# laprade117/interactive-unet

Measured on AMD Instinct MI355X. Metric: voxels/sec (train step + full-volume predict) on 128^3 chunks, higher is better.
Workload: dtype bf16

## Files before the change

### include/iunet.h

```cpp
#ifndef IUNET_H
#define IUNET_H
#ifdef __cplusplus
extern "C" {
#endif

const char* iunet_last_error(void);
int iunet_abi_version(void);

long long iunet_pack_conv3_elems(int Cout, int Cin, int taps, int mode);
int iunet_pack_conv3(int dtype, const void* w, const void* scale, void* dst, int Cout, int Cin, int taps, int mode,
                     void* stream);
long long iunet_pack_first_conv_elems(int Cout, int Cin, int taps);
int iunet_pack_first_conv(int dtype, const void* w, const void* scale, void* dst, int Cout, int Cin, int taps,
                          void* stream);
int iunet_pack_convT(int dtype, const void* w, void* dst, int Cin, int Cout, int npos, void* stream);

int iunet_pack_desc_bytes(void);
int iunet_pack_batch(const void* descs, int n, int quant_max_cout, void* stream);

int iunet_conv3_fwd(int dtype, int nd, const void* x, long long x_sstride, void* y, long long y_sstride,
                    const void* wpk, const void* bias, void* stats, int N, int D, int H, int W, int Cin, int Cout,
                    int epi, int layout, void* stream);
int iunet_conv3_pick_layout(int nd, int N, int D, int H, int W, int Cin, int Cout);
int iunet_conv3_tile_pairs(int nd, int N, int D, int H, int W, int Cin, int Cout);
int iunet_conv3_compact_ok(int nd, int N, int D, int H, int W, int Cin, int Cout, int act, int bw);
int iunet_conv3_packs_compact(int taps, int Cin);
int iunet_conv3_plan(int nd, int N, int D, int H, int W, int Cin, int Cout, int act, int bw, int have_compact, int* fused);
int iunet_conv3_fwd_act(int dtype, int nd, const void* x, long long x_sstride, void* y, long long y_sstride,
                        const void* wpk, const void* bias, void* stats, const void* in_scale, const void* in_shift,
                        int N, int D, int H, int W, int Cin, int Cout, int epi, int layout, void* stream);
int iunet_conv3_num_tiles(int nd, int N, int D, int H, int W);
int iunet_conv3_stats_parts(int nd, int N, int D, int H, int W, int Cout, int layout);
int iunet_first_conv_fwd(int dtype, int nd, const void* x, int in_dtype, const long long* in_strides, void* y,
                         long long y_sstride, const void* w, const void* bias, void* stats, int N, int D, int H, int W,
                         int Cin, int Cout, int relu, void* stream);
int iunet_maxpool_fwd(int dtype, int nd, const void* x, long long x_ss, void* y, long long y_ss, int C, int N, int Do,
                      int Ho, int Wo, void* stream);
int iunet_convT_fwd(int dtype, int nd, const void* x, long long x_ss, void* y, long long y_ss, const void* wpk,
                    const void* bias, int N, int D, int H, int W, int Cin, int Cout, void* stream);
int iunet_head_fwd(int dtype, const void* x, long long x_ss, int C0, const void* w, const void* bias, int ncls,
                   void* logits, void* probs, void* cls, const long long* out_strides, float divisor, int accumulate,
                   int N, int D, int H, int W, void* stream);

long long iunet_f32_pack_conv_elems(int Cout, int Cin, int taps);
int iunet_f32_pack_conv(const void* w, void* dst, void* bias_out, const void* gamma, const void* beta, const void* mean,
                        const void* var, float eps, int Cout, int Cin, int taps, int transposed, void* stream);
int iunet_f32_conv_fwd(int nd, const void* x, int in_dtype, const long long* in_strides, void* y, long long y_ss,
                       const void* wpk, const void* bias, int N, int D, int H, int W, int Cin, int Cout, int relu,
                       int transposed, void* stream);
int iunet_f32_maxpool_fwd(int nd, const void* x, long long x_ss, void* y, long long y_ss, int C, int N, int Do, int Ho, int Wo,
                          void* stream);
int iunet_f32_head_fwd(const void* x, long long x_ss, int C0, const void* w, const void* bias, int ncls, void* logits,
                       void* probs, void* cls, const long long* out_strides, float divisor, int accumulate, int N, int D, int H,
                       int W, void* stream);

int iunet_f32_bn_stats(const void* y, long long y_ss, int C, int N, long long vox, float eps, float momentum, void* mean, void* stdv,
                       void* run_mean, void* run_var, void* stream);
int iunet_f32_bn_relu_fwd(const void* y, long long y_ss, void* z, long long z_ss, const void* mean, const void* stdv, const void* gamma,
                          const void* beta, int C, int N, long long vox, void* stream);
int iunet_f32_bn_relu_bwd(const void* dz, long long dz_ss, const void* y, long long y_ss, void* dy, long long dy_ss, const void* mean,
                          const void* stdv, const void* gamma, const void* beta, void* dgamma, void* dbeta, int C, int N, long long vox,
                          void* stream);
int iunet_f32_maxpool_bwd(int nd, const void* z, long long z_ss, const void* dpool, long long dp_ss, void* dz, long long dz_ss, int C,
                          int N, int Do, int Ho, int Wo, int accumulate, void* stream);
int iunet_f32_wgrad_splits(int nd, int N, int D, int H, int W, int Cin, int Cout);
int iunet_f32_wgrad(int nd, const void* x, long long x_ss, const void* dy, long long dy_ss, void* slab, int N, int D, int H, int W,
                    int Cin, int Cout, int taps, void* stream);
int iunet_f32_head_loss_num_parts(int N, long long vox);
int iunet_f32_head_loss_fwd(const void* x, long long x_ss, int C0, const void* w, const void* bias, int ncls, const void* target,
                            const void* weight, int tdtype, int kind, void* slab, void* out4, void* coef, int N, long long vox,
                            void* stream);
int iunet_f32_head_loss_bwd(const void* x, long long x_ss, int C0, const void* w, const void* bias, int ncls, const void* target,
                            const void* weight, int tdtype, const void* coef, void* dlogits, long long dl_ss, void* dx, long long dx_ss,
                            int N, long long vox, void* stream);
int iunet_f32_channel_sum(const void* t, long long t_ss, void* out, int C, int N, long long vox, void* stream);

int iunet_x2_convT_kc(int Cin);
int iunet_x2_prep(const void* w, void* wv, void* oscale, void* bias_out, const void* gamma, const void* beta, const void* mean,
                  const void* var, const void* bias_in, float eps, float act_in, float act_out, int Cout, int Cin, int taps,
                  int transposed, int chunk, void* stream);
int iunet_x2_prep_desc_bytes(void);
int iunet_x2_prep_batch(const void* table, int n, int rows, void* stream);
int iunet_x2m_prep_batch(const void* table, int n, int rows, void* stream);
int iunet_x2_first_conv_fwd(int nd, const void* x, int in_dtype, const long long* in_strides, void* y, long long y_sstride, int y_lo,
                            const void* w, const void* oscale, const void* bias, float act_scale, int N, int D, int H, int W, int Cin,
                            int Cout, int relu, void* stream);
int iunet_x2_pack_mode(int nd);
int iunet_x2_conv3_fwd(int nd, const void* x, long long x_sstride, int x_lo, void* y, long long y_sstride, int y_lo, const void* wpk,
                       const void* oscale, const void* bias, int N, int D, int H, int W, int Cin, int Cout, int epi, void* stream);
int iunet_x2_conv3_fwd_flag(int nd, const void* x, long long x_sstride, int x_lo, void* y, long long y_sstride, int y_lo, const void* wpk,
                            const void* oscale, const void* bias, int N, int D, int H, int W, int Cin, int Cout, int epi, void* sat, void* stream);
int iunet_x2_maxpool_fwd(int nd, const void* x, long long x_ss, int x_lo, void* y, long long y_ss, int y_lo, int C, int N, int Do,
// ... 197 lines not shown
                           const void* gamma, const void* beta, int groups, float eps, void* slab, void* scale, void* shift, void* mean,
                           void* invstd, int C, int N, int Do, int Ho, int Wo, void* stream);
int iunet_conv3_sample_stats_rows(int dtype, int nd, int N, int D, int H, int W, int Cin, int Cout, int layout);
int iunet_conv3_fwd_sample_stats(int dtype, int nd, const void* x, long long x_sstride, void* y, long long y_sstride, const void* wpk,
                                 void* stats, int N, int D, int H, int W, int Cin, int Cout, int layout, void* stream);
int iunet_gn_relu_fwd_rows(int dtype, const void* y, long long y_ss, void* z, long long z_ss, const void* gamma, const void* beta,
                           int groups, float eps, void* slab, int rows, void* scale, void* shift, void* mean, void* invstd, int C, int N,
                           long long vox, void* stream);
int iunet_gn_relu_pool_fwd_rows(int dtype, int nd, const void* y, long long y_ss, void* z, long long z_ss, void* pooled, long long p_ss,
                                const void* gamma, const void* beta, int groups, float eps, void* slab, int rows, void* scale, void* shift,
                                void* mean, void* invstd, int C, int N, int Do, int Ho, int Wo, void* stream);
int iunet_conv3_dgrad_sample_bnstats(int dtype, int nd, const void* dy, long long dy_sstride, void* dz, long long dz_sstride, const void* wpk,
                                     void* stats, const void* yp, long long yp_sstride, const void* mean, const void* invstd, const void* scale,
                                     const void* shift, int N, int D, int H, int W, int Cin, int Cout, int layout, void* stream);
int iunet_gn_relu_bwd_rows(int dtype, const void* dz, long long dz_ss, const void* y, long long y_ss, void* dy, long long dy_ss,
                           const void* gamma, int groups, const void* scale, const void* shift, const void* mean, const void* invstd,
                           void* dgamma, void* dbeta, void* slab, int rows, void* coef, int C, int N, long long vox, void* stream);
int iunet_gn_relu_pool_bwd(int dtype, int nd, const void* dskip, long long ds_ss, const void* dpool, long long dp_ss, const void* y,
                           long long y_ss, void* dy, long long dy_ss, const void* gamma, int groups, const void* scale, const void* shift,
                           const void* mean, const void* invstd, void* dgamma, void* dbeta, void* slab, void* coef, int C, int N, int Do,
                           int Ho, int Wo, void* stream);
int iunet_bn_relu_pool_bwd(int dtype, int nd, const void* dskip, long long ds_ss, const void* dpool, long long dp_ss,
                           const void* y, long long y_ss, void* dy, long long dy_ss, const void* mean, const void* invstd,
                           const void* gamma, const void* scale, const void* shift, void* dgamma, void* dbeta, void* slab,
                           void* coef, int C, int N, int Do, int Ho, int Wo, void* stream);
int iunet_maxpool_bwd(int dtype, int nd, const void* z, long long z_ss, const void* dpool, long long dp_ss, void* dz,
                      long long dz_ss, int add_skip, int C, int N, int Do, int Ho, int Wo, void* stream);
int iunet_head_loss_num_parts(int N, long long vox);
int iunet_head_loss_fwd(int dtype, const void* x, long long x_ss, int C0, const void* w, const void* bias, int ncls,
                        const void* target, const void* weight, int tdtype, int kind, void* slab, void* out4, void* coef,
                        int N, long long vox, void* stream);
int iunet_head_loss_bwd_num_parts(int N, long long vox, int ncls, int C0);
int iunet_head_loss_bwd(int dtype, const void* x, long long x_ss, int C0, const void* w, const void* bias, int ncls,
                        const void* target, const void* weight, int tdtype, const void* coef, float loss_scale, void* dx,
                        long long dx_ss, void* dwslab, int N, long long vox, void* stream);
int iunet_head_loss_fwd_act(int dtype, const void* x, long long x_ss, int C0, const void* w, const void* bias, int ncls,
                            const void* target, const void* weight, int tdtype, int kind, void* slab, void* out4, void* coef,
                            const void* in_scale, const void* in_shift, int N, long long vox, void* stream);
int iunet_head_loss_bwd_act(int dtype, const void* x, long long x_ss, int C0, const void* w, const void* bias, int ncls,
                            const void* target, const void* weight, int tdtype, const void* coef, float loss_scale, void* dx,
                            long long dx_ss, void* dwslab, const void* in_scale, const void* in_shift, int N, long long vox,
                            void* stream);
int iunet_reduce_slab(void* slab, int nparts, long long n, void* out, float alpha, int accumulate, void* stream);
int iunet_conv3_wgrad_blocks(int nd, int N, int D, int H, int W, int Cin, int Cout);
long long iunet_conv3_wgrad_slab_floats(int nd, int N, int D, int H, int W, int Cin, int Cout);
int iunet_conv3_wgrad(int dtype, int nd, const void* x, long long x_ss, const void* dy, long long dy_ss, void* slab,
                      void* dW, float alpha, int N, int D, int H, int W, int Cin, int Cout, void* stream);
int iunet_conv3_wgrad_act(int dtype, int nd, const void* x, long long x_ss, const void* dy, long long dy_ss, void* slab,
                          void* dW, float alpha, const void* x_scale, const void* x_shift, int N, int D, int H, int W,
                          int Cin, int Cout, void* stream);
int iunet_pack_convT_dgrad(int dtype, const void* w, void* dst, int Cin, int Cout, int npos, void* stream);
int iunet_convT_dgrad(int dtype, int nd, const void* dy, long long dy_ss, void* dx, long long dx_ss, const void* wpk,
                      int N, int D, int H, int W, int Cin, int Cout, void* stream);
int iunet_convT_wgrad_blocks(int nd, int N, int D, int H, int W, int Cin, int Cout);
int iunet_convT_wgrad(int dtype, int nd, const void* x, long long x_ss, const void* dy, long long dy_ss, void* wslab,
                      void* bslab, void* dW, void* db, int N, int D, int H, int W, int Cin, int Cout, void* stream);
int iunet_first_conv_wgrad_blocks(int nd, int N, int D, int H, int W);
int iunet_first_conv_wgrad(int dtype, int nd, const void* x, int in_dtype, const long long* in_strides, const void* dy,
                           long long dy_ss, void* slab, void* dW, int N, int D, int H, int W, int Cin, int Cout,
                           void* stream);
int iunet_first_conv_wgrad_bn(int dtype, int nd, const void* x, int in_dtype, const long long* in_strides, const void* dz,
                              long long dz_ss, const void* y, long long y_ss, const void* mean, const void* invstd,
                              const void* coef, const void* scale, const void* shift, void* slab, void* dW, int N, int D, int H,
                              int W, int Cin, int Cout, void* stream);
int iunet_check_finite(const void* g, long long n, void* flag, void* stream);
int iunet_adamw_step(void* p, const void* g, void* m, void* v, long long n, float lr, float b1, float b2, float eps,
                     float wd, int step, float grad_scale_inv, const void* skip_flag, void* stream);

int iunet_train_state_init(void* state, float loss_scale, int dynamic, void* stream);
int iunet_head_loss_bwd_dev(int dtype, const void* x, long long x_ss, int C0, const void* w, const void* bias, int ncls,
                            const void* target, const void* weight, int tdtype, const void* coef, const void* state, void* dx,
                            long long dx_ss, void* dwslab, const void* in_scale, const void* in_shift, int N, long long vox,
                            void* stream);
int iunet_head_bn_bwd_ok(int C0, int ncls);
int iunet_head_bn_bwd(int dtype, const void* y, long long y_ss, int C0, const void* w, const void* bias, int ncls, const void* target,
                      const void* weight, int tdtype, const void* coef, float loss_scale, const void* state, const void* scale,
                      const void* shift, const void* mean, const void* invstd, const void* gamma, void* dgamma, void* dbeta, void* dy,
                      long long dy_ss, void* dwslab, void* bnslab, void* bncoef, void* dl_scratch, int N, long long vox, void* stream);
int iunet_head_gn_bwd(int dtype, const void* y, long long y_ss, int C0, const void* w, const void* bias, int ncls, const void* target,
                      const void* weight, int tdtype, const void* coef, float loss_scale, const void* state, const void* scale,
                      const void* shift, const void* mean, const void* invstd, const void* gamma, int groups, void* dgamma, void* dbeta, void* dy,
                      long long dy_ss, void* dwslab, void* bnslab, void* bncoef, void* dl_scratch, int N, long long vox, void* stream);
int iunet_head_loss_fwd_act_ps(int dtype, const void* x, long long x_ss, int C0, const void* w, const void* bias, int ncls,
                               const void* target, const void* weight, int tdtype, int kind, void* slab, void* out4, void* coef,
                               const void* in_scale, const void* in_shift, int per_sample, int N, long long vox, void* stream);
int iunet_head_grad_scatter(const void* row, void* dw, void* db, int ncls, int C0, void* stream);
int iunet_adamw_step_dev(void* p, const void* g, void* m, void* v, long long n, float lr, float b1, float b2, float eps, float wd,
                         void* state, int check, float world, void* stream);

typedef struct iunet_train iunet_train;
int iunet_train_create(int dim, int levels, int base, int cin, int ncls, int dtype, int loss_kind, iunet_train** out);
int iunet_train_create_ex(int dim, int levels, int base, int cin, int ncls, int dtype, int loss_kind, int norm, int groups, iunet_train** out);
int iunet_train_create_nested(int dim, int levels, int base, int cin, int ncls, int dtype, int loss_kind, iunet_train** out);
void iunet_train_destroy(iunet_train* t);
long long iunet_train_num_params(const iunet_train* t);
int iunet_train_num_tensors(const iunet_train* t);
int iunet_train_param(const iunet_train* t, int index, char* name, int name_cap, long long* offset, long long* numel);
int iunet_train_num_bn(const iunet_train* t);
long long iunet_train_packed_bytes(const iunet_train* t);
long long iunet_train_workspace_bytes(const iunet_train* t, int N, int D, int H, int W);
int iunet_train_bind(iunet_train* t, void* flat, void* grad, void* m, void* v, void* const* running, void* packed, void* state, void* stream);
int iunet_train_repack(iunet_train* t, void* stream);
int iunet_train_forward_backward(iunet_train* t, const void* x, int in_dtype, const long long* in_strides, const void* target,
                                 const void* weight, int tdtype, int N, int D, int H, int W, void* workspace, void* out4, void* stream);
typedef void (*iunet_train_hook)(void* ctx, int stage);
int iunet_train_forward_backward_hooks(iunet_train* t, const void* x, int in_dtype, const long long* in_strides, const void* target,
                                       const void* weight, int tdtype, int N, int D, int H, int W, void* workspace, void* out4,
                                       iunet_train_hook hook, void* hook_ctx, void* stream);
int iunet_train_update(iunet_train* t, float lr, float b1, float b2, float eps, float wd, float world, void* stream);
// ... 108 lines not shown
```

### interactive-unet_amd/csrc/capi.hip

```cpp
#include "common.h"
#include <cstdarg>
#include <cstdio>

static thread_local char g_err[512] = "";

void iunet_set_error(const char* fmt, ...) {
  va_list ap;
  va_start(ap, fmt);
  vsnprintf(g_err, sizeof(g_err), fmt, ap);
  va_end(ap);
}

#define DT_OK(dt) IUNET_REQUIRE((dt) == 0 || (dt) == 1, "dtype must be 0 (f16) or 1 (bf16), got %d", (dt))

extern "C" {

const char* iunet_last_error(void) { return g_err; }
int iunet_abi_version(void) { return 1; }

int iunet_conv3_num_tiles(int nd, int N, int D, int H, int W) { return iunet_conv3_tiles(nd, N, D, H, W); }

int iunet_conv3_stats_parts(int nd, int N, int D, int H, int W, int Cout, int layout) {
  return layout >= 2 ? iunet_conv3_v4_stats_parts(nd, Cout) : iunet_conv3_tiles(nd, N, D, H, W);
}
// ... 112 lines not shown
  IUNET_REQUIRE(nd == 3 || D == 1, "conv3: 2-D conv needs D == 1");
  const float* par[4] = {(const float*)mean, (const float*)invstd, (const float*)scale, (const float*)shift};
  return iunet_conv3_v4_launch(dtype, nd, dy, dy_sstride, dz, dz_sstride, wpk, nullptr, (float*)stats, N, D, H, W, Cin, Cout, 0, nullptr, nullptr,
                               (hipStream_t)stream, yp, yp_sstride, par, layout == 3, 1, nullptr);
}

int iunet_conv3_dgrad_bnstats_lay(int dtype, int nd, const void* dy, long long dy_sstride, void* dz, long long dz_sstride,
                                  const void* wpk, void* stats, const void* yp, long long yp_sstride, const void* mean,
                                  const void* invstd, const void* scale, const void* shift, int N, int D, int H, int W, int Cin,
                                  int Cout, int layout, void* stream) {
  DT_OK(dtype);
  IUNET_REQUIRE(dy && dz && wpk && stats && yp && mean && invstd && scale && shift, "conv3_dgrad_bnstats: null pointer");
  IUNET_REQUIRE_GRID("conv3_dgrad_bnstats", N, D, H, W);
  IUNET_REQUIRE(layout == 2 || layout == 3, "conv3_dgrad_bnstats: layout 2, or 3 (the compact operator: 2-D, Cin <= 64; iunet_conv3_compact_ok(.., bw = 1)) -- got %d", layout);
  const float* par[4] = {(const float*)mean, (const float*)invstd, (const float*)scale, (const float*)shift};
  return iunet_conv3_launch(dtype, nd, dy, dy_sstride, dz, dz_sstride, wpk, nullptr, (float*)stats, N, D, H, W, Cin, Cout, 0, layout,
                            (hipStream_t)stream, nullptr, nullptr, yp, yp_sstride, par);
}

int iunet_conv3_dgrad_bnstats(int dtype, int nd, const void* dy, long long dy_sstride, void* dz, long long dz_sstride,
                              const void* wpk, void* stats, const void* yp, long long yp_sstride, const void* mean,
                              const void* invstd, const void* scale, const void* shift, int N, int D, int H, int W, int Cin,
                              int Cout, void* stream) {
  return iunet_conv3_dgrad_bnstats_lay(dtype, nd, dy, dy_sstride, dz, dz_sstride, wpk, stats, yp, yp_sstride, mean, invstd, scale, shift,
                                       N, D, H, W, Cin, Cout, 2, stream);
}

int iunet_first_conv_fwd(int dtype, int nd, const void* x, int in_dtype, const long long* in_strides, void* y,
                         long long y_sstride, const void* w, const void* bias, void* stats, int N, int D, int H, int W,
                         int Cin, int Cout, int relu, void* stream) {
  DT_OK(dtype);
  IUNET_REQUIRE(x && y && w && in_strides, "first_conv: null pointer");
  IUNET_REQUIRE(in_dtype >= 0 && in_dtype <= 3, "first_conv: bad input dtype %d", in_dtype);
  IUNET_REQUIRE(nd == 2 || nd == 3, "first_conv: nd must be 2 or 3");
  IUNET_REQUIRE(nd == 3 || D == 1, "first_conv: 2-D needs D == 1");
  return iunet_first_conv_launch(dtype, nd, x, in_dtype, in_strides[0], in_strides[1], in_strides[2], in_strides[3],
                                 in_strides[4], y, y_sstride, w, (const float*)bias, (float*)stats, N, D,
                                 H, W, Cin, Cout, relu, (hipStream_t)stream);
}

int iunet_maxpool_fwd(int dtype, int nd, const void* x, long long x_ss, void* y, long long y_ss, int C, int N, int Do,
                      int Ho, int Wo, void* stream) {
  DT_OK(dtype);
  IUNET_REQUIRE(x && y, "maxpool: null pointer");
  IUNET_REQUIRE(C % 8 == 0, "maxpool: C must be a multiple of 8");
  return iunet_maxpool_launch(dtype, nd, x, x_ss, y, y_ss, C / 8, N, Do, Ho, Wo, (hipStream_t)stream);
}

int iunet_convT_fwd(int dtype, int nd, const void* x, long long x_ss, void* y, long long y_ss, const void* wpk,
                    const void* bias, int N, int D, int H, int W, int Cin, int Cout, void* stream) {
  DT_OK(dtype);
  IUNET_REQUIRE(x && y && wpk, "convT: null pointer");
  return iunet_convT_launch(dtype, nd, x, x_ss, y, y_ss, wpk, (const float*)bias, N, D, H, W, Cin, Cout, (hipStream_t)stream);
}

int iunet_head_fwd(int dtype, const void* x, long long x_ss, int C0, const void* w, const void* bias, int ncls,
                   void* logits, void* probs, void* cls, const long long* out_strides, float divisor, int accumulate,
                   int N, int D, int H, int W, void* stream) {
  DT_OK(dtype);
  IUNET_REQUIRE(x && w && bias && out_strides, "head: null pointer");
  IUNET_REQUIRE(C0 % 8 == 0, "head: C0 must be a multiple of 8");
  return iunet_head_launch(dtype, x, x_ss, C0, (const float*)w, (const float*)bias, ncls, (float*)logits, (float*)probs,
                           (unsigned char*)cls, out_strides, divisor, accumulate, N, D, H, W, (hipStream_t)stream);
}

long long iunet_f32_pack_conv_elems(int Cout, int Cin, int taps) {
  if (Cout <= 0 || Cout % 32 || Cin <= 0 || taps <= 0) return 0;
  return iunet_f32_pack_size(Cout, Cin, taps);
}

int iunet_f32_pack_conv(const void* w, void* dst, void* bias_out, const void* gamma, const void* beta, const void* mean,
                        const void* var, float eps, int Cout, int Cin, int taps, int transposed, void* stream) {
  IUNET_REQUIRE(w && dst, "f32_pack_conv: null pointer");
  IUNET_REQUIRE(Cout > 0 && Cout % 32 == 0 && Cin > 0, "f32_pack_conv: Cout must be a positive multiple of 32, Cin > 0 (got %d, %d)", Cout, Cin);
  IUNET_REQUIRE(transposed ? (taps == 4 || taps == 8) : (taps == 9 || taps == 27 || taps == 1),
                "f32_pack_conv: taps must be 9 / 27 (conv), 1 (pointwise) or 4 / 8 (transposed), got %d", taps);
  IUNET_REQUIRE(!gamma || (beta && mean && var && bias_out), "f32_pack_conv: a BatchNorm fold needs gamma, beta, mean, var and bias_out");
  return iunet_f32_pack_launch((const float*)w, (float*)dst, (float*)bias_out, (const float*)gamma, (const float*)beta,
                               (const float*)mean, (const float*)var, eps, Cout, Cin, taps, transposed, (hipStream_t)stream);
}

int iunet_f32_conv_fwd(int nd, const void* x, int in_dtype, const long long* in_strides, void* y, long long y_ss,
                       const void* wpk, const void* bias, int N, int D, int H, int W, int Cin, int Cout, int relu,
                       int transposed, void* stream) {
  IUNET_REQUIRE(x && y && wpk && in_strides, "f32_conv: null pointer");
  IUNET_REQUIRE(nd == 2 || nd == 3, "f32_conv: nd must be 2 or 3");
  IUNET_REQUIRE(N > 0 && D > 0 && H > 0 && W > 0 && (nd == 3 || D == 1), "f32_conv: bad shape %d %d %d %d", N, D, H, W);
  IUNET_REQUIRE(in_dtype >= 0 && in_dtype <= 3, "f32_conv: bad input dtype %d", in_dtype);
  IUNET_REQUIRE(Cout > 0 && Cout % 32 == 0 && Cin > 0, "f32_conv: Cout must be a positive multiple of 32, Cin > 0 (got %d, %d)", Cout, Cin);
  IUNET_REQUIRE(transposed >= 0 && transposed <= 2, "f32_conv: transposed must be 0 (conv), 1 (ConvTranspose k2 s2) or 2 (1x1), got %d", transposed);
  return iunet_f32_conv_launch(nd, x, in_dtype, in_strides, (float*)y, y_ss, (const float*)wpk, (const float*)bias, N, D, H, W,
                               Cin, Cout, relu, transposed, (hipStream_t)stream);
}

int iunet_f32_maxpool_fwd(int nd, const void* x, long long x_ss, void* y, long long y_ss, int C, int N, int Do, int Ho, int Wo,
                          void* stream) {
  IUNET_REQUIRE(x && y, "f32_maxpool: null pointer");
  IUNET_REQUIRE(nd == 2 || nd == 3, "f32_maxpool: nd must be 2 or 3");
  IUNET_REQUIRE(C > 0 && N > 0 && Do > 0 && Ho > 0 && Wo > 0, "f32_maxpool: bad shape");
  return iunet_f32_maxpool_launch(nd, (const float*)x, x_ss, (float*)y, y_ss, C, N, Do, Ho, Wo, (hipStream_t)stream);
}

int iunet_f32_head_fwd(const void* x, long long x_ss, int C0, const void* w, const void* bias, int ncls, void* logits,
                       void* probs, void* cls, const long long* out_strides, float divisor, int accumulate, int N, int D, int H,
                       int W, void* stream) {
  IUNET_REQUIRE(x && w && bias && out_strides, "f32_head: null pointer");
// ... 96 lines not shown
```

### interactive-unet_amd/csrc/launchers.h

```cpp
#pragma once
#include <hip/hip_runtime.h>

void iunet_set_error(const char* fmt, ...);

int iunet_conv3_launch(int dtype, int nd, const void* x, long long x_sstride, void* y, long long y_sstride,
                       const void* wpk, const float* bias, float* stats, int N, int D, int H, int W, int Cin,
                       int Cout, int epi, int layout, hipStream_t stream, const float* in_scale = nullptr,
                       const float* in_shift = nullptr, const void* bw_y = nullptr, long long bw_y_ss = 0,
                       const float* const* bw_par = nullptr);
int iunet_conv3_tiles(int nd, int N, int D, int H, int W);
long long iunet_pack_conv3_size(int Cout, int Cin, int taps, int mode);
int iunet_pack_conv3_launch(int dtype, const float* w, const float* scale, void* dst, int Cout, int Cin, int taps,
                            int mode, hipStream_t stream);

int iunet_conv3_v4_launch(int dtype, int nd, const void* x, long long x_sstride, void* y, long long y_sstride, const void* wpk,
                          const float* bias, float* stats, int N, int D, int H, int W, int Cin, int Cout, int epi,
                          const float* in_scale, const float* in_shift, hipStream_t stream, const void* bw_y = nullptr,
                          long long bw_y_ss = 0, const float* const* bw_par = nullptr, int compact = 0, int per_sample = 0,
                          int* query_rows = nullptr);
int iunet_conv3_v4_stats_parts(int nd, int Cout);
int iunet_conv3_v4_pairs(int nd, int N, int D, int H, int W, int Cin, int Cout, int bw);
int iunet_conv3_v4_x2_launch(int nd, const void* x, long long x_sstride, int x_lo, void* y, long long y_sstride, int y_lo, const void* wpk,
                             const float* oscale, const float* bias, int N, int D, int H, int W, int Cin, int Cout, int epi,
                             int* sat, hipStream_t stream);
int iunet_conv3_v4_x2_pack_mode(int nd);

int iunet_first_conv_launch(int dtype, int nd, const void* x, int in_dtype, long long sN, long long sC, long long sD,
                            long long sH, long long sW, void* y, long long y_sstride, const void* w,
                            const float* bias, float* stats, int N, int D, int H, int W, int Cin, int Cout, int relu,
                            hipStream_t stream, int out8 = 0);
int iunet_pack_first_conv_launch(int dtype, const float* w, const float* scale, void* dst, int Cout, int Cin, int taps,
                                 hipStream_t stream);
int iunet_maxpool_launch(int dtype, int nd, const void* x, long long x_ss, void* y, long long y_ss, int planes, int N,
                         int Do, int Ho, int Wo, hipStream_t stream);
int iunet_maxpool_q_launch(int nd, const void* x, long long x_ss, void* y, long long y_ss, int planes16, int N, int Do, int Ho, int Wo,
                           hipStream_t stream);
int iunet_convT_launch(int dtype, int nd, const void* x, long long x_ss, void* y, long long y_ss, const void* wpk,
                       const float* bias, int N, int D, int H, int W, int Cin, int Cout, hipStream_t stream, int out8 = 0);
int iunet_pack_convT_launch(int dtype, const float* w, void* dst, int Cin, int Cout, int npos, hipStream_t stream);
int iunet_head_launch(int dtype, const void* x, long long x_ss, int C0, const float* w, const float* bias, int ncls,
                      float* logits, float* probs, unsigned char* cls, const long long* os, float divisor, int accumulate, int N,
                      int D, int H, int W,
                      hipStream_t stream);

long long iunet_f32_pack_size(int Cout, int Cin, int taps);
int iunet_f32_pack_launch(const float* w, float* dst, float* bias_out, const float* gamma, const float* beta,
                          const float* mean, const float* var, float eps, int Cout, int Cin, int taps, int transposed,
                          hipStream_t stream);
int iunet_f32_conv_launch(int nd, const void* x, int in_dtype, const long long* st, float* y, long long y_ss, const float* wpk,
                          const float* bias, int N, int D, int H, int W, int Cin, int Cout, int relu, int transposed,
                          hipStream_t stream);
int iunet_f32_maxpool_launch(int nd, const float* x, long long x_ss, float* y, long long y_ss, int C, int N, int Do, int Ho,
                             int Wo, hipStream_t stream);
int iunet_f32_head_launch(const float* x, long long x_ss, int C0, const float* w, const float* bias, int ncls, float* logits,
                          float* probs, unsigned char* cls, const long long* os, float divisor, int accumulate, int N, int D,
                          int H, int W, hipStream_t stream);

long long iunet_f8_pack_bytes(int Cout, int Cin, int taps);
int iunet_f8_pack_launch(const float* w, const float* gamma, const float* beta, const float* mean, const float* var, float eps,
                         void* dst, float* wscale, float* bias_out, int Cout, int Cin, int taps, hipStream_t stream);
long long iunet_conv3_f8_workspace_floats(int nd, int N, int D, int H, int W, int Cin, int Cout);
int iunet_conv3_f8_launch(int dtype, int nd, const void* x, long long x_sstride, void* y, long long y_sstride, const void* wpk,
                          const float* wscale, const float* bias, int N, int D, int H, int W, int Cin, int Cout, int epi,
                          float* workspace, hipStream_t stream);
int iunet_conv3_f8_launch_q(int dtype, int nd, const void* x, long long x_sstride, int x_fmt, void* y, long long y_sstride, int y_fmt,
                            const void* wpk, const float* wscale, const float* bias, int N, int D, int H, int W, int Cin, int Cout,
                            int epi, float* workspace, hipStream_t stream);

int iunet_f8_k128(int taps, int Cin);
int iunet_conv3_f8k_launch(int dtype, const void* x, long long x_sstride, void* y, long long y_sstride, const void* wpk,
                           const float* wscale, const float* bias, int N, int D, int H, int W, int Cin, int Cout, int epi,
                           int ksplit, float* partial, int small, int in8, int out8, hipStream_t stream);

int iunet_conv3_wgrad_v2_blocks(int N, int D, int H, int W, int Cin, int Cout);
int iunet_conv3_wgrad_v2_launch(int dtype, const void* x, long long x_ss, const void* dy, long long dy_ss, float* slab,
                                int N, int D, int H, int W, int Cin, int Cout, const float* x_scale, const float* x_shift,
                                hipStream_t stream);
int iunet_conv2_wgrad_v2_blocks(int N, int H, int W, int Cin, int Cout, int* rows);
int iunet_conv2_wgrad_v2_launch(int dtype, const void* x, long long x_ss, const void* dy, long long dy_ss, float* slab, int N, int H, int W,
                                int Cin, int Cout, const float* x_scale, const float* x_shift, hipStream_t stream);

int iunet_loss_finalize_launch(const float* slab, int nparts, int ncls, int kind, int has_weight, double nvox_total, float* out4,
                               float* coef, hipStream_t stream);
```

### interactive-unet_amd/csrc/pointwise.hip

```cpp
#include "common.h"
#include "head_out.h"

namespace {

struct FirstConvParams {
  const void* x;
  long long sN, sC, sD, sH, sW;
  int in_dtype;
  void* y; long long y_sstride;
  const void* w;
  const float* bias;
  float* stats;
  int N, D, H, W, Cin, Cout, nd, relu;
  int out8;
};

__device__ __forceinline__ float load_in(const void* p, long long off, int dt) {
  switch (dt) {
    case 0: return ((const float*)p)[off];
    case 1: return (float)((const f16*)p)[off];
    case 2: return (float)((const unsigned char*)p)[off] / 255.0f;
    default: return (float)((const bf16*)p)[off];
  }
}
// ... 155 lines not shown
#pragma unroll
  for (int j = 0; j < 8; ++j) o[j] = from_f32<T>(m[j]);
  *(V8*)(y + n * y_ss + (long long)pl * ovox * 8 + r * 8) = o;
}

template <int ND>
__global__ __launch_bounds__(256) void maxpool_q_kernel(const unsigned char* __restrict__ x, long long x_ss, unsigned char* __restrict__ y,
                                                        long long y_ss, int planes16, int Do, int Ho, int Wo) {
  const long long ovox = (long long)Do * Ho * Wo;
  const long long total = ovox * planes16;
  const long long i = (long long)blockIdx.x * 256 + threadIdx.x;
  if (i >= total) return;
  const int n = blockIdx.y;
  const int pl = (int)(i / ovox);
  const long long r = i - (long long)pl * ovox;
  const int ox = (int)(r % Wo), oy = (int)((r / Wo) % Ho), oz = (int)(r / ((long long)Wo * Ho));
  const int Di = ND == 3 ? Do * 2 : 1, Hi = Ho * 2, Wi = Wo * 2;
  const unsigned char* xp = x + n * x_ss + (long long)pl * Di * Hi * Wi * 16;
  float m[16];
#pragma unroll
  for (int j = 0; j < 16; ++j) m[j] = -INFINITY;
#pragma unroll
  for (int a = 0; a < (ND == 3 ? 2 : 1); ++a)
#pragma unroll
    for (int b = 0; b < 2; ++b)
#pragma unroll
      for (int c = 0; c < 2; ++c) {
        const int z = ND == 3 ? oz * 2 + a : 0;
        const u32x4 v = *(const u32x4*)(xp + (((long long)z * Hi + oy * 2 + b) * Wi + ox * 2 + c) * 16);
#pragma unroll
        for (int d = 0; d < 4; ++d) {
          m[4 * d + 0] = fmaxf(m[4 * d + 0], __builtin_amdgcn_cvt_f32_fp8((int)v[d], 0));
          m[4 * d + 1] = fmaxf(m[4 * d + 1], __builtin_amdgcn_cvt_f32_fp8((int)v[d], 1));
          m[4 * d + 2] = fmaxf(m[4 * d + 2], __builtin_amdgcn_cvt_f32_fp8((int)v[d], 2));
          m[4 * d + 3] = fmaxf(m[4 * d + 3], __builtin_amdgcn_cvt_f32_fp8((int)v[d], 3));
        }
      }
  u32x4 o;
#pragma unroll
  for (int d = 0; d < 4; ++d) {
    int w = __builtin_amdgcn_cvt_pk_fp8_f32(m[4 * d], m[4 * d + 1], 0, false);
    w = __builtin_amdgcn_cvt_pk_fp8_f32(m[4 * d + 2], m[4 * d + 3], w, true);
    o[d] = (unsigned)w;
  }
  *(u32x4*)(y + n * y_ss + ((long long)pl * ovox + r) * 16) = o;
}

struct ConvTParams {
  const void* x; long long x_sstride;
  void* y; long long y_sstride;
  const void* wpk; const float* bias;
  int N, D, H, W, Cin, Cout;
  int out8;
};

template <typename T, int ND, bool O8 = false>
__global__ __launch_bounds__(256) void convT_kernel(ConvTParams p) {
  using V8 = typename Vec8<T>::type;
  constexpr int NPOS = ND == 3 ? 8 : 4;
  const int lane = threadIdx.x & 63, wave = threadIdx.x >> 6;
  const int l15 = lane & 15, q = lane >> 4;
  const int xg = (p.W + 15) / 16;
  const long long rows = (long long)p.D * p.H * xg;
  const long long wid = (long long)blockIdx.x * 4 + wave;
  if (wid >= rows * p.N) return;
  const int n = (int)(wid / rows);
  const long long r = wid - n * rows;
  const int xb = (int)(r % xg), y = (int)((r / xg) % p.H), z = (int)(r / ((long long)xg * p.H));
  const int cob = blockIdx.y;
  const int x = xb * 16 + l15;
  const bool ok = x < p.W;
  const int xc = ok ? x : p.W - 1;
  const long long in_plane = (long long)p.D * p.H * p.W * 8;
  const T* xin = (const T*)p.x + n * p.x_sstride + (((long long)z * p.H + y) * p.W + xc) * 8;
  const int nk = p.Cin >> 5;
  const V8* wp = (const V8*)p.wpk + (long long)cob * nk * NPOS * 2 * 64 + lane;

  f32x4 acc[NPOS][2];
#pragma unroll
  for (int s = 0; s < NPOS; ++s) { acc[s][0] = f32x4{0, 0, 0, 0}; acc[s][1] = f32x4{0, 0, 0, 0}; }
  for (int ks = 0; ks < nk; ++ks) {
    const V8 b = *(const V8*)(xin + (long long)(ks * 4 + q) * in_plane);
#pragma unroll
    for (int s = 0; s < NPOS; ++s) {
      const V8 a0 = wp[((ks * NPOS + s) * 2 + 0) * 64];
      const V8 a1 = wp[((ks * NPOS + s) * 2 + 1) * 64];
      acc[s][0] = mfma16<T>(a0, b, acc[s][0]);
      acc[s][1] = mfma16<T>(a1, b, acc[s][1]);
    }
  }
  const int Do = ND == 3 ? p.D * 2 : 1, Ho = p.H * 2, Wo = p.W * 2;
  const long long out_plane = (long long)Do * Ho * Wo * 8;
  T* yout = (T*)p.y + n * p.y_sstride + (long long)(cob * 4 + q) * out_plane;
  float bias[8];
#pragma unroll
  for (int j = 0; j < 8; ++j) bias[j] = p.bias ? p.bias[cob * 32 + q * 8 + j] : 0.f;
  const int src_lo = ((lane & 48) | (l15 >> 1)) * 4, src_hi = src_lo + 8 * 4;
  const bool odd = l15 & 1;
  const int x0 = xb * 16;
#pragma unroll
  for (int sp = 0; sp < NPOS / 2; ++sp) {
    const int a = ND == 3 ? (sp >> 1) : 0, b = sp & 1;
    typedef int i32x4 __attribute__((ext_vector_type(4)));
    i32x4 oc[2];
#pragma unroll
    for (int c = 0; c < 2; ++c) {
      V8 o;
#pragma unroll
      for (int j = 0; j < 4; ++j) {
        o[j] = from_f32<T>(acc[sp * 2 + c][0][j] + bias[j]);
        o[4 + j] = from_f32<T>(acc[sp * 2 + c][1][j] + bias[4 + j]);
      }
      oc[c] = __builtin_bit_cast(i32x4, o);
    }
    const int oz = ND == 3 ? z * 2 + a : 0;
    T* row = yout + (((long long)oz * Ho + y * 2 + b) * Wo + 2 * x0) * 8;
#pragma unroll
    for (int h = 0; h < 2; ++h) {
      const int src = h ? src_hi : src_lo;
      i32x4 v;
#pragma unroll
      for (int d = 0; d < 4; ++d) {
        const int t0 = __builtin_amdgcn_ds_bpermute(src, oc[0][d]);
        const int t1 = __builtin_amdgcn_ds_bpermute(src, oc[1][d]);
        v[d] = odd ? t1 : t0;
      }
      const int xo = 2 * x0 + 16 * h + l15;
      if (xo < Wo) {
        if constexpr (!O8) *(i32x4*)(row + (16 * h + l15) * 8) = v;
        else e4m3_store8<T>((unsigned char*)p.y + (long long)n * p.y_sstride, cob * 4 + q, ((long long)oz * Ho + y * 2 + b) * Wo + xo,
                            (long long)Do * Ho * Wo, __builtin_bit_cast(u32x4, v));
      }
    }
  }
}

template <typename T, int ND, int NK, bool O8 = false, int NT = 256>
__global__ __launch_bounds__(NT, NT == 256 ? 2 : 1) void convT_lds_kernel(ConvTParams p) {
  constexpr int NW = NT / 64;
  using V8 = typename Vec8<T>::type;
  constexpr int NPOS = ND == 3 ? 8 : 4;
  constexpr int G = 2;
  extern __shared__ __attribute__((aligned(256))) unsigned char smem[];
  const int lane = threadIdx.x & 63, wave = threadIdx.x >> 6;
  const int l15 = lane & 15, q = lane >> 4;
  const int cob = blockIdx.y;
  {
    const u32x4* wsrc = (const u32x4*)p.wpk + (long long)cob * NK * NPOS * 2 * 64;
    stage_to_lds(smem, wsrc, NK * NPOS * 2 * 64, threadIdx.x, NT);
    if (threadIdx.x < 32) ((float*)(smem + NK * NPOS * 2 * 1024))[threadIdx.x] = p.bias ? p.bias[cob * 32 + threadIdx.x] : 0.f;
  }
  __syncthreads();
  const int xg = (p.W + 15) / 16;
  const long long rows = (long long)p.D * p.H * xg, ngroups = rows * p.N;
  const long long in_plane = (long long)p.D * p.H * p.W * 8;
  const int Do = ND == 3 ? p.D * 2 : 1, Ho = p.H * 2, Wo = p.W * 2;
  const long long out_plane = (long long)Do * Ho * Wo * 8;
  const int src_lo = ((lane & 48) | (l15 >> 1)) * 4, src_hi = src_lo + 8 * 4;
  const bool odd = l15 & 1;

  struct Where { int n, z, y, xb; const T* xin; };
  auto locate = [&](long long wid) -> Where {
    wid = wid < ngroups ? wid : ngroups - 1;
    Where w;
    w.n = (int)(wid / rows);
    const long long r = wid - w.n * rows;
    w.xb = (int)(r % xg); w.y = (int)((r / xg) % p.H); w.z = (int)(r / ((long long)xg * p.H));
    const int xc = min(w.xb * 16 + l15, p.W - 1);
    w.xin = (const T*)p.x + w.n * p.x_sstride + (((long long)w.z * p.H + w.y) * p.W + xc) * 8 + (long long)q * in_plane;
    return w;
  };
  const long long stride = (long long)gridDim.x * NW * G;
  long long g0 = ((long long)blockIdx.x * NW + wave) * G;
  if (g0 >= ngroups) return;
  Where cur[G];
  V8 b[G][NK];
#pragma unroll
  for (int g = 0; g < G; ++g) {
    cur[g] = locate(g0 + g);
#pragma unroll
    for (int ks = 0; ks < NK; ++ks) b[g][ks] = *(const V8*)(cur[g].xin + (long long)(ks * 4) * in_plane);
  }
  for (; g0 < ngroups; g0 += stride) {
    Where nxt[G];
#pragma unroll
    for (int g = 0; g < G; ++g) nxt[g] = locate(g0 + stride + g);
    unsigned woff = lane * 16;
    asm volatile("" : "+v"(woff));
    const V8* wl = (const V8*)(smem + woff);
#pragma unroll
    for (int hf = 0; hf < 2; ++hf) {
      constexpr int HP = NPOS / 2;
      f32x4 acc[G][HP][2];
#pragma unroll
      for (int g = 0; g < G; ++g)
#pragma unroll
        for (int s = 0; s < HP; ++s) { acc[g][s][0] = f32x4{0, 0, 0, 0}; acc[g][s][1] = f32x4{0, 0, 0, 0}; }
#pragma unroll
      for (int ks = 0; ks < NK; ++ks) {
#pragma unroll
        for (int s = 0; s < HP; ++s) {
          const V8 a0 = wl[((ks * NPOS + hf * HP + s) * 2 + 0) * 64];
          const V8 a1 = wl[((ks * NPOS + hf * HP + s) * 2 + 1) * 64];
#pragma unroll
          for (int g = 0; g < G; ++g) {
            acc[g][s][0] = mfma16<T>(a0, b[g][ks], acc[g][s][0]);
            acc[g][s][1] = mfma16<T>(a1, b[g][ks], acc[g][s][1]);
          }
        }
        if (hf == 1) {
#pragma unroll
          for (int g = 0; g < G; ++g) b[g][ks] = *(const V8*)(nxt[g].xin + (long long)(ks * 4) * in_plane);
        }
      }
#pragma unroll
      for (int g = 0; g < G; ++g) {
        if (g0 + g >= ngroups) break;
        T* yout = (T*)p.y + cur[g].n * p.y_sstride + (long long)(cob * 4 + q) * out_plane;
        const int x0 = cur[g].xb * 16;
#pragma unroll
        for (int s2 = 0; s2 < HP / 2; ++s2) {
          const int sp = hf * (HP / 2) + s2;
          const int a = ND == 3 ? (sp >> 1) : 0, bb = sp & 1;
          typedef int i32x4 __attribute__((ext_vector_type(4)));
          i32x4 oc[2];
          const f32x4 bias0 = ((const f32x4*)(smem + NK * NPOS * 2 * 1024))[2 * q], bias1 = ((const f32x4*)(smem + NK * NPOS * 2 * 1024))[2 * q + 1];
#pragma unroll
          for (int c = 0; c < 2; ++c) {
            V8 o;
#pragma unroll
            for (int j = 0; j < 4; ++j) {
              o[j] = from_f32<T>(acc[g][s2 * 2 + c][0][j] + bias0[j]);
              o[4 + j] = from_f32<T>(acc[g][s2 * 2 + c][1][j] + bias1[j]);
            }
            oc[c] = __builtin_bit_cast(i32x4, o);
          }
          const int oz = ND == 3 ? cur[g].z * 2 + a : 0;
          if constexpr (O8) {
            unsigned E[2][2];
            e4m3_pack8<T>(__builtin_bit_cast(u32x4, oc[0]), E[0][0], E[0][1]);
            e4m3_pack8<T>(__builtin_bit_cast(u32x4, oc[1]), E[1][0], E[1][1]);
            const bool oq = q & 1;
            const int partner = (lane ^ 16) * 4;
            const unsigned r0 = (unsigned)__builtin_amdgcn_ds_bpermute(partner, (int)(oq ? E[0][0] : E[1][0]));
            const unsigned r1 = (unsigned)__builtin_amdgcn_ds_bpermute(partner, (int)(oq ? E[0][1] : E[1][1]));
            const u32x4 gran = oq ? u32x4{r0, r1, E[1][0], E[1][1]} : u32x4{E[0][0], E[0][1], r0, r1};
            if (x0 + l15 < p.W)
              *(u32x4*)((unsigned char*)p.y + (long long)cur[g].n * p.y_sstride +
                        ((long long)((cob * 4 + q) >> 1) * ((long long)Do * Ho * Wo) + ((long long)oz * Ho + cur[g].y * 2 + bb) * Wo + 2 * (x0 + l15) + (oq ? 1 : 0)) * 16) = gran;
            continue;
          }
          T* row = yout + (((long long)oz * Ho + cur[g].y * 2 + bb) * Wo + 2 * x0) * 8;
#pragma unroll
          for (int h = 0; h < 2; ++h) {
            const int src = h ? src_hi : src_lo;
            i32x4 v;
#pragma unroll
            for (int d = 0; d < 4; ++d) {
              const int t0 = __builtin_amdgcn_ds_bpermute(src, oc[0][d]);
              const int t1 = __builtin_amdgcn_ds_bpermute(src, oc[1][d]);
              v[d] = odd ? t1 : t0;
            }
            if (2 * x0 + 16 * h + l15 < Wo) {
              if constexpr (!O8) *(i32x4*)(row + (16 * h + l15) * 8) = v;
              else e4m3_store8<T>((unsigned char*)p.y + (long long)cur[g].n * p.y_sstride, cob * 4 + q,
                                  ((long long)oz * Ho + cur[g].y * 2 + bb) * Wo + 2 * x0 + 16 * h + l15, (long long)Do * Ho * Wo,
                                  __builtin_bit_cast(u32x4, v));
            }
          }
        }
      }
    }
#pragma unroll
    for (int g = 0; g < G; ++g) cur[g] = nxt[g];
  }
}

template <typename T, int ND, bool O8 = false>
__global__ __launch_bounds__(256) void convT_chunk_kernel(ConvTParams p) {
  constexpr int NK = 4;
  using V8 = typename Vec8<T>::type;
  constexpr int NPOS = ND == 3 ? 8 : 4;
  constexpr int G = 2;
  extern __shared__ __attribute__((aligned(256))) unsigned char smem[];
  const int lane = threadIdx.x & 63, wave = threadIdx.x >> 6;
  const int l15 = lane & 15, q = lane >> 4;
  const int cob = blockIdx.y;
  const int nchunks = (p.Cin >> 5) / NK;
  const u32x4* wsrc = (const u32x4*)p.wpk + (long long)cob * nchunks * NK * NPOS * 2 * 64;
  const int xg = (p.W + 15) / 16;
  const long long rows = (long long)p.D * p.H * xg, ngroups = rows * p.N;
  const long long in_plane = (long long)p.D * p.H * p.W * 8;
  const int Do = ND == 3 ? p.D * 2 : 1, Ho = p.H * 2, Wo = p.W * 2;
  const long long out_plane = (long long)Do * Ho * Wo * 8;
  float bias[8];
#pragma unroll
  for (int j = 0; j < 8; ++j) bias[j] = p.bias ? p.bias[cob * 32 + q * 8 + j] : 0.f;
  const int src_lo = ((lane & 48) | (l15 >> 1)) * 4, src_hi = src_lo + 8 * 4;
  const bool odd = l15 & 1;
  const V8* wl = (const V8*)smem + lane;

  for (long long base = (long long)blockIdx.x * 4 * G; base < ngroups; base += (long long)gridDim.x * 4 * G) {
    const long long g0 = base + wave * G;
    int n_[G], z_[G], y_[G], xb_[G];
    const T* xin_[G];
#pragma unroll
    for (int g = 0; g < G; ++g) {
      const long long wid = g0 + g < ngroups ? g0 + g : ngroups - 1;
      n_[g] = (int)(wid / rows);
      const long long r = wid - n_[g] * rows;
      xb_[g] = (int)(r % xg); y_[g] = (int)((r / xg) % p.H); z_[g] = (int)(r / ((long long)xg * p.H));
      const int xc = min(xb_[g] * 16 + l15, p.W - 1);
      xin_[g] = (const T*)p.x + n_[g] * p.x_sstride + (((long long)z_[g] * p.H + y_[g]) * p.W + xc) * 8;
    }
    f32x4 acc[G][NPOS][2];
#pragma unroll
    for (int g = 0; g < G; ++g)
#pragma unroll
      for (int s = 0; s < NPOS; ++s) { acc[g][s][0] = f32x4{0, 0, 0, 0}; acc[g][s][1] = f32x4{0, 0, 0, 0}; }
    constexpr int CHB = NK * NPOS * 2 * 1024;
    const unsigned lds0 = (unsigned)(size_t)(__attribute__((address_space(3))) unsigned char*)smem;
    auto dma_chunk = [&](int ch) {
      const u32x4* src = wsrc + (long long)ch * (CHB / 16);
#pragma unroll
      for (int i = 0; i < CHB / 16 / 256; ++i) {
        const int base = (i * 4 + wave) * 64;
        const unsigned dst = __builtin_amdgcn_readfirstlane(lds0 + (ch & 1) * CHB + base * 16);
        const u32x4* gsrc = src + base + lane;
        unsigned keep;
        asm volatile("s_mov_b32 %0, m0\n\ts_mov_b32 m0, %2\n\ts_nop 0\n\tglobal_load_lds_dwordx4 %1, off\n\ts_mov_b32 m0, %0"
                     : "=&s"(keep) : "v"(gsrc), "s"(dst) : "memory");
      }
    };
    auto load_b = [&](int ch, V8 (&bb)[G][NK]) {
#pragma unroll
      for (int g = 0; g < G; ++g)
#pragma unroll
        for (int ks = 0; ks < NK; ++ks) bb[g][ks] = *(const V8*)(xin_[g] + (long long)((ch * NK + ks) * 4 + q) * in_plane);
    };
    V8 bcur[G][NK], bnext[G][NK];
    __syncthreads();
    dma_chunk(0);
    load_b(0, bcur);
    for (int ch = 0; ch < nchunks; ++ch) {
      asm volatile("s_waitcnt vmcnt(0)" ::: "memory");
      __syncthreads();
      if (ch + 1 < nchunks) { dma_chunk(ch + 1); load_b(ch + 1, bnext); }
      const V8* wb = wl + (ch & 1) * (CHB / 16);
#pragma unroll
      for (int ks = 0; ks < NK; ++ks)
#pragma unroll
        for (int s = 0; s < NPOS; ++s) {
          const V8 a0 = wb[((ks * NPOS + s) * 2 + 0) * 64];
          const V8 a1 = wb[((ks * NPOS + s) * 2 + 1) * 64];
#pragma unroll
          for (int g = 0; g < G; ++g) {
            acc[g][s][0] = mfma16<T>(a0, bcur[g][ks], acc[g][s][0]);
            acc[g][s][1] = mfma16<T>(a1, bcur[g][ks], acc[g][s][1]);
          }
        }
      if (ch + 1 < nchunks) {
#pragma unroll
        for (int g = 0; g < G; ++g)
#pragma unroll
          for (int ks = 0; ks < NK; ++ks) bcur[g][ks] = bnext[g][ks];
      }
    }
#pragma unroll
    for (int g = 0; g < G; ++g) {
      if (g0 + g >= ngroups) break;
      T* yout = (T*)p.y + n_[g] * p.y_sstride + (long long)(cob * 4 + q) * out_plane;
      const int x0 = xb_[g] * 16;
#pragma unroll
      for (int sp = 0; sp < NPOS / 2; ++sp) {
        const int a = ND == 3 ? (sp >> 1) : 0, bb = sp & 1;
        typedef int i32x4 __attribute__((ext_vector_type(4)));
        i32x4 oc[2];
#pragma unroll
        for (int c = 0; c < 2; ++c) {
          V8 o;
#pragma unroll
          for (int j = 0; j < 4; ++j) {
            o[j] = from_f32<T>(acc[g][sp * 2 + c][0][j] + bias[j]);
            o[4 + j] = from_f32<T>(acc[g][sp * 2 + c][1][j] + bias[4 + j]);
          }
          oc[c] = __builtin_bit_cast(i32x4, o);
        }
        const int oz = ND == 3 ? z_[g] * 2 + a : 0;
        T* row = yout + (((long long)oz * Ho + y_[g] * 2 + bb) * Wo + 2 * x0) * 8;
#pragma unroll
        for (int h = 0; h < 2; ++h) {
          const int src = h ? src_hi : src_lo;
          i32x4 v;
#pragma unroll
          for (int d = 0; d < 4; ++d) {
            const int t0 = __builtin_amdgcn_ds_bpermute(src, oc[0][d]);
            const int t1 = __builtin_amdgcn_ds_bpermute(src, oc[1][d]);
            v[d] = odd ? t1 : t0;
          }
          if (2 * x0 + 16 * h + l15 < Wo) {
// ... 70 lines not shown
  FirstConvParams p;
  p.x = x; p.sN = sN; p.sC = sC; p.sD = sD; p.sH = sH; p.sW = sW; p.in_dtype = in_dtype;
  p.y = y; p.y_sstride = y_sstride; p.w = w; p.bias = bias; p.stats = stats;
  p.N = N; p.D = D; p.H = H; p.W = W; p.Cin = Cin; p.Cout = Cout; p.nd = nd; p.relu = relu; p.out8 = out8;
  const int TZ = nd == 3 ? 4 : 1, TY = nd == 3 ? 8 : 16, TX = nd == 3 ? 16 : 32;
  dim3 grid(N * ((D + TZ - 1) / TZ) * ((H + TY - 1) / TY) * ((W + TX - 1) / TX), Cout / 32);
#define IUNET_FC(TT, NDV, CI) hipLaunchKernelGGL((first_conv_kernel<TT, NDV, CI>), grid, dim3(256), 0, stream, p)
#define IUNET_FC_CIN(TT, NDV)                                              \
  switch (Cin) { case 1: IUNET_FC(TT, NDV, 1); break; case 2: IUNET_FC(TT, NDV, 2); break; \
                 case 3: IUNET_FC(TT, NDV, 3); break; default: IUNET_FC(TT, NDV, 4); break; }
  if (dtype == 0) { if (nd == 3) { IUNET_FC_CIN(f16, 3) } else { IUNET_FC_CIN(f16, 2) } }
  else            { if (nd == 3) { IUNET_FC_CIN(bf16, 3) } else { IUNET_FC_CIN(bf16, 2) } }
#undef IUNET_FC_CIN
#undef IUNET_FC
  IUNET_CHECK_HIP(hipGetLastError());
  return IUNET_OK;
}

int iunet_pack_first_conv_launch(int dtype, const float* w, const float* scale, void* dst, int Cout, int Cin, int taps,
                                 hipStream_t stream) {
  const int total = Cout * (((taps * Cin + 31) / 32) * 32);
  if (dtype == 0) hipLaunchKernelGGL(pack_first_conv_kernel<f16>, dim3((total + 255) / 256), dim3(256), 0, stream, w, scale, (f16*)dst, Cout, Cin, taps);
  else hipLaunchKernelGGL(pack_first_conv_kernel<bf16>, dim3((total + 255) / 256), dim3(256), 0, stream, w, scale, (bf16*)dst, Cout, Cin, taps);
  IUNET_CHECK_HIP(hipGetLastError());
  return IUNET_OK;
}

int iunet_maxpool_launch(int dtype, int nd, const void* x, long long x_ss, void* y, long long y_ss, int planes, int N,
                         int Do, int Ho, int Wo, hipStream_t stream) {
  const long long total = (long long)Do * Ho * Wo * planes;
  dim3 grid((unsigned)((total + 255) / 256), N);
  if (dtype == 0) {
    if (nd == 3) hipLaunchKernelGGL((maxpool_kernel<f16, 3>), grid, dim3(256), 0, stream, (const f16*)x, x_ss, (f16*)y, y_ss, planes, Do, Ho, Wo);
    else hipLaunchKernelGGL((maxpool_kernel<f16, 2>), grid, dim3(256), 0, stream, (const f16*)x, x_ss, (f16*)y, y_ss, planes, Do, Ho, Wo);
  } else {
    if (nd == 3) hipLaunchKernelGGL((maxpool_kernel<bf16, 3>), grid, dim3(256), 0, stream, (const bf16*)x, x_ss, (bf16*)y, y_ss, planes, Do, Ho, Wo);
    else hipLaunchKernelGGL((maxpool_kernel<bf16, 2>), grid, dim3(256), 0, stream, (const bf16*)x, x_ss, (bf16*)y, y_ss, planes, Do, Ho, Wo);
  }
  IUNET_CHECK_HIP(hipGetLastError());
  return IUNET_OK;
}

int iunet_maxpool_q_launch(int nd, const void* x, long long x_ss, void* y, long long y_ss, int planes16, int N, int Do, int Ho, int Wo,
                           hipStream_t stream) {
  const long long total = (long long)Do * Ho * Wo * planes16;
  dim3 grid((unsigned)((total + 255) / 256), N);
  if (nd == 3) hipLaunchKernelGGL((maxpool_q_kernel<3>), grid, dim3(256), 0, stream, (const unsigned char*)x, x_ss, (unsigned char*)y, y_ss, planes16, Do, Ho, Wo);
  else hipLaunchKernelGGL((maxpool_q_kernel<2>), grid, dim3(256), 0, stream, (const unsigned char*)x, x_ss, (unsigned char*)y, y_ss, planes16, Do, Ho, Wo);
  IUNET_CHECK_HIP(hipGetLastError());
  return IUNET_OK;
}

int iunet_convT_launch(int dtype, int nd, const void* x, long long x_ss, void* y, long long y_ss, const void* wpk,
                       const float* bias, int N, int D, int H, int W, int Cin, int Cout, hipStream_t stream, int out8) {
  IUNET_REQUIRE(Cin % 32 == 0 && Cout % 32 == 0, "convT: Cin (%d) and Cout (%d) must be multiples of 32", Cin, Cout);
  IUNET_REQUIRE(!out8 || nd == 3, "convT: e4m3 planes out exist in 3-D only (the K = 128 fp8 convolution's format)");
  ConvTParams p;
  p.x = x; p.x_sstride = x_ss; p.y = y; p.y_sstride = y_ss; p.wpk = wpk; p.bias = bias;
  p.N = N; p.D = D; p.H = H; p.W = W; p.Cin = Cin; p.Cout = Cout; p.out8 = out8;
  const long long waves = (long long)N * D * H * ((W + 15) / 16);
  const int nk = Cin / 32;
  static const int chunk4 = getenv("IUNET_CONVT_CHUNK4") ? atoi(getenv("IUNET_CONVT_CHUNK4")) : 0;
  static const int res8 = getenv("IUNET_CONVT_RES8") ? atoi(getenv("IUNET_CONVT_RES8")) : 1;
  if ((nk <= 4 || (nk == 8 && res8 && nd == 3 && waves >= 2048)) && waves >= 256 && !(chunk4 && nk == 4)) {
    const int npos = nd == 3 ? 8 : 4;
    const int lds = nk * npos * 2 * 1024 + 128;
    const bool big = lds > 65 * 1024;
    const int per_wg = big ? 16 : 8;
    int gx = (int)((waves + per_wg - 1) / per_wg);
    static const int cap_all = getenv("IUNET_CONVT_CAP") ? atoi(getenv("IUNET_CONVT_CAP")) : 512;
    const int cap = (big ? cap_all / 2 : cap_all) / (Cout / 32) > 8 ? (big ? cap_all / 2 : cap_all) / (Cout / 32) : 8;
    if (gx > cap) gx = cap;
    dim3 g2(gx, Cout / 32);
#define CTL(TT, NDV, NKV, NTV) do { if (out8 && NDV == 3) { IUNET_SET_MAX_LDS((convT_lds_kernel<TT, 3, NKV, true, NTV>), lds); \
    hipLaunchKernelGGL((convT_lds_kernel<TT, 3, NKV, true, NTV>), g2, dim3(NTV), lds, stream, p); } else { IUNET_SET_MAX_LDS((convT_lds_kernel<TT, NDV, NKV, false, NTV>), lds); \
    hipLaunchKernelGGL((convT_lds_kernel<TT, NDV, NKV, false, NTV>), g2, dim3(NTV), lds, stream, p); } } while (0)
#define CTL_NK(TT, NDV) switch (nk) { case 1: CTL(TT, NDV, 1, 256); break; case 2: CTL(TT, NDV, 2, 256); break; case 3: CTL(TT, NDV, 3, 256); break; \
    case 4: CTL(TT, NDV, 4, 256); break; default: CTL(TT, NDV, 8, (NDV == 3 ? 512 : 256)); break; }
    if (dtype == 0) { if (nd == 3) { CTL_NK(f16, 3) } else { CTL_NK(f16, 2) } }
    else            { if (nd == 3) { CTL_NK(bf16, 3) } else { CTL_NK(bf16, 2) } }
#undef CTL_NK
#undef CTL
    IUNET_CHECK_HIP(hipGetLastError());
    return IUNET_OK;
  }
  if (nk >= 4 && nk % 4 == 0 && waves >= 64) {
    const int npos = nd == 3 ? 8 : 4;
    const int lds = 2 * 4 * npos * 2 * 1024;
    int gx = (int)((waves + 7) / 8);
    const int cap = 512 / (Cout / 32) > 1 ? 512 / (Cout / 32) : 1;
    if (gx > cap) gx = cap;
    dim3 g2(gx, Cout / 32);
#define CTC(TT, NDV) do { if (out8 && NDV == 3) { IUNET_SET_MAX_LDS((convT_chunk_kernel<TT, 3, true>), lds); \
    hipLaunchKernelGGL((convT_chunk_kernel<TT, 3, true>), g2, dim3(256), lds, stream, p); } else { IUNET_SET_MAX_LDS((convT_chunk_kernel<TT, NDV>), lds); \
    hipLaunchKernelGGL((convT_chunk_kernel<TT, NDV>), g2, dim3(256), lds, stream, p); } } while (0)
    if (dtype == 0) { if (nd == 3) CTC(f16, 3); else CTC(f16, 2); } else { if (nd == 3) CTC(bf16, 3); else CTC(bf16, 2); }
#undef CTC
    IUNET_CHECK_HIP(hipGetLastError());
    return IUNET_OK;
  }
  dim3 grid((unsigned)((waves + 3) / 4), Cout / 32);
  if (dtype == 0) {
    if (nd == 3 && out8) hipLaunchKernelGGL((convT_kernel<f16, 3, true>), grid, dim3(256), 0, stream, p);
    else if (nd == 3) hipLaunchKernelGGL((convT_kernel<f16, 3>), grid, dim3(256), 0, stream, p);
    else hipLaunchKernelGGL((convT_kernel<f16, 2>), grid, dim3(256), 0, stream, p);
  } else {
    if (nd == 3 && out8) hipLaunchKernelGGL((convT_kernel<bf16, 3, true>), grid, dim3(256), 0, stream, p);
    else if (nd == 3) hipLaunchKernelGGL((convT_kernel<bf16, 3>), grid, dim3(256), 0, stream, p);
    else hipLaunchKernelGGL((convT_kernel<bf16, 2>), grid, dim3(256), 0, stream, p);
  }
  IUNET_CHECK_HIP(hipGetLastError());
  return IUNET_OK;
}

int iunet_pack_convT_launch(int dtype, const float* w, void* dst, int Cin, int Cout, int npos, hipStream_t stream) {
  const long long total = (long long)Cin * Cout * npos;
  const int blocks = (int)((total + 255) / 256 < 4096 ? (total + 255) / 256 : 4096);
  if (dtype == 0) hipLaunchKernelGGL(pack_convT_kernel<f16>, dim3(blocks), dim3(256), 0, stream, w, (f16*)dst, Cin, Cout, npos);
  else hipLaunchKernelGGL(pack_convT_kernel<bf16>, dim3(blocks), dim3(256), 0, stream, w, (bf16*)dst, Cin, Cout, npos);
  IUNET_CHECK_HIP(hipGetLastError());
  return IUNET_OK;
}

int iunet_head_launch(int dtype, const void* x, long long x_ss, int C0, const float* w, const float* bias, int ncls,
                      float* logits, float* probs, unsigned char* cls, const long long* os, float divisor, int accumulate, int N,
                      int D, int H, int W, hipStream_t stream) {
  IUNET_REQUIRE(ncls >= 2 && ncls <= 10, "head: num_classes must be 2..10 (got %d)", ncls);
  HeadParams p;
  p.x = x; p.x_sstride = x_ss; p.planes = C0 / 8; p.w = w; p.bias = bias;
  if (const int rc = head_out_fill(p.o, "head", logits, probs, cls, os, divisor, accumulate)) return rc;
  p.N = N; p.D = D; p.H = H; p.W = W;
  const long long vox = (long long)D * H * W;
  dim3 grid((unsigned)((vox + 255) / 256), N);
#define IUNET_HEAD(TT, NC) case NC: hipLaunchKernelGGL((head_kernel<TT, NC>), grid, dim3(256), 0, stream, p); break;
#define IUNET_HEAD_ALL(TT) switch (ncls) { IUNET_HEAD(TT, 2) IUNET_HEAD(TT, 3) IUNET_HEAD(TT, 4) IUNET_HEAD(TT, 5) \
  IUNET_HEAD(TT, 6) IUNET_HEAD(TT, 7) IUNET_HEAD(TT, 8) IUNET_HEAD(TT, 9) IUNET_HEAD(TT, 10) }
  if (dtype == 0) { IUNET_HEAD_ALL(f16) } else { IUNET_HEAD_ALL(bf16) }
#undef IUNET_HEAD_ALL
#undef IUNET_HEAD
  IUNET_CHECK_HIP(hipGetLastError());
  return IUNET_OK;
}
```

### interactive-unet_amd/csrc/train_misc.hip

```cpp
#include "common.h"

namespace {


struct ConvTDgradParams {
  const void* dy; long long dy_ss;
  void* dx; long long dx_ss;
  const void* wpk;
  int N, D, H, W, Cin, Cout;
};

template <typename T, int ND>
__global__ __launch_bounds__(256) void convT_dgrad_kernel(ConvTDgradParams p) {
  using V8 = V8T<T>;
  constexpr int NPOS = ND == 3 ? 8 : 4;
  const int lane = threadIdx.x & 63, wave = threadIdx.x >> 6;
  const int l15 = lane & 15, q = lane >> 4;
  const int xg = (p.W + 15) / 16;
  const long long rows = (long long)p.D * p.H * xg;
  const long long wid = (long long)blockIdx.x * 4 + wave;
  if (wid >= rows * p.N) return;
  const int n = (int)(wid / rows);
  const long long r = wid - n * rows;
  const int xb = (int)(r % xg), y = (int)((r / xg) % p.H), z = (int)(r / ((long long)xg * p.H));
  const int cib = blockIdx.y;
  const int x = xb * 16 + l15;
  const bool ok = x < p.W;
  const int xc = ok ? x : p.W - 1;
  const int Do = ND == 3 ? p.D * 2 : 1, Ho = p.H * 2, Wo = p.W * 2;
  const long long out_plane = (long long)Do * Ho * Wo * 8;
  const T* dyin = (const T*)p.dy + n * p.dy_ss;
  const int nk = p.Cout >> 5;
  const V8* wp = (const V8*)p.wpk + (long long)cib * NPOS * nk * 2 * 64 + lane;
  f32x4 acc0 = f32x4{0, 0, 0, 0}, acc1 = f32x4{0, 0, 0, 0};
#pragma unroll
  for (int s = 0; s < NPOS; ++s) {
    const int a = ND == 3 ? (s >> 2) : 0, b = (s >> 1) & 1, c = s & 1;
    const int oz = ND == 3 ? z * 2 + a : 0;
    const long long voff = (((long long)oz * Ho + y * 2 + b) * Wo + xc * 2 + c) * 8;
    for (int kc = 0; kc < nk; ++kc) {
      const V8 bf = *(const V8*)(dyin + (long long)(kc * 4 + q) * out_plane + voff);
      const V8 a0 = wp[((s * nk + kc) * 2 + 0) * 64];
      const V8 a1 = wp[((s * nk + kc) * 2 + 1) * 64];
      acc0 = mfma16<T>(a0, bf, acc0);
      acc1 = mfma16<T>(a1, bf, acc1);
    }
  }
  const long long in_plane = (long long)p.D * p.H * p.W * 8;
  V8 o;
#pragma unroll
  for (int j = 0; j < 4; ++j) { o[j] = from_f32<T>(acc0[j]); o[4 + j] = from_f32<T>(acc1[j]); }
  if (ok)
    *(V8*)((T*)p.dx + n * p.dx_ss + (long long)(cib * 4 + q) * in_plane + (((long long)z * p.H + y) * p.W + x) * 8) = o;
}

template <typename T, int ND, int NK, int NCI>
__global__ __launch_bounds__(256, (NCI * NK * (ND == 3 ? 16 : 8) <= 64) ? 2 : 1) void convT_dgrad_lds_kernel(ConvTDgradParams p) {
  using V8 = V8T<T>;
  constexpr int NPOS = ND == 3 ? 8 : 4, G = 2;
  constexpr int WCI = NPOS * NK * 2 * 64;
  extern __shared__ __attribute__((aligned(256))) unsigned char smem[];
  const int lane = threadIdx.x & 63, wave = threadIdx.x >> 6;
  const int l15 = lane & 15, q = lane >> 4;
  const int cib0 = blockIdx.y * NCI;
  {
    const u32x4* wsrc = (const u32x4*)p.wpk + (long long)cib0 * WCI;
    stage_to_lds(smem, wsrc, NCI * WCI, threadIdx.x, 256);
  }
  __syncthreads();
  const int xg = (p.W + 15) / 16;
  const long long rows = (long long)p.D * p.H * xg, ngroups = rows * p.N;
  const int Do = ND == 3 ? p.D * 2 : 1, Ho = p.H * 2, Wo = p.W * 2;
  const long long out_plane = (long long)Do * Ho * Wo * 8, in_plane = (long long)p.D * p.H * p.W * 8;
  for (long long g0 = ((long long)blockIdx.x * 4 + wave) * G; g0 < ngroups; g0 += (long long)gridDim.x * 4 * G) {
    unsigned woff = lane * 16;
    asm volatile("" : "+v"(woff));
    const V8* wl = (const V8*)(smem + woff);
    f32x4 acc[NCI][G][2];
    const T* dyb[G];
    long long xoff[G];
    bool okg[G];
#pragma unroll
    for (int g = 0; g < G; ++g) {
      const long long wid = g0 + g < ngroups ? g0 + g : ngroups - 1;
      const int n = (int)(wid / rows);
      const long long r = wid - n * rows;
      const int xb = (int)(r % xg), y = (int)((r / xg) % p.H), z = (int)(r / ((long long)xg * p.H));
      const int x = xb * 16 + l15, xc = min(x, p.W - 1);
      okg[g] = x < p.W && g0 + g < ngroups;
      const int oz = ND == 3 ? z * 2 : 0;
      dyb[g] = (const T*)p.dy + n * p.dy_ss + (((long long)oz * Ho + y * 2) * Wo + xc * 2) * 8;
      xoff[g] = n * p.dx_ss + (long long)(cib0 * 4 + q) * in_plane + (((long long)z * p.H + y) * p.W + x) * 8;
#pragma unroll
      for (int c = 0; c < NCI; ++c) { acc[c][g][0] = f32x4{0, 0, 0, 0}; acc[c][g][1] = f32x4{0, 0, 0, 0}; }
    }
#pragma unroll
    for (int s = 0; s < NPOS; ++s) {
      const int a = ND == 3 ? (s >> 2) : 0, b = (s >> 1) & 1, c = s & 1;
      const long long voff = (((long long)a * Ho + b) * Wo + c) * 8;
#pragma unroll
      for (int kc = 0; kc < NK; ++kc) {
        V8 bf[G];
#pragma unroll
        for (int g = 0; g < G; ++g) bf[g] = *(const V8*)(dyb[g] + (long long)(kc * 4 + q) * out_plane + voff);
#pragma unroll
        for (int c = 0; c < NCI; ++c) {
          const V8 a0 = wl[c * WCI + ((s * NK + kc) * 2 + 0) * 64];
          const V8 a1 = wl[c * WCI + ((s * NK + kc) * 2 + 1) * 64];
#pragma unroll
          for (int g = 0; g < G; ++g) {
            acc[c][g][0] = mfma16<T>(a0, bf[g], acc[c][g][0]);
            acc[c][g][1] = mfma16<T>(a1, bf[g], acc[c][g][1]);
          }
        }
      }
    }
#pragma unroll
    for (int c = 0; c < NCI; ++c)
#pragma unroll
      for (int g = 0; g < G; ++g) {
        V8 o;
#pragma unroll
        for (int j = 0; j < 4; ++j) { o[j] = from_f32<T>(acc[c][g][0][j]); o[4 + j] = from_f32<T>(acc[c][g][1][j]); }
        if (okg[g]) *(V8*)((T*)p.dx + xoff[g] + (long long)c * 4 * in_plane) = o;
      }
  }
}

template <typename T>
__global__ void pack_convT_dgrad_kernel(const float* __restrict__ w, T* __restrict__ dst, int Cin, int Cout, int npos) {
  const long long total = (long long)Cin * Cout * npos;
  const int nk = Cout >> 5;
  for (long long i = blockIdx.x * (long long)blockDim.x + threadIdx.x; i < total; i += (long long)gridDim.x * blockDim.x) {
    long long r = i;
    const int j = r & 7; r >>= 3;
    const int lane = r & 63; r >>= 6;
    const int t = r & 1; r >>= 1;
    const int kc = r % nk; r /= nk;
    const int s = r % npos;
    const int cib = r / npos;
    const int row = lane & 15, qq = lane >> 4;
    const int ci = cib * 32 + 8 * (row >> 2) + 4 * t + (row & 3);
    const int co = kc * 32 + 8 * qq + j;
    dst[i] = from_f32<T>(w[((long long)ci * Cout + co) * npos + s]);
  }
}

typedef short s16x4w __attribute__((ext_vector_type(4)));
typedef short s16x8w __attribute__((ext_vector_type(8)));
typedef __attribute__((address_space(3))) s16x4w* lds_s4w_ptr;

template <typename T>
__device__ __forceinline__ typename Vec8<T>::type tr_frag2(unsigned addr, unsigned hi_off) {
  const s16x4w lo = __builtin_amdgcn_ds_read_tr16_b64_v4i16((lds_s4w_ptr)addr);
  const s16x4w hi = __builtin_amdgcn_ds_read_tr16_b64_v4i16((lds_s4w_ptr)(addr + hi_off));
  const s16x8w v = __builtin_shufflevector(lo, hi, 0, 1, 2, 3, 4, 5, 6, 7);
  return __builtin_bit_cast(typename Vec8<T>::type, v);
}

struct ConvTWgradParams {
  const void* x; long long x_ss;
  const void* dy; long long dy_ss;
  float* wslab;
  float* bslab;
  int N, D, H, W, Cin, Cout;
  int tilesZ, tilesY, tilesX;
};

template <typename T, int ND, int NCI>
__global__ __launch_bounds__(256, 2) void convT_wgrad_kernel(ConvTWgradParams p) {
  using V8 = V8T<T>;
  constexpr int NPOS = ND == 3 ? 8 : 4;
  constexpr int TZ = ND == 3 ? 2 : 1, TY = ND == 3 ? 4 : 8, TX = 16;
  constexpr int NVI = TZ * TY * TX;
  constexpr int OZ = ND == 3 ? 2 * TZ : 1, OY = 2 * TY, OX = 2 * TX;
  constexpr int NVO = OZ * OY * OX;
  constexpr int PLANE_X = NVI * 16 + 64, PLANE_Y = NVO * 16 + 64;
  constexpr int OFF_Y = 4 * PLANE_X;
  constexpr int NKS = NVI / 32;
  constexpr int PL = NPOS / 4;
  extern __shared__ __attribute__((aligned(256))) unsigned char smem[];
  const unsigned lds0 = (unsigned)(size_t)(__attribute__((address_space(3))) unsigned char*)smem;
  const int tid = threadIdx.x, lane = tid & 63;
  const int wave = __builtin_amdgcn_readfirstlane(tid >> 6);
  const int g = lane >> 4, i16 = lane & 15, q = i16 >> 2, pp = i16 & 3, gh = g >> 1, gl = g & 1;
  const int cib0 = blockIdx.y * NCI, cob = blockIdx.z;
  const unsigned laneX = lds0 + (pp >> 1) * PLANE_X + (pp & 1) * 8 + (gh * 16 + gl * 8 + q) * 16;
  const unsigned laneY = lds0 + OFF_Y + (pp >> 1) * PLANE_Y + (pp & 1) * 8 + (gh * 2 * OX + 2 * (gl * 8 + q)) * 16;
  unsigned pos_off[PL];
#pragma unroll
  for (int i = 0; i < PL; ++i) {
    const int s = wave * PL + i;
    const int a = ND == 3 ? (s >> 2) : 0, b = (s >> 1) & 1, c = s & 1;
    pos_off[i] = (unsigned)(((a * OY + b) * OX + c) * 16);
  }
  f32x4 acc[NCI][PL][2][2];
#pragma unroll
  for (int c = 0; c < NCI; ++c)
#pragma unroll
    for (int i = 0; i < PL; ++i)
#pragma unroll
      for (int t = 0; t < 2; ++t) { acc[c][i][t][0] = f32x4{0, 0, 0, 0}; acc[c][i][t][1] = f32x4{0, 0, 0, 0}; }
  float bacc[8] = {0.f, 0.f, 0.f, 0.f, 0.f, 0.f, 0.f, 0.f};

  const int tps = p.tilesZ * p.tilesY * p.tilesX, ntiles = tps * p.N;
  const int Do = ND == 3 ? p.D * 2 : 1, Ho = p.H * 2, Wo = p.W * 2;
  const long long in_plane = (long long)p.D * p.H * p.W * 8, out_plane = (long long)Do * Ho * Wo * 8;
  constexpr int XIT = NVI * 4 / 256, YIT = NVO * 4 / 256;
  u32x4 xr[NCI * XIT], xkeep[NCI > 1 ? XIT : 1];
  V8 yr[YIT];
  auto load_tile = [&](int tile) {
    const int n = tile / tps;
    int trem = tile - n * tps;
    const int tz_i = trem / (p.tilesY * p.tilesX);
    trem -= tz_i * p.tilesY * p.tilesX;
    const int ty_i = trem / p.tilesX, tx_i = trem - ty_i * p.tilesX;
    const int z0 = tz_i * TZ, y0 = ty_i * TY, x0 = tx_i * TX;
    const T* xin = (const T*)p.x + (long long)n * p.x_ss + (long long)cib0 * 4 * in_plane;
    const T* dyin = (const T*)p.dy + (long long)n * p.dy_ss + (long long)cob * 4 * out_plane;
#pragma unroll
    for (int k = 0; k < NCI * XIT; ++k) {
      const int it = tid + k * 256;
      const int pl = it / NVI, pix = it - pl * NVI;
      const int px = pix % TX, t2 = pix / TX, py = t2 % TY, pz = t2 / TY;
      const int gz = z0 + pz, gy = y0 + py, gx = x0 + px;
      u32x4 v = u32x4{0u, 0u, 0u, 0u};
      if (gz < p.D && gy < p.H && gx < p.W) v = *(const u32x4*)(xin + pl * in_plane + (((long long)gz * p.H + gy) * p.W + gx) * 8);
      xr[k] = v;
    }
#pragma unroll
    for (int k = 0; k < YIT; ++k) {
      const int it = tid + k * 256;
      const int pl = it & 3, pix = it >> 2;
      const int px = pix % OX, t2 = pix / OX, py = t2 % OY, pz = t2 / OY;
      const int gz = 2 * z0 + pz, gy = 2 * y0 + py, gx = 2 * x0 + px;
      V8 v;
#pragma unroll
      for (int j = 0; j < 8; ++j) v[j] = from_f32<T>(0.f);
      if (gz < Do && gy < Ho && gx < Wo) v = *(const V8*)(dyin + pl * out_plane + (((long long)gz * Ho + gy) * Wo + gx) * 8);
      yr[k] = v;
    }
  };
  auto commit_x = [&](const u32x4* src) {
#pragma unroll
    for (int k = 0; k < XIT; ++k) {
      const int it = tid + k * 256;
      const int pl = it / NVI, pix = it - pl * NVI;
      *(u32x4*)(smem + pl * PLANE_X + pix * 16) = src[k];
    }
  };
  auto commit_tile = [&]() {
    commit_x(xr);
    if (NCI > 1) {
#pragma unroll
      for (int k = 0; k < XIT; ++k) xkeep[k] = xr[XIT + k];
    }
#pragma unroll
    for (int k = 0; k < YIT; ++k) {
      const int it = tid + k * 256;
      const int pl = it & 3, pix = it >> 2;
      *(V8*)(smem + OFF_Y + pl * PLANE_Y + pix * 16) = yr[k];
#pragma unroll
      for (int j = 0; j < 8; ++j) bacc[j] += to_f32<T>(yr[k][j]);
    }
  };
  if ((int)blockIdx.x < ntiles) load_tile(blockIdx.x);
  for (int tile = blockIdx.x; tile < ntiles; tile += gridDim.x) {
    __syncthreads();
    commit_tile();
    __syncthreads();
    if (tile + (int)gridDim.x < ntiles) load_tile(tile + gridDim.x);
#pragma unroll
    for (int c = 0; c < NCI; ++c) {
      if (c > 0) {
        __syncthreads();
        commit_x(xkeep);
        __syncthreads();
      }
#pragma unroll
      for (int ks = 0; ks < NKS; ++ks) {
        const int r = 2 * ks, rz = r / TY, ry = r % TY;
        const unsigned offX = (unsigned)(r * TX * 16);
        const unsigned offY = (unsigned)(((2 * rz * OY + 2 * ry) * OX) * 16);
        const V8 a0 = tr_frag2<T>(laneX + offX, 64);
        const V8 a1 = tr_frag2<T>(laneX + offX + 2 * PLANE_X, 64);
#pragma unroll
        for (int i = 0; i < PL; ++i) {
          const V8 b0 = tr_frag2<T>(laneY + offY + pos_off[i], 128);
          const V8 b1 = tr_frag2<T>(laneY + offY + pos_off[i] + 2 * PLANE_Y, 128);
          acc[c][i][0][0] = mfma16<T>(a0, b0, acc[c][i][0][0]);
          acc[c][i][0][1] = mfma16<T>(a0, b1, acc[c][i][0][1]);
          acc[c][i][1][0] = mfma16<T>(a1, b0, acc[c][i][1][0]);
          acc[c][i][1][1] = mfma16<T>(a1, b1, acc[c][i][1][1]);
        }
      }
    }
  }
#pragma unroll
  for (int c = 0; c < NCI; ++c) {
    float* ws = p.wslab + ((((long long)blockIdx.x * (gridDim.y * NCI) + cib0 + c) * gridDim.z + cob) * NPOS) * 1024;
#pragma unroll
    for (int i = 0; i < PL; ++i) {
      const int s = wave * PL + i;
#pragma unroll
      for (int t = 0; t < 2; ++t)
#pragma unroll
        for (int u = 0; u < 2; ++u)
#pragma unroll
          for (int j = 0; j < 4; ++j) ws[s * 1024 + (t * 16 + 4 * g + j) * 32 + u * 16 + i16] = acc[c][i][t][u][j];
    }
  }
  if (blockIdx.y == 0) {
    __syncthreads();
    float* red = (float*)smem;
#pragma unroll
    for (int j = 0; j < 8; ++j) red[tid * 8 + j] = bacc[j];
    __syncthreads();
    if (tid < 32) {
// ... 198 lines not shown
  for (int i = tid; i < 32 * KKP; i += 256)
    slab[i] = red[i] + red[32 * KKP + i] + red[2 * 32 * KKP + i] + red[3 * 32 * KKP + i];
}

__global__ __launch_bounds__(256) void first_wgrad_reduce_kernel(const float* __restrict__ slab, int nb, int Cout, int Cin, int taps,
                                                                 int KKP, float* __restrict__ dW) {
  __shared__ float red[8][32];
  const int total = Cout * Cin * taps;
  const int o = threadIdx.x & 31, grp = threadIdx.x >> 5;
  const int i = blockIdx.x * 32 + o;
  float s = 0.f;
  if (i < total) {
    const int tap = i % taps, c = (i / taps) % Cin, co = i / (taps * Cin);
    const float* src = slab + (long long)co * KKP + tap * Cin + c;
    const long long st = (long long)Cout * KKP;
    int b = grp;
    float s1 = 0.f, s2 = 0.f, s3 = 0.f;
    for (; b + 24 < nb; b += 32) {
      const float a0 = src[b * st], a1 = src[(b + 8) * st], a2 = src[(b + 16) * st], a3 = src[(b + 24) * st];
      s += a0; s1 += a1; s2 += a2; s3 += a3;
    }
    for (; b < nb; b += 8) s += src[b * st];
    s = (s + s1) + (s2 + s3);
  }
  red[grp][o] = s;
  __syncthreads();
  if (grp == 0 && i < total) {
    float a = red[0][o];
#pragma unroll
    for (int g = 1; g < 8; ++g) a += red[g][o];
    dW[i] = a;
  }
}

}

#define DT_OK(dt) IUNET_REQUIRE((dt) == 0 || (dt) == 1, "dtype must be 0 (f16) or 1 (bf16), got %d", (dt))

extern "C" {

int iunet_pack_convT_dgrad(int dtype, const void* w, void* dst, int Cin, int Cout, int npos, void* stream) {
  DT_OK(dtype);
  IUNET_REQUIRE(w && dst, "pack_convT_dgrad: null pointer");
  IUNET_REQUIRE(Cin >= 32 && Cout >= 32 && Cin % 32 == 0 && Cout % 32 == 0, "pack_convT_dgrad: channels must be positive multiples of 32");
  IUNET_REQUIRE(npos == 4 || npos == 8, "pack_convT_dgrad: npos must be 4 or 8");
  const long long total = (long long)Cin * Cout * npos;
  const int blocks = (int)((total + 255) / 256 < 4096 ? (total + 255) / 256 : 4096);
  if (dtype == 0) hipLaunchKernelGGL(pack_convT_dgrad_kernel<f16>, dim3(blocks), dim3(256), 0, (hipStream_t)stream, (const float*)w, (f16*)dst, Cin, Cout, npos);
  else hipLaunchKernelGGL(pack_convT_dgrad_kernel<bf16>, dim3(blocks), dim3(256), 0, (hipStream_t)stream, (const float*)w, (bf16*)dst, Cin, Cout, npos);
  IUNET_CHECK_HIP(hipGetLastError());
  return IUNET_OK;
}

int iunet_convT_dgrad(int dtype, int nd, const void* dy, long long dy_ss, void* dx, long long dx_ss, const void* wpk,
                      int N, int D, int H, int W, int Cin, int Cout, void* stream) {
  DT_OK(dtype);
  IUNET_REQUIRE(dy && dx && wpk, "convT_dgrad: null pointer");
  IUNET_REQUIRE(nd == 2 || nd == 3, "convT_dgrad: nd must be 2 or 3");
  IUNET_REQUIRE_GRID("convT_dgrad", N, D, H, W);
  IUNET_REQUIRE(Cin >= 32 && Cout >= 32 && Cin % 32 == 0 && Cout % 32 == 0, "convT_dgrad: channels must be positive multiples of 32 (%d, %d)", Cin, Cout);
  ConvTDgradParams p;
  p.dy = dy; p.dy_ss = dy_ss; p.dx = dx; p.dx_ss = dx_ss; p.wpk = wpk; p.N = N; p.D = D; p.H = H; p.W = W; p.Cin = Cin; p.Cout = Cout;
  const long long waves = (long long)N * D * H * ((W + 15) / 16);
  const int nk = Cout / 32;
  if (nk <= 4 && waves >= 256) {
    const int nci = (nk <= 2 && (Cin / 32) % 2 == 0 && (nd == 3 ? 8 : 4) * nk * 2 * 1024 * 2 <= 32768) ? 2 : 1;
    const int lds = (nd == 3 ? 8 : 4) * nk * 2 * 1024 * nci;
    int gx = (int)((waves + 7) / 8);
    const int cap = 1024 / (Cin / 32 / nci);
    if (gx > cap) gx = cap;
    dim3 g2(gx, Cin / 32 / nci);
#define CDL(TT, NDV, NKV) do { if (nci == 2) { IUNET_SET_MAX_LDS((convT_dgrad_lds_kernel<TT, NDV, NKV, 2>), lds); \
      hipLaunchKernelGGL((convT_dgrad_lds_kernel<TT, NDV, NKV, 2>), g2, dim3(256), lds, (hipStream_t)stream, p); } \
    else { IUNET_SET_MAX_LDS((convT_dgrad_lds_kernel<TT, NDV, NKV, 1>), lds); \
      hipLaunchKernelGGL((convT_dgrad_lds_kernel<TT, NDV, NKV, 1>), g2, dim3(256), lds, (hipStream_t)stream, p); } } while (0)
#define CDL_NK(TT, NDV) switch (nk) { case 1: CDL(TT, NDV, 1); break; case 2: CDL(TT, NDV, 2); break; case 3: CDL(TT, NDV, 3); break; default: CDL(TT, NDV, 4); break; }
    if (dtype == 0) { if (nd == 3) { CDL_NK(f16, 3) } else { CDL_NK(f16, 2) } }
    else            { if (nd == 3) { CDL_NK(bf16, 3) } else { CDL_NK(bf16, 2) } }
#undef CDL_NK
#undef CDL
    IUNET_CHECK_HIP(hipGetLastError());
    return IUNET_OK;
  }
  dim3 grid((unsigned)((waves + 3) / 4), Cin / 32);
  if (dtype == 0) { if (nd == 3) hipLaunchKernelGGL((convT_dgrad_kernel<f16, 3>), grid, dim3(256), 0, (hipStream_t)stream, p);
                    else hipLaunchKernelGGL((convT_dgrad_kernel<f16, 2>), grid, dim3(256), 0, (hipStream_t)stream, p); }
  else { if (nd == 3) hipLaunchKernelGGL((convT_dgrad_kernel<bf16, 3>), grid, dim3(256), 0, (hipStream_t)stream, p);
         else hipLaunchKernelGGL((convT_dgrad_kernel<bf16, 2>), grid, dim3(256), 0, (hipStream_t)stream, p); }
  IUNET_CHECK_HIP(hipGetLastError());
  return IUNET_OK;
}

int iunet_convT_wgrad_blocks(int nd, int N, int D, int H, int W, int Cin, int Cout) {
  if (N < 1 || D < 1 || H < 1 || W < 1 || Cin < 32 || Cout < 32) return 0;
  const int TZ = nd == 3 ? 2 : 1, TY = nd == 3 ? 4 : 8, TX = 16;
  const long long ntiles = (long long)N * ((D + TZ - 1) / TZ) * ((H + TY - 1) / TY) * ((W + TX - 1) / TX);
  const int nci = (Cin / 32) % 2 == 0 ? 2 : 1;
  const int pairs = (Cin / 32 / nci) * (Cout / 32);
  long long nb = (512 + pairs - 1) / pairs;
  if (nb > ntiles) nb = ntiles;
  return (int)(nb < 1 ? 1 : nb);
}

int iunet_convT_wgrad(int dtype, int nd, const void* x, long long x_ss, const void* dy, long long dy_ss, void* wslab,
                      void* bslab, void* dW, void* db, int N, int D, int H, int W, int Cin, int Cout, void* stream) {
  DT_OK(dtype);
  IUNET_REQUIRE(x && dy && wslab && bslab && dW && db, "convT_wgrad: null pointer");
  IUNET_REQUIRE(Cin >= 32 && Cout >= 32 && Cin % 32 == 0 && Cout % 32 == 0, "convT_wgrad: channels must be positive multiples of 32");
  IUNET_REQUIRE(nd == 2 || nd == 3, "convT_wgrad: nd must be 2 or 3");
  IUNET_REQUIRE_GRID("convT_wgrad", N, D, H, W);
  ConvTWgradParams p;
  p.x = x; p.x_ss = x_ss; p.dy = dy; p.dy_ss = dy_ss; p.wslab = (float*)wslab; p.bslab = (float*)bslab;
  p.N = N; p.D = D; p.H = H; p.W = W; p.Cin = Cin; p.Cout = Cout;
  const int TZ = nd == 3 ? 2 : 1, TY = nd == 3 ? 4 : 8, TX = 16;
  p.tilesZ = (D + TZ - 1) / TZ; p.tilesY = (H + TY - 1) / TY; p.tilesX = (W + TX - 1) / TX;
  const int nb = iunet_convT_wgrad_blocks(nd, N, D, H, W, Cin, Cout);
  const int npos = nd == 3 ? 8 : 4;
  const int nvi = 128, nvo = nd == 3 ? 1024 : 512;
  const int lds = 4 * (nvi * 16 + 64) + 4 * (nvo * 16 + 64);
  const int nci = (Cin / 32) % 2 == 0 ? 2 : 1;
  dim3 grid(nb, Cin / 32 / nci, Cout / 32);
#define CTW(TT, NDV) do { if (nci == 2) { IUNET_SET_MAX_LDS((convT_wgrad_kernel<TT, NDV, 2>), lds); \
      hipLaunchKernelGGL((convT_wgrad_kernel<TT, NDV, 2>), grid, dim3(256), lds, (hipStream_t)stream, p); } \
    else { IUNET_SET_MAX_LDS((convT_wgrad_kernel<TT, NDV, 1>), lds); \
      hipLaunchKernelGGL((convT_wgrad_kernel<TT, NDV, 1>), grid, dim3(256), lds, (hipStream_t)stream, p); } } while (0)
  if (dtype == 0) { if (nd == 3) CTW(f16, 3); else CTW(f16, 2); } else { if (nd == 3) CTW(bf16, 3); else CTW(bf16, 2); }
#undef CTW
  const long long total = (long long)Cin * Cout * npos;
  hipLaunchKernelGGL(convT_wgrad_reduce_kernel, dim3((unsigned)(total / 64)), dim3(256), 0, (hipStream_t)stream,
                     (const float*)wslab, nb, Cin, Cout, npos, (float*)dW);
  IUNET_CHECK_HIP(hipGetLastError());
  return iunet_reduce_slab(bslab, nb, Cout, db, 1.0f, 0, stream);
}

int iunet_first_conv_wgrad_blocks(int nd, int N, int D, int H, int W) {
  if (N < 1 || D < 1 || H < 1 || W < 1) return 0;
  const int TZ = nd == 3 ? 4 : 1, TY = nd == 3 ? 8 : 16, TX = nd == 3 ? 16 : 32;
  const long long ntiles = (long long)N * ((D + TZ - 1) / TZ) * ((H + TY - 1) / TY) * ((W + TX - 1) / TX);
  return (int)(ntiles < 512 ? ntiles : 512);
}

static int first_wgrad_impl(int dtype, int nd, const void* x, int in_dtype, const long long* in_strides, const void* dy,
                            long long dy_ss, void* slab, void* dW, int N, int D, int H, int W, int Cin, int Cout,
                            const void* yraw, long long y_ss, const float* mean, const float* invstd, const float* coef,
                            const float* scale, const float* shift, void* stream) {
  DT_OK(dtype);
  IUNET_REQUIRE(x && dy && slab && dW && in_strides, "first_conv_wgrad: null pointer");
  IUNET_REQUIRE(Cin >= 1 && Cin <= 4 && Cout >= 32 && Cout % 32 == 0, "first_conv_wgrad: Cin 1..4, Cout a positive multiple of 32");
  IUNET_REQUIRE(nd == 2 || nd == 3, "first_conv_wgrad: nd must be 2 or 3");
  IUNET_REQUIRE(in_dtype >= 0 && in_dtype <= 3, "first_conv_wgrad: bad input dtype %d", in_dtype);
  IUNET_REQUIRE_GRID("first_conv_wgrad", N, D, H, W);
  FirstWgradParams p;
  p.x = x; p.sN = in_strides[0]; p.sC = in_strides[1]; p.sD = in_strides[2]; p.sH = in_strides[3]; p.sW = in_strides[4];
  p.in_dtype = in_dtype; p.dy = dy; p.dy_ss = dy_ss; p.slab = (float*)slab;
  p.yraw = yraw; p.y_ss = y_ss; p.mean = mean; p.invstd = invstd; p.coef = coef; p.scale = scale; p.shift = shift;
  p.N = N; p.D = D; p.H = H; p.W = W; p.Cin = Cin; p.Cout = Cout;
  const int TZ = nd == 3 ? 4 : 1, TY = nd == 3 ? 8 : 16, TX = nd == 3 ? 16 : 32;
  p.tilesZ = (D + TZ - 1) / TZ; p.tilesY = (H + TY - 1) / TY; p.tilesX = (W + TX - 1) / TX;
  const int nb = iunet_first_conv_wgrad_blocks(nd, N, D, H, W);
  const int taps = nd == 3 ? 27 : 9, KKP = ((taps * Cin + 15) / 16) * 16;
  const int npix = (nd == 3 ? 6 : 1) * (TY + 2) * (TX + 2);
  const int xs_bytes = ((Cin * npix * 2 + 255) / 256) * 256;
  int lds = xs_bytes + 4 * (512 * 16 + 64);
  if (lds < 4 * 32 * KKP * 4) lds = 4 * 32 * KKP * 4;
  dim3 grid(nb, Cout / 32);
#define FW(TT, NDV, CI) do { IUNET_SET_MAX_LDS((first_wgrad_kernel<TT, NDV, CI>), lds); \
    hipLaunchKernelGGL((first_wgrad_kernel<TT, NDV, CI>), grid, dim3(256), lds, (hipStream_t)stream, p); } while (0)
#define FW_CIN(TT, NDV) switch (Cin) { case 1: FW(TT, NDV, 1); break; case 2: FW(TT, NDV, 2); break; case 3: FW(TT, NDV, 3); break; default: FW(TT, NDV, 4); break; }
  if (dtype == 0) { if (nd == 3) { FW_CIN(f16, 3) } else { FW_CIN(f16, 2) } }
  else            { if (nd == 3) { FW_CIN(bf16, 3) } else { FW_CIN(bf16, 2) } }
#undef FW_CIN
#undef FW
  const int total = Cout * Cin * taps;
  hipLaunchKernelGGL(first_wgrad_reduce_kernel, dim3((total + 31) / 32), dim3(256), 0, (hipStream_t)stream,
                     (const float*)slab, nb, Cout, Cin, taps, KKP, (float*)dW);
  IUNET_CHECK_HIP(hipGetLastError());
  return IUNET_OK;
}

int iunet_first_conv_wgrad(int dtype, int nd, const void* x, int in_dtype, const long long* in_strides, const void* dy,
                           long long dy_ss, void* slab, void* dW, int N, int D, int H, int W, int Cin, int Cout,
                           void* stream) {
  return first_wgrad_impl(dtype, nd, x, in_dtype, in_strides, dy, dy_ss, slab, dW, N, D, H, W, Cin, Cout, nullptr, 0, nullptr,
                          nullptr, nullptr, nullptr, nullptr, stream);
}
// ... 13 lines not shown
```

### interactive-unet_amd/csrc/train_net.hip

```cpp
#include "common.h"
#include "pack_desc.h"
#include <algorithm>
#include <cstdio>
#include <cstdlib>
#include <string>
#include <vector>

namespace {

long long align256(long long v) { return (v + 255) & ~255ll; }
bool env_on(const char* name) { const char* e = getenv(name); return e != nullptr && e[0] != 0; }

struct TParam { std::string name; long long off, numel; };

struct TPack {
  int cout = 0, cin = 0, dg = 0;
  long long buf[2] = {-1, -1};
  long long elems[2] = {0, 0};
};

struct TConv {
  std::string name;
  int ci, co, l, first;
  long long w, gamma, beta;
  int bn;
  TPack fwd, dgr;
  long long first_pk = -1, first_elems = 0;
};
struct TUp { int ci, co, l; long long w, b, fwd, dgr; };

struct TWs {
  std::vector<long long> y, z, dz, scale, shift, mean, invstd;
  std::vector<long long> cat, dcat, bslab, pin, dpin;
  std::vector<long long> up, ndcat, dT;
  long long dy, stats, wslab, bnslab, bncoef, lslab, hslab, htmp, out4, coef, bytes;
};

}

struct iunet_train {
  int norm = 0, groups = 8;
  int dim, levels, base, cin, ncls, dtype, kind;
  int taps, npos;
  bool fuse_act, fuse_bw, head_act, gn_conv_stats, gn_bw, head_bn, gn_head;
  std::vector<int> ch;
  std::vector<TParam> params;
  long long nparams = 0;
  std::vector<TConv> conv;
  std::vector<TUp> up;
  bool nested = false;
  std::vector<std::pair<int, int>> nodes;
  std::vector<int> node_at;
  long long head_w = 0, head_b = 0;
  long long packed_bytes = 0, table_off = 0;
  int ndesc = 0;
  float *flat = nullptr, *grad = nullptr, *m = nullptr, *v = nullptr, *state = nullptr;
  std::vector<float*> running;
  unsigned char* packed = nullptr;
};

namespace {

int stage_index(const iunet_train* n, bool dec, int l) { return dec ? n->levels + (n->levels - 2 - l) : l; }
const TConv& conv_of(const iunet_train* n, bool dec, int l, int j) { return n->conv[2 * stage_index(n, dec, l) + (j - 1)]; }

void pack_alloc(TPack& p, int cout, int cin, int taps, int dg, long long& pk) {
  p.cout = cout; p.cin = cin; p.dg = dg;
  auto take = [&](int k, int mode) { p.elems[k] = iunet_pack_conv3_elems(cout, cin, taps, mode | dg); p.buf[k] = pk; pk = align256(pk + p.elems[k] * 2); };
  take(0, 2);
  if (iunet_conv3_packs_compact(taps, dg ? cout : cin) > 0) take(1, 6);
}

int pack_pick(const TPack& p, int nd, int N, int D, int H, int W, bool act, bool bw, long long* off, int* fused = nullptr) {
  const int in_ch = p.dg ? p.cout : p.cin, out_ch = p.dg ? p.cin : p.cout;
  const int lay = iunet_conv3_plan(nd, N, D, H, W, in_ch, out_ch, act, bw, p.buf[1] >= 0, fused);
  *off = p.buf[lay == 3];
  return lay;
}

TWs ws_layout_nested(const iunet_train* n, int N, int D, int H, int W);

TWs ws_layout(const iunet_train* n, int N, int D, int H, int W) {
  if (n->nested) return ws_layout_nested(n, N, D, H, W);
  TWs L;
  const int lv = n->levels, dim = n->dim;
  long long off = 0;
  auto act = [&](long long elems) { const long long o = off; off = align256(off + elems * 2); return o; };
  auto f32 = [&](long long nfl) { const long long o = off; off = align256(off + nfl * 4); return o; };
  auto dims = [&](int l, int& d, int& h, int& w) { d = dim == 3 ? D >> l : 1; h = H >> l; w = W >> l; };
  auto vox = [&](int l) { int d, h, w; dims(l, d, h, w); return (long long)d * h * w; };
  const size_t nc = n->conv.size();
  L.y.assign(nc, -1); L.z.assign(nc, -1); L.dz.assign(nc, -1);
  L.scale.assign(nc, -1); L.shift.assign(nc, -1); L.mean.assign(nc, -1); L.invstd.assign(nc, -1);
  long long max_stats = 0, max_wslab = 0, max_bn = 0, max_dy = 0;
  for (size_t k = 0; k < nc; ++k) {
    const TConv& c = n->conv[k];
    int d, h, w;
// ... 99 lines not shown
  const long long v0 = vox(0);
  L.dy = act((long long)N * max_dy);
  L.stats = f32(max_stats); L.wslab = f32(max_wslab); L.bnslab = f32(max_bn);
  L.bncoef = f32(3ll * n->ch[lv - 1]);
  L.lslab = f32((long long)iunet_head_loss_num_parts(N, v0) * n->ncls * 8);
  L.hslab = f32((long long)iunet_head_loss_bwd_num_parts(N, v0, n->ncls, n->ch[0]) * n->ncls * (n->ch[0] + 1));
  L.htmp = f32((long long)n->ncls * (n->ch[0] + 1));
  L.out4 = f32(4);
  L.coef = f32((long long)n->ncls * 3);
  L.bytes = off;
  return L;
}

int copy_slot(void* dst, long long dst_ss, const void* src, long long src_ss, long long elems, int N, void* stream) {
  IUNET_CHECK_HIP(hipMemcpy2DAsync(dst, (size_t)dst_ss * 2, src, (size_t)src_ss * 2, (size_t)elems * 2, (size_t)N, hipMemcpyDeviceToDevice,
                                   (hipStream_t)stream));
  return IUNET_OK;
}

}

extern "C" {

int iunet_train_create(int dim, int levels, int base, int cin, int ncls, int dtype, int loss_kind, iunet_train** out) {
  return iunet_train_create_ex(dim, levels, base, cin, ncls, dtype, loss_kind, 0, 8, out);
}
static int train_create(int dim, int levels, int base, int cin, int ncls, int dtype, int loss_kind, int norm, int groups, bool nested, iunet_train** out);
int iunet_train_create_ex(int dim, int levels, int base, int cin, int ncls, int dtype, int loss_kind, int norm, int groups, iunet_train** out) {
  return train_create(dim, levels, base, cin, ncls, dtype, loss_kind, norm, groups, false, out);
}
int iunet_train_create_nested(int dim, int levels, int base, int cin, int ncls, int dtype, int loss_kind, iunet_train** out) {
  return train_create(dim, levels, base, cin, ncls, dtype, loss_kind, 0, 8, true, out);
}
static int train_create(int dim, int levels, int base, int cin, int ncls, int dtype, int loss_kind, int norm, int groups, bool nested, iunet_train** out) {
  IUNET_REQUIRE(out != nullptr, "train_create: null handle pointer");
  IUNET_REQUIRE(norm == 0 || (norm == 1 && groups > 0 && base % groups == 0), "train_create: norm must be 0 (batch) or 1 (group, groups dividing base): %d, %d groups", norm, groups);
  IUNET_REQUIRE(dim == 2 || dim == 3, "train_create: dim must be 2 or 3 (got %d)", dim);
  if (nested) IUNET_REQUIRE(levels >= 2 && levels <= 9, "train_create_nested: levels must be 2..9 (got %d)", levels);
  else IUNET_REQUIRE(levels >= 2 && levels <= 6, "train_create: levels must be 2..6 (got %d)", levels);
  IUNET_REQUIRE(base > 0 && base % 32 == 0, "train_create: base channels must be a positive multiple of 32 (got %d)", base);
  IUNET_REQUIRE(base == 32 || base == 64, "train_create: the fused head + loss kernels take 32 or 64 head input channels (base %d)", base);
  IUNET_REQUIRE(cin >= 1 && cin <= 4, "train_create: 1..4 input channels (got %d)", cin);
  IUNET_REQUIRE(ncls >= 2 && ncls <= 10, "train_create: 2..10 classes (app.py:162; got %d)", ncls);
  IUNET_REQUIRE(dtype == 0 || dtype == 1, "train_create: dtype must be 0 (fp16) or 1 (bf16), got %d", dtype);
  IUNET_REQUIRE(loss_kind >= 0 && loss_kind <= 6, "train_create: loss kind must be 0..6 (got %d)", loss_kind);
  IUNET_REQUIRE(iunet_pack_desc_bytes() == (int)sizeof(PackDesc), "train_create: PackDesc layout mismatch");
  iunet_train* n = new iunet_train();
  n->dim = dim; n->levels = levels; n->base = base; n->cin = cin; n->ncls = ncls; n->dtype = dtype; n->kind = loss_kind;
  n->taps = dim == 3 ? 27 : 9; n->npos = dim == 3 ? 8 : 4;
  n->norm = norm; n->groups = groups;
  n->fuse_act = norm == 0 && !env_on("IUNET_NO_ACT_FUSION");
  n->fuse_bw = norm == 0 && !env_on("IUNET_NO_BW_FUSION");
  n->head_act = norm == 0 && !env_on("IUNET_NO_HEAD_ACT");
  n->gn_head = norm == 1 && !env_on("IUNET_NO_HEAD_ACT") && !env_on("IUNET_NO_HEAD_BN_FUSION") && iunet_head_bn_bwd_ok(base, ncls);
  n->head_bn = n->head_act && !env_on("IUNET_NO_HEAD_BN_FUSION");
  n->gn_conv_stats = norm == 1 && !env_on("IUNET_NO_GN_CONV_STATS");
  n->gn_bw = n->gn_conv_stats && !env_on("IUNET_NO_GN_BW_FUSION");
  for (int l = 0; l < levels; ++l) n->ch.push_back(base << l);
  long long off = 0, pk = 0;
  int nbn = 0;
  auto add = [&](const std::string& name, long long numel) { n->params.push_back({name, off, numel}); const long long o = off; off += numel; return o; };
  auto stage = [&](const std::string& prefix, int ci, int co, int l) {
    for (int j = 1; j <= 2; ++j) {
      TConv c;
      c.ci = j == 1 ? ci : co; c.co = co; c.l = l; c.first = (prefix == "enc0" && j == 1);
      c.name = prefix + ".conv" + std::to_string(j);
      const std::string b = prefix + ".bn" + std::to_string(j);
      c.w = add(c.name + ".weight", (long long)co * c.ci * n->taps);
      c.gamma = add(b + ".weight", co);
      c.beta = add(b + ".bias", co);
      c.bn = nbn++;
      if (c.first) {
        c.first_elems = iunet_pack_first_conv_elems(co, c.ci, n->taps);
        c.first_pk = pk; pk = align256(pk + c.first_elems * 2);
        n->ndesc += 1;
      } else {
        pack_alloc(c.fwd, co, c.ci, n->taps, 0, pk);
        pack_alloc(c.dgr, co, c.ci, n->taps, 1, pk);
        for (int k = 0; k < 2; ++k) n->ndesc += (c.fwd.buf[k] >= 0) + (c.dgr.buf[k] >= 0);
      }
      n->conv.push_back(c);
    }
  };
  for (int l = 0; l < levels; ++l) stage("enc" + std::to_string(l), l == 0 ? cin : n->ch[l - 1], n->ch[l], l);
  auto up_op = [&](const std::string& p, int l) {
    TUp u;
    u.ci = n->ch[l + 1]; u.co = n->ch[l]; u.l = l;
    u.w = add(p + ".up.weight", (long long)u.ci * u.co * n->npos);
    u.b = add(p + ".up.bias", u.co);
    const long long ne = (long long)u.ci * u.co * n->npos;
    u.fwd = pk; pk = align256(pk + ne * 2);
    u.dgr = pk; pk = align256(pk + ne * 2);
    n->ndesc += 2;
    n->up.push_back(u);
  };
  n->nested = nested;
  n->node_at.assign((size_t)levels * levels, -1);
  for (int j = 1; j < levels && nested; ++j)
    for (int i = 0; i + j < levels; ++i) {
      n->node_at[i * levels + j] = (int)n->nodes.size();
      n->nodes.push_back({i, j});
      const std::string p = "dec" + std::to_string(i) + "_" + std::to_string(j);
      up_op(p, i);
      stage(p, (j + 1) * n->ch[i], n->ch[i], i);
    }
  for (int l = levels - 2; l >= 0 && !nested; --l) {
// ... 164 lines not shown
  if (n->nested) {
    for (int l = 0; l < lv; ++l) {
      const long long v = vox(l);
      const int c = n->ch[l], ci = l == 0 ? n->cin : n->ch[l - 1];
      const int k1 = 2 * l, k2 = 2 * l + 1;
      const bool fused = conv2_fused(l);
      void* z1p = fused ? nullptr : (void*)(WS + L.z[k1]);
      const void* x2 = fused ? (const void*)(WS + L.y[k1]) : (const void*)(WS + L.z[k1]);
      rc = l == 0 ? conv_fwd(k1, nullptr, 0, z1p, (long long)c * v, -1, nullptr, 0)
                  : conv_fwd(k1, WS + L.pin[l], (long long)ci * v, z1p, (long long)c * v, -1, nullptr, 0);
      if (rc) return rc;
      const long long z0_ss = (long long)(lv - l) * c * v;
      if (l < lv - 1) rc = conv_fwd(k2, x2, (long long)c * v, WS + L.cat[l], z0_ss, fused ? k1 : -1, WS + L.pin[l + 1], (long long)c * vox(l + 1));
      else rc = conv_fwd(k2, x2, (long long)c * v, WS + L.cat[l], z0_ss, fused ? k1 : -1, nullptr, 0);
      if (rc) return rc;
    }
    for (size_t k = 0; k < n->nodes.size(); ++k) {
      const int i = n->nodes[k].first, j = n->nodes[k].second;
      int di, hi, wi;
      dims(i + 1, di, hi, wi);
      const long long v = vox(i), vi = vox(i + 1);
      const int c = n->ch[i], cn = n->ch[i + 1];
      const int k1 = 2 * (lv + (int)k), k2 = k1 + 1;
      const TUp& u = n->up[k];
      const long long cat_ss = (long long)(lv - i) * c * v, src_ss = (long long)(lv - i - 1) * cn * vi;
      unsigned char* up = WS + L.cat[i] + (long long)j * c * v * 2;
      rc = iunet_convT_fwd(dt, dim, WS + L.cat[i + 1] + (long long)(j - 1) * cn * vi * 2, src_ss, up, cat_ss, K + u.fwd, P + u.b, N, di, hi, wi, cn, c,
                           stream);
      if (rc) return rc;
      const bool fused = conv2_fused(i);
      void* z1p = fused ? nullptr : (void*)(WS + L.z[k1]);
      const void* x2 = fused ? (const void*)(WS + L.y[k1]) : (const void*)(WS + L.z[k1]);
      rc = conv_fwd(k1, WS + L.cat[i], cat_ss, z1p, (long long)c * v, -1, nullptr, 0);
      if (rc) return rc;
      rc = copy_slot(WS + L.up[k], (long long)c * v, up, cat_ss, (long long)c * v, N, stream);
      if (rc) return rc;
      const bool last = k + 1 == n->nodes.size();
      void* z2 = last ? (n->head_act ? nullptr : (void*)(WS + L.z[k2])) : (void*)up;
      rc = conv_fwd(k2, x2, (long long)c * v, z2, last ? (long long)c * v : cat_ss, fused ? k1 : -1, nullptr, 0);
      if (rc) return rc;
    }
  }
  for (int l = 0; l < lv && !n->nested; ++l) {
    const long long v = vox(l);
    const int c = n->ch[l], ci = l == 0 ? n->cin : n->ch[l - 1];
    const int k1 = idx(false, l, 1), k2 = idx(false, l, 2);
    const bool fused = conv2_fused(l);
    void* z1p = fused ? nullptr : (void*)(WS + L.z[k1]);
    const void* x2 = fused ? (const void*)(WS + L.y[k1]) : (const void*)(WS + L.z[k1]);
    rc = l == 0 ? conv_fwd(k1, nullptr, 0, z1p, (long long)c * v, -1, nullptr, 0)
                : conv_fwd(k1, WS + L.pin[l], (long long)ci * v, z1p, (long long)c * v, -1, nullptr, 0);
    if (rc) return rc;
    if (l < lv - 1) rc = conv_fwd(k2, x2, (long long)c * v, WS + L.cat[l], 2ll * c * v, fused ? k1 : -1, WS + L.pin[l + 1], (long long)c * vox(l + 1));
    else rc = conv_fwd(k2, x2, (long long)c * v, WS + L.z[k2], (long long)c * v, fused ? k1 : -1, nullptr, 0);
    if (rc) return rc;
  }
  for (int l = lv - 2; l >= 0 && !n->nested; --l) {
    int di, hi, wi;
    dims(l + 1, di, hi, wi);
    const long long v = vox(l), vi = vox(l + 1);
    const int c = n->ch[l], cn = n->ch[l + 1];
    const int ksrc = l == lv - 2 ? idx(false, l + 1, 2) : idx(true, l + 1, 2);
    const TUp& u = n->up[lv - 2 - l];
    rc = iunet_convT_fwd(dt, dim, WS + L.z[ksrc], (long long)cn * vi, WS + L.cat[l] + (long long)c * v * 2, 2ll * c * v, K + u.fwd, P + u.b, N, di, hi,
                         wi, cn, c, stream);
    if (rc) return rc;
    const int k1 = idx(true, l, 1), k2 = idx(true, l, 2);
    const bool fused = conv2_fused(l);
    void* z1p = fused ? nullptr : (void*)(WS + L.z[k1]);
    const void* x2 = fused ? (const void*)(WS + L.y[k1]) : (const void*)(WS + L.z[k1]);
    rc = conv_fwd(k1, WS + L.cat[l], 2ll * c * v, z1p, (long long)c * v, -1, nullptr, 0);
    if (rc) return rc;
    void* z2 = (l == 0 && (n->head_act || n->gn_head)) ? nullptr : (void*)(WS + L.z[k2]);
    rc = conv_fwd(k2, x2, (long long)c * v, z2, (long long)c * v, fused ? k1 : -1, nullptr, 0);
    if (rc) return rc;
  }

  const long long v0 = vox(0);
  const int c0 = n->ch[0], kl = n->nested ? (int)n->conv.size() - 1 : idx(true, 0, 2);
  if (n->gn_head)
    rc = iunet_head_loss_fwd_act_ps(dt, WS + L.y[kl], (long long)c0 * v0, c0, P + n->head_w, P + n->head_b, n->ncls, target, weight, tdtype, n->kind,
                                    F(L.lslab), F(L.out4), F(L.coef), F(L.scale[kl]), F(L.shift[kl]), 1, N, v0, stream);
  else if (n->head_act)
    rc = iunet_head_loss_fwd_act(dt, WS + L.y[kl], (long long)c0 * v0, c0, P + n->head_w, P + n->head_b, n->ncls, target, weight, tdtype, n->kind,
                                 F(L.lslab), F(L.out4), F(L.coef), F(L.scale[kl]), F(L.shift[kl]), N, v0, stream);
  else
    rc = iunet_head_loss_fwd(dt, WS + L.z[kl], (long long)c0 * v0, c0, P + n->head_w, P + n->head_b, n->ncls, target, weight, tdtype, n->kind,
                             F(L.lslab), F(L.out4), F(L.coef), N, v0, stream);
  if (rc) return rc;
  if (out4 != nullptr) IUNET_CHECK_HIP(hipMemcpyAsync(out4, F(L.out4), 4 * sizeof(float), hipMemcpyDeviceToDevice, (hipStream_t)stream));

  int dy_ready = -1;
  {
    const int nparts = iunet_head_loss_bwd_num_parts(N, v0, n->ncls, c0);
    const TConv& cl = n->conv[kl];
    if (n->gn_head) {
      rc = iunet_head_gn_bwd(dt, WS + L.y[kl], (long long)c0 * v0, c0, P + n->head_w, P + n->head_b, n->ncls, target, weight, tdtype, F(L.coef), 0.f,
                             n->state, F(L.scale[kl]), F(L.shift[kl]), F(L.mean[kl]), F(L.invstd[kl]), P + cl.gamma, n->groups, G + cl.gamma, G + cl.beta,
                             WS + L.dy, (long long)c0 * v0, F(L.hslab), F(L.bnslab), F(L.bncoef), WS + L.dz[kl], N, v0, stream);
      dy_ready = kl;
    } else if (n->head_bn && iunet_head_bn_bwd_ok(c0, n->ncls)) {
      rc = iunet_head_bn_bwd(dt, WS + L.y[kl], (long long)c0 * v0, c0, P + n->head_w, P + n->head_b, n->ncls, target, weight, tdtype, F(L.coef), 0.f,
                             n->state, F(L.scale[kl]), F(L.shift[kl]), F(L.mean[kl]), F(L.invstd[kl]), P + cl.gamma, G + cl.gamma, G + cl.beta,
                             WS + L.dy, (long long)c0 * v0, F(L.hslab), F(L.bnslab), F(L.bncoef), WS + L.dz[kl] ,
                             N, v0, stream);
      dy_ready = kl;
    } else if (n->head_act)
      rc = iunet_head_loss_bwd_dev(dt, WS + L.y[kl], (long long)c0 * v0, c0, P + n->head_w, P + n->head_b, n->ncls, target, weight, tdtype, F(L.coef),
                                   n->state, WS + L.dz[kl], (long long)c0 * v0, F(L.hslab), F(L.scale[kl]), F(L.shift[kl]), N, v0, stream);
    else
      rc = iunet_head_loss_bwd_dev(dt, WS + L.z[kl], (long long)c0 * v0, c0, P + n->head_w, P + n->head_b, n->ncls, target, weight, tdtype, F(L.coef),
                                   n->state, WS + L.dz[kl], (long long)c0 * v0, F(L.hslab), nullptr, nullptr, N, v0, stream);
    if (rc) return rc;
    rc = iunet_reduce_slab(F(L.hslab), nparts, (long long)n->ncls * (c0 + 1), F(L.htmp), 1.0f, 0, stream);
    if (rc) return rc;
    rc = iunet_head_grad_scatter(F(L.htmp), G + n->head_w, G + n->head_b, n->ncls, c0, stream);
    if (rc) return rc;
  }
  auto conv_bwd = [&](int k, const void* dzp, long long dz_ss, const void* xp, long long x_ss, void* dxp, long long dx_ss, int x_act,
                      const void* dpool, long long dpool_ss, int feeds) -> int {
    const TConv& c = n->conv[k];
    int d, h, w;
    dims(c.l, d, h, w);
    const long long v = vox(c.l);
    void* dy = WS + L.dy;
    const void* y = WS + L.y[k];
// ... 96 lines not shown
      if (k + 1 == (int)n->nodes.size() && dy_ready != kl) {
        const bool fused = conv2_fused(i);
        const void* x2 = fused ? (const void*)(WS + L.y[k1]) : (const void*)(WS + L.z[k1]);
        rc = conv_bwd(kl, WS + L.dz[kl], (long long)c * v, x2, (long long)c * v, WS + L.dz[k1], (long long)c * v, fused ? k1 : -1, nullptr, 0, k1);
      } else {
        rc = node_conv2_bwd(s, i, j, nullptr, 0);
      }
      if (rc) return rc;
      const long long cat_ss = (long long)(lv - i) * c * v, dcat_ss = (long long)(j + 1) * c * v;
      rc = copy_slot(WS + L.cat[i] + (long long)j * c * v * 2, cat_ss, WS + L.up[k], (long long)c * v, (long long)c * v, N, stream);
      if (rc) return rc;
      rc = conv_bwd(k1, WS + L.dz[k1], (long long)c * v, WS + L.cat[i], cat_ss, WS + L.ndcat[k], dcat_ss, -1, nullptr, 0, -1);
      if (rc) return rc;
      const TUp& u = n->up[k];
      const void* src = WS + L.cat[i + 1] + (long long)(j - 1) * cn * vi * 2;
      void* dup = WS + L.ndcat[k] + (long long)j * c * v * 2;
      rc = iunet_convT_wgrad(dt, dim, src, (long long)(lv - i - 1) * cn * vi, dup, dcat_ss, F(L.wslab), F(L.bslab[k]), G + u.w, G + u.b, N, di, hi, wi, cn,
                             c, stream);
      if (rc) return rc;
      rc = iunet_convT_dgrad(dt, dim, dup, dcat_ss, WS + L.dT[k], (long long)cn * vi, K + u.dgr, N, di, hi, wi, cn, c, stream);
      if (rc) return rc;
    }
    if (hook) hook(hook_ctx, 0);
    for (int l = lv - 1; l >= 0; --l) {
      const long long v = vox(l);
      const int c = n->ch[l], k1 = 2 * l;
      rc = l < lv - 1 ? node_conv2_bwd(l, l, 0, WS + L.dpin[l + 1], (long long)c * vox(l + 1)) : node_conv2_bwd(l, l, 0, nullptr, 0);
      if (rc) return rc;
      if (l == 0) rc = conv_bwd(k1, WS + L.dz[k1], (long long)c * v, nullptr, 0, nullptr, 0, -1, nullptr, 0, -1);
      else {
        const int cp = n->ch[l - 1];
        rc = conv_bwd(k1, WS + L.dz[k1], (long long)c * v, WS + L.pin[l], (long long)cp * v, WS + L.dpin[l], (long long)cp * v, -1, nullptr, 0, -1);
      }
      if (rc) return rc;
      if (hook && l == lv - 1) hook(hook_ctx, 1);
    }
    return IUNET_OK;
  }
  for (int l = 0; l < lv - 1; ++l) {
    int di, hi, wi;
    dims(l + 1, di, hi, wi);
    const long long v = vox(l), vi = vox(l + 1);
    const int c = n->ch[l], cn = n->ch[l + 1];
    const int k1 = idx(true, l, 1), k2 = idx(true, l, 2);
    const bool fused = conv2_fused(l);
    const void* x2 = fused ? (const void*)(WS + L.y[k1]) : (const void*)(WS + L.z[k1]);
    rc = conv_bwd(k2, WS + L.dz[k2], (long long)c * v, x2, (long long)c * v, WS + L.dz[k1], (long long)c * v, fused ? k1 : -1, nullptr, 0, k1);
    if (rc) return rc;
    rc = conv_bwd(k1, WS + L.dz[k1], (long long)c * v, WS + L.cat[l], 2ll * c * v, WS + L.dcat[l], 2ll * c * v, -1, nullptr, 0, -1);
    if (rc) return rc;
    const int ksrc = l == lv - 2 ? idx(false, l + 1, 2) : idx(true, l + 1, 2);
    const TUp& u = n->up[lv - 2 - l];
    void* dup = WS + L.dcat[l] + (long long)c * v * 2;
    rc = iunet_convT_wgrad(dt, dim, WS + L.z[ksrc], (long long)cn * vi, dup, 2ll * c * v, F(L.wslab), F(L.bslab[l]), G + u.w, G + u.b, N, di, hi, wi, cn,
                           c, stream);
    if (rc) return rc;
    rc = iunet_convT_dgrad(dt, dim, dup, 2ll * c * v, WS + L.dz[ksrc], (long long)cn * vi, K + u.dgr, N, di, hi, wi, cn, c, stream);
    if (rc) return rc;
  }
  if (hook) hook(hook_ctx, 0);
  for (int l = lv - 1; l >= 0; --l) {
    const long long v = vox(l);
    const int c = n->ch[l];
    const int k1 = idx(false, l, 1), k2 = idx(false, l, 2);
    const bool fused = conv2_fused(l);
    const void* x2 = fused ? (const void*)(WS + L.y[k1]) : (const void*)(WS + L.z[k1]);
    if (l == lv - 1)
      rc = conv_bwd(k2, WS + L.dz[k2], (long long)c * v, x2, (long long)c * v, WS + L.dz[k1], (long long)c * v, fused ? k1 : -1, nullptr, 0, k1);
    else
      rc = conv_bwd(k2, WS + L.dcat[l], 2ll * c * v, x2, (long long)c * v, WS + L.dz[k1], (long long)c * v, fused ? k1 : -1, WS + L.dpin[l + 1],
                    (long long)c * vox(l + 1), k1);
    if (rc) return rc;
    if (l == 0) rc = conv_bwd(k1, WS + L.dz[k1], (long long)c * v, nullptr, 0, nullptr, 0, -1, nullptr, 0, -1);
    else {
      const int cp = n->ch[l - 1];
      rc = conv_bwd(k1, WS + L.dz[k1], (long long)c * v, WS + L.pin[l], (long long)cp * v, WS + L.dpin[l], (long long)cp * v, -1, nullptr, 0, -1);
    }
    if (rc) return rc;
    if (hook && l == lv - 1 && lv > 1) hook(hook_ctx, 1);
  }
  return IUNET_OK;
}

int iunet_train_update(iunet_train* n, float lr, float b1, float b2, float eps, float wd, float world, void* stream) {
  IUNET_REQUIRE(n && n->packed, "train_update: iunet_train_bind has not been called");
  const int rc = iunet_adamw_step_dev(n->flat, n->grad, n->m, n->v, n->nparams, lr, b1, b2, eps, wd, n->state, n->dtype == 0 ? 1 : 0, world, stream);
  if (rc) return rc;
  return iunet_pack_batch(n->packed + n->table_off, n->ndesc, 0, stream);
}

int iunet_train_step(iunet_train* n, const void* x, int in_dtype, const long long* in_strides, const void* target, const void* weight,
                     int tdtype, int N, int D, int H, int W, void* workspace, float lr, float b1, float b2, float eps, float wd, void* out4,
                     void* stream) {
  const int rc = iunet_train_forward_backward(n, x, in_dtype, in_strides, target, weight, tdtype, N, D, H, W, workspace, out4, stream);
  if (rc) return rc;
  return iunet_train_update(n, lr, b1, b2, eps, wd, 1.0f, stream);
}

}
```

### interactive-unet_amd/interactive_unet/train_engine.py

```python
import ctypes
import math

import os

import torch

from . import _native as nv
from . import topology
from .engine import BN_EPS
from .topology import _vox, check_spatial

LOSS_KINDS = {'ce': 0, 'dice': 1, 'iou': 2, 'mcc': 3, 'dice_ce': 4, 'iou_ce': 5, 'mcc_ce': 6}
BN_MOMENTUM = 0.1


def metrics(out4, sync):
    if not sync:
        return out4
    o = out4.tolist()
    return {'Loss': o[0], 'Dice': o[1], 'IoU': o[2], 'MCC': o[3]}


class TrainEngineBase:

# ... 49 lines not shown
        D, H, W = sp if self.dim == 3 else (1,) + sp
        vox = D * H * W
        if convert_x and X.dtype not in nv.IN_DTYPE_CODE:
            X = X.float()
        return X, y, w, N, D, H, W, vox, (self.cin * vox, vox, H * W, W, 1)

    def _repack_more(self):
        """sync_weights: what holds packed operators beside repack()'s."""

    def sync_weights(self):
        ver = sum(self.p(n)._version for n in self.names)
        if ver != getattr(self, '_seen_version', None):
            if getattr(self, '_seen_version', None) is not None:
                self.repack()
                self._repack_more()
                self.model._packed_sig = None
            self._seen_version = ver


class TrainEngine(TrainEngineBase):
    def __init__(self, model, lr=None, loss_kind='mcc_ce', betas=(0.9, 0.999), eps=1e-8, weight_decay=1e-2,
                 loss_scale=None, process_group=None):
        self.model = model
        self.dev = model.device
        if self.dev.type != 'cuda':
            raise RuntimeError('native training runs on the GPU only (no CPU fallback)')
        nv.lib()
        self.dim, self.levels, self.ch = model.dim, model.levels, topology.channels(model.base, model.levels)
        self.cin, self.ncls = model.num_channels, model.num_classes
        self.T = model.act_dtype
        if self.T not in nv.DTYPE_CODE:
            raise NotImplementedError("native training runs with 16-bit activations (act_dtype 'fp16' / 'bf16'); "
                                      "act_dtype='fp32' is the inference parity mode")
        self.dt = nv.DTYPE_CODE[self.T]
        self.es = 2
        self.taps, self.npos = 3 ** self.dim, 2 ** self.dim
        self.lr = model.lr if lr is None else lr
        self.kind = LOSS_KINDS[loss_kind] if isinstance(loss_kind, str) else int(loss_kind)
        self.betas, self.eps, self.wd = betas, eps, weight_decay
        self.dynamic_scale = self.T == torch.float16 and loss_scale is None
        self.state = torch.zeros(8, dtype=torch.float32, device=self.dev)
        nv.call('iunet_train_state_init', nv.ptr(self.state), float(loss_scale) if loss_scale is not None else (1024.0 if self.T == torch.float16 else 1.0),
                int(self.dynamic_scale), nv.stream())
        self.pg = process_group
        self.fuse_act = not os.environ.get('IUNET_NO_ACT_FUSION')
        self.norm, self.groups = getattr(model, 'norm', 'batch'), getattr(model, 'groups', 8)
        self.gn = self.norm == 'group'
        if self.gn:
            self.fuse_act = False
        self.fuse_bw = not self.gn and not os.environ.get('IUNET_NO_BW_FUSION')
        self.gn_conv_stats = self.gn and not os.environ.get('IUNET_NO_GN_CONV_STATS')
        self.gn_bw = self.gn_conv_stats and not os.environ.get('IUNET_NO_GN_BW_FUSION')
        self.head_act = not self.gn and not os.environ.get('IUNET_NO_HEAD_ACT')
        self.head_bn = self.head_act and not os.environ.get('IUNET_NO_HEAD_BN_FUSION')
        self.gn_head = (self.gn and not os.environ.get('IUNET_NO_HEAD_ACT') and not os.environ.get('IUNET_NO_HEAD_BN_FUSION')
                        and bool(nv.lib().iunet_head_bn_bwd_ok(self.ch[0], self.ncls)))
        self._bw_ready = {}
        self._flatten()
        self._bucket_bounds(self._first_decoder_param())
        if self.pg is not None:
            from . import dp
            dp.broadcast_state(self.flat, [model.tensor(n) for n in model._names
                                           if n.endswith('running_mean') or n.endswith('running_var')], self.pg)
            self.buckets = dp.GradBuckets(self.grad, self._dec_start, self.pg)
        self._alloc_packed()
        self._ws = {}
        self.probe = None
        self.use_handle = True
        self.repack()
        model._packed_sig = None

    @property
    def loss_scale(self):
        return float(self.state[0].item())

    @loss_scale.setter
    def loss_scale(self, value):
        self.state[0:1].fill_(float(value))
        self._fixed_scale = None

    @property
    def step_count(self):
        return int(self.state.view(torch.int32)[1].item())

    @property
    def good_steps(self):
        return int(self.state.view(torch.int32)[2].item())

    @property
    def last_step_ok(self):
        return int(self.state.view(torch.int32)[3].item()) == 0

    def _first_decoder_param(self):
        return f'dec{self.levels - 2}.up.weight'

    def _alloc_packed(self):
        self.pk = {}
        for prefix in self.stage_names():
            ci, co, _ = self.stage_io(prefix)
            for j, (a, b) in enumerate(((ci, co), (co, co)), 1):
                name = f'{prefix}.conv{j}'
                if name == 'enc0.conv1':
                    self.pk[name] = (torch.empty(nv.lib().iunet_pack_first_conv_elems(b, a, self.taps), dtype=self.T,
                                                 device=self.dev), None)
                else:
                    self.pk[name] = (nv.PackedConv(b, a, self.taps, self.T, self.dev),
# ... 120 lines not shown
            lay, w, _ = pk.pick(self.dim, N, *d, act=x_act is not None)
            nparts = nv.lib().iunet_conv3_stats_parts(self.dim, N, *d, co, lay)
            probe = self.probe if (self.probe is not None and self.probe['name'] == name) else None
            if probe is not None:
                e0 = torch.cuda.Event(enable_timing=True)
                e0.record()
            if self.gn and x_act is None and self.gn_conv_stats:
                gn_rows = nv.lib().iunet_conv3_sample_stats_rows(self.dt, self.dim, N, d[0], d[1], d[2], ci, co, lay)
            if gn_rows > 0:
                nv.call('iunet_conv3_fwd_sample_stats', self.dt, self.dim, x_ptr, x_ss, self._P(y), co * v, nv.ptr(w), nv.ptr(stats),
                        N, d[0], d[1], d[2], ci, co, lay, s)
            elif x_act is None:
                nv.call('iunet_conv3_fwd', self.dt, self.dim, x_ptr, x_ss, self._P(y), co * v, nv.ptr(w), None,
                        None if self.gn else nv.ptr(stats), N, d[0], d[1], d[2], ci, co, 0, lay, s)
            else:
                nv.call('iunet_conv3_fwd_act', self.dt, self.dim, x_ptr, x_ss, self._P(y), co * v, nv.ptr(w), None,
                        nv.ptr(stats), nv.ptr(ws['scale.' + x_act]), nv.ptr(ws['shift.' + x_act]),
                        N, d[0], d[1], d[2], ci, co, 0, lay, s)
            if probe is not None:
                e1 = torch.cuda.Event(enable_timing=True)
                e1.record()
                probe['events'].append((e0, e1, N))
        bn = name.replace('conv', 'bn')
        if self.gn:
            if pool is not None:
                p_ptr, p_ss, do = pool
                nv.call('iunet_gn_relu_pool_fwd_rows', self.dt, self.dim, self._P(y), co * v, z_ptr, z_ss, p_ptr, p_ss, nv.ptr(self.p(bn + '.weight')),
                        nv.ptr(self.p(bn + '.bias')), self.groups, BN_EPS, nv.ptr(stats if gn_rows > 0 else ws['bnslab']), gn_rows, nv.ptr(ws['scale.' + name]),
                        nv.ptr(ws['shift.' + name]), nv.ptr(ws['mean.' + name]), nv.ptr(ws['invstd.' + name]), co, N, do[0], do[1], do[2], s)
            else:
                nv.call('iunet_gn_relu_fwd_rows', self.dt, self._P(y), co * v, z_ptr, z_ss, nv.ptr(self.p(bn + '.weight')),
                        nv.ptr(self.p(bn + '.bias')), self.groups, BN_EPS, nv.ptr(stats if gn_rows > 0 else ws['bnslab']), gn_rows, nv.ptr(ws['scale.' + name]),
                        nv.ptr(ws['shift.' + name]), nv.ptr(ws['mean.' + name]), nv.ptr(ws['invstd.' + name]), co, N, v, s)
            return
        nv.call('iunet_bn_finalize', nv.ptr(stats), nparts, co, float(N) * v,
                nv.ptr(self.p(bn + '.weight')), nv.ptr(self.p(bn + '.bias')),
                nv.ptr(self.p(bn + '.running_mean')), nv.ptr(self.p(bn + '.running_var')), BN_MOMENTUM, BN_EPS,
                nv.ptr(ws['scale.' + name]), nv.ptr(ws['shift.' + name]), nv.ptr(ws['mean.' + name]),
                nv.ptr(ws['invstd.' + name]), s)
        if z_ptr is not None and pool is not None:
            p_ptr, p_ss, do = pool
            nv.call('iunet_bn_relu_pool_fwd', self.dt, self.dim, self._P(y), co * v, z_ptr, z_ss, p_ptr, p_ss,
                    nv.ptr(ws['scale.' + name]), nv.ptr(ws['shift.' + name]), co, N, do[0], do[1], do[2], s)
        elif z_ptr is not None:
            nv.call('iunet_bn_relu_fwd', self.dt, self._P(y), co * v, z_ptr, z_ss, nv.ptr(ws['scale.' + name]),
                    nv.ptr(ws['shift.' + name]), co, N, v, s)

    def _conv2_input(self, ws, stage, l, N):
        if self.fuse_act and self.pk[f'{stage}.conv2'][0].pick(self.dim, N, *ws['dims'][l], act=True)[2]:
            return self._P(ws[f'y.{stage}.conv1']), f'{stage}.conv1', None
        z1 = ws[f'z.{stage}.conv1']
        return self._P(z1), None, self._P(z1)

    def forward_train(self, x, x_strides, N, D, H, W):
        ws = self.workspace(N, D, H, W)
        L, ch, dims = self.levels, self.ch, ws['dims']
        s = nv.stream()
        for l in range(L):
            v = _vox(dims[l])
            ci = self.cin if l == 0 else ch[l - 1]
            x2, act, z1p = self._conv2_input(ws, f'enc{l}', l, N)
            if l == 0:
                self._stage_conv_fwd(ws, 'enc0.conv1', None, 0, ci, ch[0], 0, z1p, ch[0] * v, N, x_raw=(x, x_strides))
            else:
                self._stage_conv_fwd(ws, f'enc{l}.conv1', self._P(ws[f'pin{l}']), ci * v, ci, ch[l], l, z1p, ch[l] * v, N)
            if l < L - 1:
                do = dims[l + 1]
                self._stage_conv_fwd(ws, f'enc{l}.conv2', x2, ch[l] * v, ch[l], ch[l], l,
                                     self._P(ws[f'cat{l}']), 2 * ch[l] * v, N, x_act=act,
                                     pool=(self._P(ws[f'pin{l + 1}']), ch[l] * _vox(do), do))
            else:
                self._stage_conv_fwd(ws, f'enc{l}.conv2', x2, ch[l] * v, ch[l], ch[l], l,
                                     self._P(ws[f'z.enc{l}.conv2']), ch[l] * v, N, x_act=act)
        for l in range(L - 2, -1, -1):
            v, vi, di = _vox(dims[l]), _vox(dims[l + 1]), dims[l + 1]
            src = ws[f'z.enc{l + 1}.conv2'] if l == L - 2 else ws[f'z.dec{l + 1}.conv2']
            wf, _ = self.pk[f'dec{l}.up']
            nv.call('iunet_convT_fwd', self.dt, self.dim, self._P(src), ch[l + 1] * vi, self._P(ws[f'cat{l}'], ch[l] * v),
                    2 * ch[l] * v, nv.ptr(wf), nv.ptr(self.p(f'dec{l}.up.bias')), N, di[0], di[1], di[2],
                    ch[l + 1], ch[l], s)
            x2, act, z1p = self._conv2_input(ws, f'dec{l}', l, N)
            self._stage_conv_fwd(ws, f'dec{l}.conv1', self._P(ws[f'cat{l}']), 2 * ch[l] * v, 2 * ch[l], ch[l], l,
                                 z1p, ch[l] * v, N)
            z2 = None if (l == 0 and (self.head_act or self.gn_head)) else self._P(ws[f'z.dec{l}.conv2'])
            self._stage_conv_fwd(ws, f'dec{l}.conv2', x2, ch[l] * v, ch[l], ch[l], l, z2, ch[l] * v, N, x_act=act)
        return ws

    def train_loss_forward(self, ws, y, w, N, vox):
        if self.head_act or self.gn_head:
            return self.loss_forward(ws, ws['y.dec0.conv2'], y, w, N, vox, act='dec0.conv2')
        return self.loss_forward(ws, ws['z.dec0.conv2'], y, w, N, vox)

    def loss_forward(self, ws, feat, y, w, N, vox, act=None):
        hw = self.p('head.weight')
        tdt = {torch.float32: 0, torch.float16: 1}[y.dtype]
        if w is not None and w.dtype != y.dtype:
            w = w.to(y.dtype)
        if act is None:
            nv.call('iunet_head_loss_fwd', self.dt, self._P(feat), self.ch[0] * vox, self.ch[0], nv.ptr(hw),
                    nv.ptr(self.p('head.bias')), self.ncls, nv.ptr(y), nv.ptr(w), tdt, self.kind, nv.ptr(ws['lslab']),
                    nv.ptr(ws['out4']), nv.ptr(ws['coef']), N, vox, nv.stream())
        else:
            nv.call('iunet_head_loss_fwd_act_ps', self.dt, self._P(feat), self.ch[0] * vox, self.ch[0], nv.ptr(hw),
                    nv.ptr(self.p('head.bias')), self.ncls, nv.ptr(y), nv.ptr(w), tdt, self.kind, nv.ptr(ws['lslab']),
                    nv.ptr(ws['out4']), nv.ptr(ws['coef']), nv.ptr(ws['scale.' + act]), nv.ptr(ws['shift.' + act]),
                    int(self.gn), N, vox, nv.stream())
        return tdt, w

    def _stage_conv_bwd(self, ws, name, dz_ptr, dz_ss, z_ptr, z_ss, x_ptr, x_ss, ci, co, l, dx_ptr, dx_ss, N,
                        x_raw=None, x_act=None, pool_bwd=None, feeds=None, dy_ready=False):
        d = ws['dims'][l]
        v = _vox(d)
        s = nv.stream()
        bn = name.replace('conv', 'bn')
        dy = ws['dy']
        first = name == 'enc0.conv1'
        if dy_ready:
            pass
        elif self.gn and pool_bwd is not None:
            dp_ptr, dp_ss, do = pool_bwd
            nv.call('iunet_gn_relu_pool_bwd', self.dt, self.dim, dz_ptr, dz_ss, dp_ptr, dp_ss, self._P(ws['y.' + name]), co * v, self._P(dy), co * v,
                    nv.ptr(self.p(bn + '.weight')), self.groups, nv.ptr(ws['scale.' + name]), nv.ptr(ws['shift.' + name]),
                    nv.ptr(ws['mean.' + name]), nv.ptr(ws['invstd.' + name]), nv.ptr(self.g(bn + '.weight')),
                    nv.ptr(self.g(bn + '.bias')), nv.ptr(ws['bnslab']), nv.ptr(ws['bncoef']), co, N, do[0], do[1], do[2], s)
        elif self.gn:
            rows = self._bw_ready.pop(name, 0)
            nv.call('iunet_gn_relu_bwd_rows', self.dt, dz_ptr, dz_ss, self._P(ws['y.' + name]), co * v, self._P(dy), co * v,
                    nv.ptr(self.p(bn + '.weight')), self.groups, nv.ptr(ws['scale.' + name]), nv.ptr(ws['shift.' + name]),
                    nv.ptr(ws['mean.' + name]), nv.ptr(ws['invstd.' + name]), nv.ptr(self.g(bn + '.weight')),
                    nv.ptr(self.g(bn + '.bias')), nv.ptr(ws['stats'] if rows > 0 else ws['bnslab']), rows, nv.ptr(ws['bncoef']), co, N, v, s)
        elif pool_bwd is not None:
            dp_ptr, dp_ss, do = pool_bwd
            nv.call('iunet_bn_relu_pool_bwd', self.dt, self.dim, dz_ptr, dz_ss, dp_ptr, dp_ss, self._P(ws['y.' + name]), co * v,
                    self._P(dy), co * v, nv.ptr(ws['mean.' + name]), nv.ptr(ws['invstd.' + name]),
                    nv.ptr(self.p(bn + '.weight')), nv.ptr(ws['scale.' + name]), nv.ptr(ws['shift.' + name]),
                    nv.ptr(self.g(bn + '.weight')), nv.ptr(self.g(bn + '.bias')),
                    nv.ptr(ws['bnslab']), nv.ptr(ws['bncoef']), co, N, do[0], do[1], do[2], s)
# ... 45 lines not shown
                        nv.ptr(ws['stats']), self._P(ws['y.' + feeds]), ci * v, nv.ptr(ws['mean.' + feeds]),
                        nv.ptr(ws['invstd.' + feeds]), nv.ptr(ws['scale.' + feeds]), nv.ptr(ws['shift.' + feeds]),
                        N, d[0], d[1], d[2], co, ci, lay, s)
                self._bw_ready[feeds] = gn_rows
            else:
                nv.call('iunet_conv3_fwd', self.dt, self.dim, self._P(dy), co * v, dx_ptr, dx_ss, nv.ptr(wd), None, None,
                        N, d[0], d[1], d[2], co, ci, 0, lay, s)

    def backward(self, ws, x, x_strides, y, w, tdt, N):
        L, ch, dims = self.levels, self.ch, ws['dims']
        s = nv.stream()
        v0 = _vox(dims[0])
        dfeat = ws['dz.dec0.conv2']
        nparts = nv.lib().iunet_head_loss_bwd_num_parts(N, v0, self.ncls, ch[0])
        dy_ready = None
        if self.gn_head:
            bn = 'dec0.bn2'
            nv.call('iunet_head_gn_bwd', self.dt, self._P(ws['y.dec0.conv2']), ch[0] * v0, ch[0], nv.ptr(self.p('head.weight')),
                    nv.ptr(self.p('head.bias')), self.ncls, nv.ptr(y), nv.ptr(w), tdt, nv.ptr(ws['coef']), 0.0, nv.ptr(self.state),
                    nv.ptr(ws['scale.dec0.conv2']), nv.ptr(ws['shift.dec0.conv2']), nv.ptr(ws['mean.dec0.conv2']), nv.ptr(ws['invstd.dec0.conv2']),
                    nv.ptr(self.p(bn + '.weight')), self.groups, nv.ptr(self.g(bn + '.weight')), nv.ptr(self.g(bn + '.bias')), self._P(ws['dy']), ch[0] * v0,
                    nv.ptr(ws['hslab']), nv.ptr(ws['bnslab']), nv.ptr(ws['bncoef']), self._P(dfeat), N, v0, s)
            dy_ready = 'dec0.conv2'
        elif self.head_bn and nv.lib().iunet_head_bn_bwd_ok(ch[0], self.ncls):
            bn = 'dec0.bn2'
            nv.call('iunet_head_bn_bwd', self.dt, self._P(ws['y.dec0.conv2']), ch[0] * v0, ch[0], nv.ptr(self.p('head.weight')),
                    nv.ptr(self.p('head.bias')), self.ncls, nv.ptr(y), nv.ptr(w), tdt, nv.ptr(ws['coef']), 0.0, nv.ptr(self.state),
                    nv.ptr(ws['scale.dec0.conv2']), nv.ptr(ws['shift.dec0.conv2']), nv.ptr(ws['mean.dec0.conv2']), nv.ptr(ws['invstd.dec0.conv2']),
                    nv.ptr(self.p(bn + '.weight')), nv.ptr(self.g(bn + '.weight')), nv.ptr(self.g(bn + '.bias')), self._P(ws['dy']), ch[0] * v0,
                    nv.ptr(ws['hslab']), nv.ptr(ws['bnslab']), nv.ptr(ws['bncoef']), self._P(dfeat), N, v0, s)
            dy_ready = 'dec0.conv2'
        elif self.head_act:
            nv.call('iunet_head_loss_bwd_dev', self.dt, self._P(ws['y.dec0.conv2']), ch[0] * v0, ch[0], nv.ptr(self.p('head.weight')),
                    nv.ptr(self.p('head.bias')), self.ncls, nv.ptr(y), nv.ptr(w), tdt, nv.ptr(ws['coef']),
                    nv.ptr(self.state), self._P(dfeat), ch[0] * v0, nv.ptr(ws['hslab']), nv.ptr(ws['scale.dec0.conv2']),
                    nv.ptr(ws['shift.dec0.conv2']), N, v0, s)
        else:
            nv.call('iunet_head_loss_bwd_dev', self.dt, self._P(ws['z.dec0.conv2']), ch[0] * v0, ch[0], nv.ptr(self.p('head.weight')),
                    nv.ptr(self.p('head.bias')), self.ncls, nv.ptr(y), nv.ptr(w), tdt, nv.ptr(ws['coef']),
                    nv.ptr(self.state), self._P(dfeat), ch[0] * v0, nv.ptr(ws['hslab']), None, None, N, v0, s)
        nv.call('iunet_reduce_slab', nv.ptr(ws['hslab']), nparts, self.ncls * (ch[0] + 1), nv.ptr(ws['htmp']), 1.0, 0, s)
        nv.call('iunet_head_grad_scatter', nv.ptr(ws['htmp']), nv.ptr(self.g('head.weight')), nv.ptr(self.g('head.bias')), self.ncls, ch[0], s)
        for l in range(0, L - 1):
            v, vi, di = _vox(dims[l]), _vox(dims[l + 1]), dims[l + 1]
            z1, z2 = ws[f'z.dec{l}.conv1'], ws[f'z.dec{l}.conv2']
            dz1, dz2 = ws[f'dz.dec{l}.conv1'], ws[f'dz.dec{l}.conv2']
            x2, act, _ = self._conv2_input(ws, f'dec{l}', l, N)
            self._stage_conv_bwd(ws, f'dec{l}.conv2', self._P(dz2), ch[l] * v, self._P(z2), ch[l] * v, x2,
                                 ch[l] * v, ch[l], ch[l], l, self._P(dz1), ch[l] * v, N, x_act=act, feeds=f'dec{l}.conv1',
                                 dy_ready=dy_ready == f'dec{l}.conv2')
            self._stage_conv_bwd(ws, f'dec{l}.conv1', self._P(dz1), ch[l] * v, self._P(z1), ch[l] * v,
                                 self._P(ws[f'cat{l}']), 2 * ch[l] * v, 2 * ch[l], ch[l], l, self._P(ws[f'dcat{l}']),
                                 2 * ch[l] * v, N)
            src_name = f'enc{l + 1}.conv2' if l == L - 2 else f'dec{l + 1}.conv2'
            src, dsrc = ws['z.' + src_name], ws['dz.' + src_name]
            dup = self._P(ws[f'dcat{l}'], ch[l] * v)
            nv.call('iunet_convT_wgrad', self.dt, self.dim, self._P(src), ch[l + 1] * vi, dup, 2 * ch[l] * v,
                    nv.ptr(ws['wslab']), nv.ptr(ws[f'bslab{l}']), nv.ptr(self.g(f'dec{l}.up.weight')),
                    nv.ptr(self.g(f'dec{l}.up.bias')), N, di[0], di[1], di[2], ch[l + 1], ch[l], s)
            _, wd = self.pk[f'dec{l}.up']
            nv.call('iunet_convT_dgrad', self.dt, self.dim, dup, 2 * ch[l] * v, self._P(dsrc), ch[l + 1] * vi,
                    nv.ptr(wd), N, di[0], di[1], di[2], ch[l + 1], ch[l], s)
        if self.pg is not None:
            self.buckets.start_tail()
        for l in range(L - 1, -1, -1):
            v = _vox(dims[l])
            z1, dz1 = ws[f'z.enc{l}.conv1'], ws[f'dz.enc{l}.conv1']
            pool_bwd = None
            if l == L - 1:
                dz2_ptr, dz2_ss = self._P(ws[f'dz.enc{l}.conv2']), ch[l] * v
                z2_ptr, z2_ss = self._P(ws[f'z.enc{l}.conv2']), ch[l] * v
            else:
                do = dims[l + 1]
                pool_bwd = (self._P(ws[f'dpin{l + 1}']), ch[l] * _vox(do), do)
                dz2_ptr, dz2_ss = self._P(ws[f'dcat{l}']), 2 * ch[l] * v
                z2_ptr, z2_ss = self._P(ws[f'cat{l}']), 2 * ch[l] * v
            x2, act, _ = self._conv2_input(ws, f'enc{l}', l, N)
            self._stage_conv_bwd(ws, f'enc{l}.conv2', dz2_ptr, dz2_ss, z2_ptr, z2_ss, x2, ch[l] * v, ch[l],
                                 ch[l], l, self._P(dz1), ch[l] * v, N, x_act=act, pool_bwd=pool_bwd, feeds=f'enc{l}.conv1')
            if l == 0:
                self._stage_conv_bwd(ws, 'enc0.conv1', self._P(dz1), ch[0] * v, self._P(z1), ch[0] * v, None, 0,
                                     self.cin, ch[0], 0, None, 0, N, x_raw=(x, x_strides))
            else:
                self._stage_conv_bwd(ws, f'enc{l}.conv1', self._P(dz1), ch[l] * v, self._P(z1), ch[l] * v,
                                     self._P(ws[f'pin{l}']), ch[l - 1] * v, ch[l - 1], ch[l], l,
                                     self._P(ws[f'dpin{l}']), ch[l - 1] * v, N)
            if l == L - 1 and L > 1 and self.pg is not None and self._bottom_start is not None:
                self.buckets.start(self._bottom_start, self._dec_start)

    def optimizer_step(self):
        s = nv.stream()
        n = self.flat.numel()
        world = self.buckets.finish() if self.pg is not None else 1
        nv.call('iunet_adamw_step_dev', nv.ptr(self.flat), nv.ptr(self.grad), nv.ptr(self.m), nv.ptr(self.v), n,
                float(self.lr), self.betas[0], self.betas[1], self.eps, self.wd, nv.ptr(self.state),
                int(self.T == torch.float16), float(world), s)
        self.repack()
        self.model._packed_sig = None

    def train_step(self, X, y, w=None, sync=True):
        self.sync_weights()
        X, y, w, N, D, H, W, vox, xs = self._prep(X, y, w)
        h = self._handle()
        if h is not None and self.pg is not None:
            out4 = h.forward_backward(X, xs, y, w, N, D, H, W, buckets=self.buckets, bottom=(self._bottom_start, self._dec_start))
            world = self.buckets.finish()
            h.update(float(self.lr), self.betas, self.eps, self.wd, float(world))
            self._py_stale = True
            self.model._packed_sig = None
        elif h is not None:
            out4 = h.step(X, xs, y, w, N, D, H, W, float(self.lr), self.betas, self.eps, self.wd)
            self._py_stale = True
# ... 363 lines not shown
```

Before: 753.6 million.

## Fuse BN+ReLU of upsample sources into transposed-conv forward and weight-grad

Adds activation-fused variants of the transposed-conv forward and weight-gradient kernels that apply the previous layer's BN scale/shift and ReLU on load from the raw pre-norm output. The encoder/decoder conv2 stages feeding an upsample no longer write the normalized activation tensor z, which saves a full activation write and read per level. A convT dgrad variant with fused BN statistics is also introduced. In exchange, the per-channel affine is recomputed inside the convT kernels, which costs extra LDS staging and ALU work, and the code paths are enabled by default when group norm is off.

Result: no change. 753.4 million, median of 6 (-0.0%).

```diff
diff --git a/include/iunet.h b/include/iunet.h
--- a/include/iunet.h
+++ b/include/iunet.h
@@ -38,6 +38,9 @@
                       int Ho, int Wo, void* stream);
 int iunet_convT_fwd(int dtype, int nd, const void* x, long long x_ss, void* y, long long y_ss, const void* wpk,
                     const void* bias, int N, int D, int H, int W, int Cin, int Cout, void* stream);
+int iunet_convT_fwd_act(int dtype, int nd, const void* x, long long x_ss, void* y, long long y_ss, const void* wpk,
+                        const void* bias, const void* scale, const void* shift, int N, int D, int H, int W, int Cin, int Cout,
+                        void* stream);
 int iunet_head_fwd(int dtype, const void* x, long long x_ss, int C0, const void* w, const void* bias, int ncls,
                    void* logits, void* probs, void* cls, const long long* out_strides, float divisor, int accumulate,
                    int N, int D, int H, int W, void* stream);
@@ -341,9 +344,16 @@
 int iunet_pack_convT_dgrad(int dtype, const void* w, void* dst, int Cin, int Cout, int npos, void* stream);
 int iunet_convT_dgrad(int dtype, int nd, const void* dy, long long dy_ss, void* dx, long long dx_ss, const void* wpk,
                       int N, int D, int H, int W, int Cin, int Cout, void* stream);
+int iunet_convT_dgrad_stats_rows(int nd, int N, int D, int H, int W, int Cin, int Cout);
+int iunet_convT_dgrad_bnstats(int dtype, int nd, const void* dy, long long dy_ss, void* dx, long long dx_ss, const void* wpk, void* stats,
+                              const void* bw_y, long long bw_y_ss, const void* mean, const void* invstd, const void* scale, const void* shift,
+                              int N, int D, int H, int W, int Cin, int Cout, void* stream);
 int iunet_convT_wgrad_blocks(int nd, int N, int D, int H, int W, int Cin, int Cout);
 int iunet_convT_wgrad(int dtype, int nd, const void* x, long long x_ss, const void* dy, long long dy_ss, void* wslab,
                       void* bslab, void* dW, void* db, int N, int D, int H, int W, int Cin, int Cout, void* stream);
+int iunet_convT_wgrad_act(int dtype, int nd, const void* x, long long x_ss, const void* dy, long long dy_ss, void* wslab,
+                          void* bslab, void* dW, void* db, const void* x_scale, const void* x_shift, int N, int D, int H, int W,
+                          int Cin, int Cout, void* stream);
 int iunet_first_conv_wgrad_blocks(int nd, int N, int D, int H, int W);
 int iunet_first_conv_wgrad(int dtype, int nd, const void* x, int in_dtype, const long long* in_strides, const void* dy,
                            long long dy_ss, void* slab, void* dW, int N, int D, int H, int W, int Cin, int Cout,
diff --git a/interactive-unet_amd/csrc/capi.hip b/interactive-unet_amd/csrc/capi.hip
--- a/interactive-unet_amd/csrc/capi.hip
+++ b/interactive-unet_amd/csrc/capi.hip
@@ -188,6 +188,15 @@
   DT_OK(dtype);
   IUNET_REQUIRE(x && y && wpk, "convT: null pointer");
   return iunet_convT_launch(dtype, nd, x, x_ss, y, y_ss, wpk, (const float*)bias, N, D, H, W, Cin, Cout, (hipStream_t)stream);
+}
+
+int iunet_convT_fwd_act(int dtype, int nd, const void* x, long long x_ss, void* y, long long y_ss, const void* wpk,
+                        const void* bias, const void* scale, const void* shift, int N, int D, int H, int W, int Cin, int Cout, void* stream) {
+  DT_OK(dtype);
+  IUNET_REQUIRE(x && y && wpk, "convT_fwd_act: null pointer");
+  IUNET_REQUIRE(scale && shift, "convT_fwd_act: null scale / shift");
+  return iunet_convT_launch(dtype, nd, x, x_ss, y, y_ss, wpk, (const float*)bias, N, D, H, W, Cin, Cout, (hipStream_t)stream, 0,
+                            (const float*)scale, (const float*)shift);
 }
 
 int iunet_head_fwd(int dtype, const void* x, long long x_ss, int C0, const void* w, const void* bias, int ncls,
diff --git a/interactive-unet_amd/csrc/launchers.h b/interactive-unet_amd/csrc/launchers.h
--- a/interactive-unet_amd/csrc/launchers.h
+++ b/interactive-unet_amd/csrc/launchers.h
@@ -36,7 +36,8 @@
 int iunet_maxpool_q_launch(int nd, const void* x, long long x_ss, void* y, long long y_ss, int planes16, int N, int Do, int Ho, int Wo,
                            hipStream_t stream);
 int iunet_convT_launch(int dtype, int nd, const void* x, long long x_ss, void* y, long long y_ss, const void* wpk,
-                       const float* bias, int N, int D, int H, int W, int Cin, int Cout, hipStream_t stream, int out8 = 0);
+                       const float* bias, int N, int D, int H, int W, int Cin, int Cout, hipStream_t stream, int out8 = 0,
+                       const float* act_scale = nullptr, const float* act_shift = nullptr);
 int iunet_pack_convT_launch(int dtype, const float* w, void* dst, int Cin, int Cout, int npos, hipStream_t stream);
 int iunet_head_launch(int dtype, const void* x, long long x_ss, int C0, const float* w, const float* bias, int ncls,
                       float* logits, float* probs, unsigned char* cls, const long long* os, float divisor, int accumulate, int N,
diff --git a/interactive-unet_amd/csrc/pointwise.hip b/interactive-unet_amd/csrc/pointwise.hip
--- a/interactive-unet_amd/csrc/pointwise.hip
+++ b/interactive-unet_amd/csrc/pointwise.hip
@@ -231,9 +231,22 @@
   const void* wpk; const float* bias;
   int N, D, H, W, Cin, Cout;
   int out8;
+  const float* act_scale; const float* act_shift;
 };
 
-template <typename T, int ND, bool O8 = false>
+template <typename T>
+__device__ __forceinline__ V8T<T> bn_relu8_lds(V8T<T> v, const float* sc, const float* sh, int c0) {
+  const f32x4 s0 = *(const f32x4*)(sc + c0), s1 = *(const f32x4*)(sc + c0 + 4), h0 = *(const f32x4*)(sh + c0), h1 = *(const f32x4*)(sh + c0 + 4);
+  V8T<T> o;
+#pragma unroll
+  for (int j = 0; j < 4; ++j) {
+    o[j] = from_f32<T>(fmaxf(fmaf(s0[j], to_f32<T>(v[j]), h0[j]), 0.f));
+    o[4 + j] = from_f32<T>(fmaxf(fmaf(s1[j], to_f32<T>(v[4 + j]), h1[j]), 0.f));
+  }
+  return o;
+}
+
+template <typename T, int ND, bool O8 = false, bool ACT = false>
 __global__ __launch_bounds__(256) void convT_kernel(ConvTParams p) {
   using V8 = typename Vec8<T>::type;
   constexpr int NPOS = ND == 3 ? 8 : 4;
@@ -259,7 +272,8 @@
 #pragma unroll
   for (int s = 0; s < NPOS; ++s) { acc[s][0] = f32x4{0, 0, 0, 0}; acc[s][1] = f32x4{0, 0, 0, 0}; }
   for (int ks = 0; ks < nk; ++ks) {
-    const V8 b = *(const V8*)(xin + (long long)(ks * 4 + q) * in_plane);
+    V8 b = *(const V8*)(xin + (long long)(ks * 4 + q) * in_plane);
+    if constexpr (ACT) b = bn_relu8<T>(b, p.act_scale, p.act_shift, ks * 32 + q * 8);
 #pragma unroll
     for (int s = 0; s < NPOS; ++s) {
       const V8 a0 = wp[((ks * NPOS + s) * 2 + 0) * 64];
@@ -314,7 +328,7 @@
   }
 }
 
-template <typename T, int ND, int NK, bool O8 = false, int NT = 256>
+template <typename T, int ND, int NK, bool O8 = false, int NT = 256, bool ACT = false>
 __global__ __launch_bounds__(NT, NT == 256 ? 2 : 1) void convT_lds_kernel(ConvTParams p) {
   constexpr int NW = NT / 64;
   using V8 = typename Vec8<T>::type;
@@ -328,7 +342,13 @@
     const u32x4* wsrc = (const u32x4*)p.wpk + (long long)cob * NK * NPOS * 2 * 64;
     stage_to_lds(smem, wsrc, NK * NPOS * 2 * 64, threadIdx.x, NT);
     if (threadIdx.x < 32) ((float*)(smem + NK * NPOS * 2 * 1024))[threadIdx.x] = p.bias ? p.bias[cob * 32 + threadIdx.x] : 0.f;
-  }
+    if constexpr (ACT) {
+      float* act = (float*)(smem + NK * NPOS * 2 * 1024 + 128);
+      for (int c = threadIdx.x; c < NK * 32; c += NT) { act[c] = p.act_scale[c]; act[NK * 32 + c] = p.act_shift[c]; }
+    }
+  }
+  const float* act_sc = (const float*)(smem + NK * NPOS * 2 * 1024 + 128);
+  const float* act_sh = act_sc + NK * 32;
   __syncthreads();
   const int xg = (p.W + 15) / 16;
   const long long rows = (long long)p.D * p.H * xg, ngroups = rows * p.N;
@@ -377,6 +397,12 @@
         for (int s = 0; s < HP; ++s) { acc[g][s][0] = f32x4{0, 0, 0, 0}; acc[g][s][1] = f32x4{0, 0, 0, 0}; }
 #pragma unroll
       for (int ks = 0; ks < NK; ++ks) {
+        if constexpr (ACT) {
+          if (hf == 0) {
+#pragma unroll
+            for (int g = 0; g < G; ++g) b[g][ks] = bn_relu8_lds<T>(b[g][ks], act_sc, act_sh, ks * 32 + q * 8);
+          }
+        }
 #pragma unroll
         for (int s = 0; s < HP; ++s) {
           const V8 a0 = wl[((ks * NPOS + hf * HP + s) * 2 + 0) * 64];
@@ -455,7 +481,7 @@
   }
 }
 
-template <typename T, int ND, bool O8 = false>
+template <typename T, int ND, bool O8 = false, bool ACT = false>
 __global__ __launch_bounds__(256) void convT_chunk_kernel(ConvTParams p) {
   constexpr int NK = 4;
   using V8 = typename Vec8<T>::type;
@@ -478,6 +504,12 @@
   const int src_lo = ((lane & 48) | (l15 >> 1)) * 4, src_hi = src_lo + 8 * 4;
   const bool odd = l15 & 1;
   const V8* wl = (const V8*)smem + lane;
+  const float* act_sc = (const float*)(smem + 2 * NK * NPOS * 2 * 1024);
+  const float* act_sh = act_sc + p.Cin;
+  if constexpr (ACT) {
+    float* act = (float*)(smem + 2 * NK * NPOS * 2 * 1024);
+    for (int c = threadIdx.x; c < p.Cin; c += 256) { act[c] = p.act_scale[c]; act[p.Cin + c] = p.act_shift[c]; }
+  }
 
   for (long long base = (long long)blockIdx.x * 4 * G; base < ngroups; base += (long long)gridDim.x * 4 * G) {
     const long long g0 = base + wave * G;
@@ -525,6 +557,12 @@
       asm volatile("s_waitcnt vmcnt(0)" ::: "memory");
       __syncthreads();
       if (ch + 1 < nchunks) { dma_chunk(ch + 1); load_b(ch + 1, bnext); }
+      if constexpr (ACT) {
+#pragma unroll
+        for (int g = 0; g < G; ++g)
+#pragma unroll
+          for (int ks = 0; ks < NK; ++ks) bcur[g][ks] = bn_relu8_lds<T>(bcur[g][ks], act_sc, act_sh, (ch * NK + ks) * 32 + q * 8);
+      }
       const V8* wb = wl + (ch & 1) * (CHB / 16);
 #pragma unroll
       for (int ks = 0; ks < NK; ++ks)
@@ -701,11 +739,16 @@
 }
 
 int iunet_convT_launch(int dtype, int nd, const void* x, long long x_ss, void* y, long long y_ss, const void* wpk,
-                       const float* bias, int N, int D, int H, int W, int Cin, int Cout, hipStream_t stream, int out8) {
+                       const float* bias, int N, int D, int H, int W, int Cin, int Cout, hipStream_t stream, int out8,
+                       const float* act_scale, const float* act_shift) {
   IUNET_REQUIRE(Cin % 32 == 0 && Cout % 32 == 0, "convT: Cin (%d) and Cout (%d) must be multiples of 32", Cin, Cout);
   IUNET_REQUIRE(!out8 || nd == 3, "convT: e4m3 planes out exist in 3-D only (the K = 128 fp8 convolution's format)");
+  const bool act = act_scale != nullptr;
+  IUNET_REQUIRE(!act_scale == !act_shift, "convT: the input activation needs both scale and shift");
+  IUNET_REQUIRE(!act || !out8, "convT: the input activation exists with 16-bit output only (the training forward)");
+  IUNET_REQUIRE(!act || Cin <= 4096, "convT: the input activation keeps 8 bytes per input channel in LDS (Cin %d > 4096)", Cin);
   ConvTParams p;
-  p.x = x; p.x_sstride = x_ss; p.y = y; p.y_sstride = y_ss; p.wpk = wpk; p.bias = bias;
+  p.x = x; p.x_sstride = x_ss; p.y = y; p.y_sstride = y_ss; p.wpk = wpk; p.bias = bias; p.act_scale = act_scale; p.act_shift = act_shift;
   p.N = N; p.D = D; p.H = H; p.W = W; p.Cin = Cin; p.Cout = Cout; p.out8 = out8;
   const long long waves = (long long)N * D * H * ((W + 15) / 16);
   const int nk = Cin / 32;
@@ -713,7 +756,7 @@
   static const int res8 = getenv("IUNET_CONVT_RES8") ? atoi(getenv("IUNET_CONVT_RES8")) : 1;
   if ((nk <= 4 || (nk == 8 && res8 && nd == 3 && waves >= 2048)) && waves >= 256 && !(chunk4 && nk == 4)) {
     const int npos = nd == 3 ? 8 : 4;
-    const int lds = nk * npos * 2 * 1024 + 128;
+    const int lds = nk * npos * 2 * 1024 + 128 + (act ? nk * 256 : 0);
     const bool big = lds > 65 * 1024;
     const int per_wg = big ? 16 : 8;
     int gx = (int)((waves + per_wg - 1) / per_wg);
@@ -721,7 +764,8 @@
     const int cap = (big ? cap_all / 2 : cap_all) / (Cout / 32) > 8 ? (big ? cap_all / 2 : cap_all) / (Cout / 32) : 8;
     if (gx > cap) gx = cap;
     dim3 g2(gx, Cout / 32);
-#define CTL(TT, NDV, NKV, NTV) do { if (out8 && NDV == 3) { IUNET_SET_MAX_LDS((convT_lds_kernel<TT, 3, NKV, true, NTV>), lds); \
+#define CTL(TT, NDV, NKV, NTV) do { if (act) { IUNET_SET_MAX_LDS((convT_lds_kernel<TT, NDV, NKV, false, NTV, true>), lds); \
+    hipLaunchKernelGGL((convT_lds_kernel<TT, NDV, NKV, false, NTV, true>), g2, dim3(NTV), lds, stream, p); } else if (out8 && NDV == 3) { IUNET_SET_MAX_LDS((convT_lds_kernel<TT, 3, NKV, true, NTV>), lds); \
     hipLaunchKernelGGL((convT_lds_kernel<TT, 3, NKV, true, NTV>), g2, dim3(NTV), lds, stream, p); } else { IUNET_SET_MAX_LDS((convT_lds_kernel<TT, NDV, NKV, false, NTV>), lds); \
     hipLaunchKernelGGL((convT_lds_kernel<TT, NDV, NKV, false, NTV>), g2, dim3(NTV), lds, stream, p); } } while (0)
 #define CTL_NK(TT, NDV) switch (nk) { case 1: CTL(TT, NDV, 1, 256); break; case 2: CTL(TT, NDV, 2, 256); break; case 3: CTL(TT, NDV, 3, 256); break; \
@@ -735,12 +779,13 @@
   }
   if (nk >= 4 && nk % 4 == 0 && waves >= 64) {
     const int npos = nd == 3 ? 8 : 4;
-    const int lds = 2 * 4 * npos * 2 * 1024;
+    const int lds = 2 * 4 * npos * 2 * 1024 + (act ? Cin * 8 : 0);
     int gx = (int)((waves + 7) / 8);
     const int cap = 512 / (Cout / 32) > 1 ? 512 / (Cout / 32) : 1;
     if (gx > cap) gx = cap;
     dim3 g2(gx, Cout / 32);
-#define CTC(TT, NDV) do { if (out8 && NDV == 3) { IUNET_SET_MAX_LDS((convT_chunk_kernel<TT, 3, true>), lds); \
+#define CTC(TT, NDV) do { if (act) { IUNET_SET_MAX_LDS((convT_chunk_kernel<TT, NDV, false, true>), lds); \
+    hipLaunchKernelGGL((convT_chunk_kernel<TT, NDV, false, true>), g2, dim3(256), lds, stream, p); } else if (out8 && NDV == 3) { IUNET_SET_MAX_LDS((convT_chunk_kernel<TT, 3, true>), lds); \
     hipLaunchKernelGGL((convT_chunk_kernel<TT, 3, true>), g2, dim3(256), lds, stream, p); } else { IUNET_SET_MAX_LDS((convT_chunk_kernel<TT, NDV>), lds); \
     hipLaunchKernelGGL((convT_chunk_kernel<TT, NDV>), g2, dim3(256), lds, stream, p); } } while (0)
     if (dtype == 0) { if (nd == 3) CTC(f16, 3); else CTC(f16, 2); } else { if (nd == 3) CTC(bf16, 3); else CTC(bf16, 2); }
@@ -749,7 +794,12 @@
     return IUNET_OK;
   }
   dim3 grid((unsigned)((waves + 3) / 4), Cout / 32);
-  if (dtype == 0) {
+  if (act) {
+    if (dtype == 0) { if (nd == 3) hipLaunchKernelGGL((convT_kernel<f16, 3, false, true>), grid, dim3(256), 0, stream, p);
+                      else hipLaunchKernelGGL((convT_kernel<f16, 2, false, true>), grid, dim3(256), 0, stream, p); }
+    else { if (nd == 3) hipLaunchKernelGGL((convT_kernel<bf16, 3, false, true>), grid, dim3(256), 0, stream, p);
+           else hipLaunchKernelGGL((convT_kernel<bf16, 2, false, true>), grid, dim3(256), 0, stream, p); }
+  } else if (dtype == 0) {
     if (nd == 3 && out8) hipLaunchKernelGGL((convT_kernel<f16, 3, true>), grid, dim3(256), 0, stream, p);
     else if (nd == 3) hipLaunchKernelGGL((convT_kernel<f16, 3>), grid, dim3(256), 0, stream, p);
     else hipLaunchKernelGGL((convT_kernel<f16, 2>), grid, dim3(256), 0, stream, p);
diff --git a/interactive-unet_amd/csrc/train_misc.hip b/interactive-unet_amd/csrc/train_misc.hip
--- a/interactive-unet_amd/csrc/train_misc.hip
+++ b/interactive-unet_amd/csrc/train_misc.hip
@@ -8,9 +8,32 @@
   void* dx; long long dx_ss;
   const void* wpk;
   int N, D, H, W, Cin, Cout;
+  float* stats;
+  const void* bw_y; long long bw_y_ss;
+  const float *bw_mean, *bw_invstd, *bw_scale, *bw_shift;
 };
 
-template <typename T, int ND>
+template <int NCI>
+__device__ __forceinline__ void convT_bw_row(const float (&s1)[NCI][8], const float (&s2)[NCI][8], float* red, float* stats, int C, int cib0) {
+  const int lane = threadIdx.x & 63, wave = threadIdx.x >> 6, l15 = lane & 15, q = lane >> 4;
+#pragma unroll
+  for (int c = 0; c < NCI; ++c)
+#pragma unroll
+    for (int j = 0; j < 8; ++j) {
+      float a = s1[c][j], b = s2[c][j];
+#pragma unroll
+      for (int h = 8; h >= 1; h >>= 1) { a += __shfl_xor(a, h); b += __shfl_xor(b, h); }
+      if (l15 == 0) { red[((wave * NCI + c) * 32 + q * 8 + j) * 2] = a; red[((wave * NCI + c) * 32 + q * 8 + j) * 2 + 1] = b; }
+    }
+  __syncthreads();
+  if ((int)threadIdx.x < NCI * 64) {
+    const int t = threadIdx.x;
+    const float v = ((red[t] + red[NCI * 64 + t]) + red[2 * NCI * 64 + t]) + red[3 * NCI * 64 + t];
+    stats[((long long)blockIdx.x * C + cib0 * 32) * 2 + t] = v;
+  }
+}
+
+template <typename T, int ND, bool BW = false>
 __global__ __launch_bounds__(256) void convT_dgrad_kernel(ConvTDgradParams p) {
   using V8 = V8T<T>;
   constexpr int NPOS = ND == 3 ? 8 : 4;
@@ -18,15 +41,17 @@
   const int l15 = lane & 15, q = lane >> 4;
   const int xg = (p.W + 15) / 16;
   const long long rows = (long long)p.D * p.H * xg;
-  const long long wid = (long long)blockIdx.x * 4 + wave;
-  if (wid >= rows * p.N) return;
+  long long wid = (long long)blockIdx.x * 4 + wave;
+  const bool live = wid < rows * p.N;
+  if constexpr (!BW) { if (!live) return; }
+  else if (!live) wid = rows * p.N - 1;
   const int n = (int)(wid / rows);
   const long long r = wid - n * rows;
   const int xb = (int)(r % xg), y = (int)((r / xg) % p.H), z = (int)(r / ((long long)xg * p.H));
   const int cib = blockIdx.y;
   const int x = xb * 16 + l15;
-  const bool ok = x < p.W;
-  const int xc = ok ? x : p.W - 1;
+  const bool ok = x < p.W && live;
+  const int xc = x < p.W ? x : p.W - 1;
   const int Do = ND == 3 ? p.D * 2 : 1, Ho = p.H * 2, Wo = p.W * 2;
   const long long out_plane = (long long)Do * Ho * Wo * 8;
   const T* dyin = (const T*)p.dy + n * p.dy_ss;
@@ -50,12 +75,30 @@
   V8 o;
 #pragma unroll
   for (int j = 0; j < 4; ++j) { o[j] = from_f32<T>(acc0[j]); o[4 + j] = from_f32<T>(acc1[j]); }
-  if (ok)
-    *(V8*)((T*)p.dx + n * p.dx_ss + (long long)(cib * 4 + q) * in_plane + (((long long)z * p.H + y) * p.W + x) * 8) = o;
-}
-
-template <typename T, int ND, int NK, int NCI>
-__global__ __launch_bounds__(256, (NCI * NK * (ND == 3 ? 16 : 8) <= 64) ? 2 : 1) void convT_dgrad_lds_kernel(ConvTDgradParams p) {
+  const long long eoff = (long long)(cib * 4 + q) * in_plane + (((long long)z * p.H + y) * p.W + x) * 8;
+  if (ok) *(V8*)((T*)p.dx + n * p.dx_ss + eoff) = o;
+  if constexpr (BW) {
+    __shared__ float red[4 * 64];
+    float s1[1][8], s2[1][8];
+#pragma unroll
+    for (int j = 0; j < 8; ++j) { s1[0][j] = 0.f; s2[0][j] = 0.f; }
+    if (ok) {
+      const V8 yv = *(const V8*)((const T*)p.bw_y + n * p.bw_y_ss + eoff);
+      const int c0 = cib * 32 + q * 8;
+#pragma unroll
+      for (int j = 0; j < 8; ++j) {
+        const float yy = to_f32<T>(yv[j]);
+        norm_bwd_sums(norm_masked(norm_z<T>(p.bw_scale[c0 + j], yy, p.bw_shift[c0 + j]), to_f32<T>(o[j])), yy, p.bw_mean[c0 + j], p.bw_invstd[c0 + j],
+                      s1[0][j], s2[0][j]);
+      }
+    }
+    convT_bw_row<1>(s1, s2, red, p.stats, p.Cin, cib);
+  }
+}
+
+template <typename T, int ND, int NK, int NCI, bool BW = false>
+__global__ __launch_bounds__(256, (NCI * NK * (ND == 3 ? 16 : 8) <= 64) ? ((BW && NCI * NK * (ND == 3 ? 16 : 8) <= 32) ? 4 : 2) : 1)
+void convT_dgrad_lds_kernel(ConvTDgradParams p) {
   using V8 = V8T<T>;
   constexpr int NPOS = ND == 3 ? 8 : 4, G = 2;
   constexpr int WCI = NPOS * NK * 2 * 64;
@@ -66,6 +109,18 @@
   {
     const u32x4* wsrc = (const u32x4*)p.wpk + (long long)cib0 * WCI;
     stage_to_lds(smem, wsrc, NCI * WCI, threadIdx.x, 256);
+  }
+  float* bwp = (float*)(smem + NCI * WCI * 16);
+  float bs1[BW ? NCI : 1][8], bs2[BW ? NCI : 1][8];
+  if constexpr (BW) {
+    if (threadIdx.x < NCI * 32) {
+      const int t = threadIdx.x, c = cib0 * 32 + t;
+      bwp[t] = p.bw_mean[c]; bwp[NCI * 32 + t] = p.bw_invstd[c]; bwp[2 * NCI * 32 + t] = p.bw_scale[c]; bwp[3 * NCI * 32 + t] = p.bw_shift[c];
+    }
+#pragma unroll
+    for (int c = 0; c < NCI; ++c)
+#pragma unroll
+      for (int j = 0; j < 8; ++j) { bs1[c][j] = 0.f; bs2[c][j] = 0.f; }
   }
   __syncthreads();
   const int xg = (p.W + 15) / 16;
@@ -80,6 +135,7 @@
     const T* dyb[G];
     long long xoff[G];
     bool okg[G];
+    long long ydel[BW ? G : 1];
 #pragma unroll
     for (int g = 0; g < G; ++g) {
       const long long wid = g0 + g < ngroups ? g0 + g : ngroups - 1;
@@ -93,8 +149,10 @@
       xoff[g] = n * p.dx_ss + (long long)(cib0 * 4 + q) * in_plane + (((long long)z * p.H + y) * p.W + x) * 8;
 #pragma unroll
       for (int c = 0; c < NCI; ++c) { acc[c][g][0] = f32x4{0, 0, 0, 0}; acc[c][g][1] = f32x4{0, 0, 0, 0}; }
-    }
-#pragma unroll
+      if constexpr (BW) ydel[g] = __builtin_amdgcn_readfirstlane(n) * (p.bw_y_ss - p.dx_ss);
+    }
+    constexpr int UNR = (BW && NCI == 2 && NK == 1) ? NPOS / 2 : NPOS;
+#pragma unroll UNR
     for (int s = 0; s < NPOS; ++s) {
       const int a = ND == 3 ? (s >> 2) : 0, b = (s >> 1) & 1, c = s & 1;
       const long long voff = (((long long)a * Ho + b) * Wo + c) * 8;
@@ -123,8 +181,22 @@
 #pragma unroll
         for (int j = 0; j < 4; ++j) { o[j] = from_f32<T>(acc[c][g][0][j]); o[4 + j] = from_f32<T>(acc[c][g][1][j]); }
         if (okg[g]) *(V8*)((T*)p.dx + xoff[g] + (long long)c * 4 * in_plane) = o;
+        if constexpr (BW) if (okg[g]) {
+          const V8 yv = *(const V8*)((const T*)p.bw_y + xoff[g] + ydel[g] + (long long)c * 4 * in_plane);
+          const f32x4* bp = (const f32x4*)(bwp + c * 32 + q * 8);
+#pragma unroll
+          for (int h = 0; h < 2; ++h) {
+            const f32x4 mu = bp[h], is = bp[NCI * 8 + h], sc = bp[2 * NCI * 8 + h], sh = bp[3 * NCI * 8 + h];
+#pragma unroll
+            for (int j = 0; j < 4; ++j) {
+              const float yy = to_f32<T>(yv[4 * h + j]);
+              norm_bwd_sums(norm_masked(norm_z<T>(sc[j], yy, sh[j]), to_f32<T>(o[4 * h + j])), yy, mu[j], is[j], bs1[c][4 * h + j], bs2[c][4 * h + j]);
+            }
+          }
+        }
       }
   }
+  if constexpr (BW) convT_bw_row<NCI>(bs1, bs2, bwp + 4 * NCI * 32, p.stats, p.Cin, cib0);
 }
 
 template <typename T>
@@ -165,9 +237,10 @@
   float* bslab;
   int N, D, H, W, Cin, Cout;
   int tilesZ, tilesY, tilesX;
+  const float* x_scale; const float* x_shift;
 };
 
-template <typename T, int ND, int NCI>
+template <typename T, int ND, int NCI, bool ACT = false>
 __global__ __launch_bounds__(256, 2) void convT_wgrad_kernel(ConvTWgradParams p) {
   using V8 = V8T<T>;
   constexpr int NPOS = ND == 3 ? 8 : 4;
@@ -177,6 +250,7 @@
   constexpr int NVO = OZ * OY * OX;
   constexpr int PLANE_X = NVI * 16 + 64, PLANE_Y = NVO * 16 + 64;
   constexpr int OFF_Y = 4 * PLANE_X;
+  constexpr int OFF_ACT = OFF_Y + 4 * PLANE_Y;
   constexpr int NKS = NVI / 32;
   constexpr int PL = NPOS / 4;
   extern __shared__ __attribute__((aligned(256))) unsigned char smem[];
@@ -241,6 +315,21 @@
       yr[k] = v;
     }
   };
+  auto act_item = [&](u32x4 v, int k) -> u32x4 {
+    if constexpr (ACT) {
+      const float* sc = (const float*)(smem + OFF_ACT) + (k / XIT) * 32 + ((wave >> 1) + 2 * (k % XIT)) * 8;
+      const V8 r = __builtin_bit_cast(V8, v);
+      V8 o;
+#pragma unroll
+      for (int h = 0; h < 2; ++h) {
+        const f32x4 s4 = *(const f32x4*)(sc + 4 * h), h4 = *(const f32x4*)(sc + NCI * 32 + 4 * h);
+#pragma unroll
+        for (int j = 0; j < 4; ++j) o[4 * h + j] = from_f32<T>(fmaxf(fmaf(s4[j], to_f32<T>(r[4 * h + j]), h4[j]), 0.f));
+      }
+      v = __builtin_bit_cast(u32x4, o);
+    }
+    return v;
+  };
   auto commit_x = [&](const u32x4* src) {
 #pragma unroll
     for (int k = 0; k < XIT; ++k) {
@@ -249,12 +338,7 @@
       *(u32x4*)(smem + pl * PLANE_X + pix * 16) = src[k];
     }
   };
-  auto commit_tile = [&]() {
-    commit_x(xr);
-    if (NCI > 1) {
-#pragma unroll
-      for (int k = 0; k < XIT; ++k) xkeep[k] = xr[XIT + k];
-    }
+  auto commit_dy = [&]() {
 #pragma unroll
     for (int k = 0; k < YIT; ++k) {
       const int it = tid + k * 256;
@@ -264,6 +348,26 @@
       for (int j = 0; j < 8; ++j) bacc[j] += to_f32<T>(yr[k][j]);
     }
   };
+  auto commit_tile = [&]() {
+    if constexpr (ACT) {
+      commit_dy();
+      __builtin_amdgcn_sched_barrier(0);
+#pragma unroll
+      for (int k = 0; k < NCI * XIT; ++k) xr[k] = act_item(xr[k], k);
+    }
+    commit_x(xr);
+    if (NCI > 1) {
+#pragma unroll
+      for (int k = 0; k < XIT; ++k) xkeep[k] = xr[XIT + k];
+    }
+    if constexpr (!ACT) commit_dy();
+  };
+  if constexpr (ACT) {
+    if (tid < NCI * 32) {
+      ((float*)(smem + OFF_ACT))[tid] = p.x_scale[cib0 * 32 + tid];
+      ((float*)(smem + OFF_ACT))[NCI * 32 + tid] = p.x_shift[cib0 * 32 + tid];
+    }
+  }
   if ((int)blockIdx.x < ntiles) load_tile(blockIdx.x);
   for (int tile = blockIdx.x; tile < ntiles; tile += gridDim.x) {
     __syncthreads();
@@ -568,8 +672,24 @@
   return IUNET_OK;
 }
 
-int iunet_convT_dgrad(int dtype, int nd, const void* dy, long long dy_ss, void* dx, long long dx_ss, const void* wpk,
-                      int N, int D, int H, int W, int Cin, int Cout, void* stream) {
+static int convT_dgrad_grid(int nd, int N, int D, int H, int W, int Cin, int Cout, int* nci_out) {
+  const long long waves = (long long)N * D * H * ((W + 15) / 16);
+  const int nk = Cout / 32;
+  if (nk <= 4 && waves >= 256) {
+    const int nci = (nk <= 2 && (Cin / 32) % 2 == 0 && (nd == 3 ? 8 : 4) * nk * 2 * 1024 * 2 <= 32768) ? 2 : 1;
+    long long gx = (waves + 7) / 8;
+    const int cap = 1024 / (Cin / 32 / nci);
+    if (gx > cap) gx = cap;
+    *nci_out = nci;
+    return (int)gx;
+  }
+  *nci_out = 0;
+  return (int)((waves + 3) / 4);
+}
+
+static int convT_dgrad_impl(int dtype, int nd, const void* dy, long long dy_ss, void* dx, long long dx_ss, const void* wpk, float* stats,
+                            const void* bw_y, long long bw_y_ss, const float* const* bw_par, int N, int D, int H, int W, int Cin, int Cout,
+                            void* stream) {
   DT_OK(dtype);
   IUNET_REQUIRE(dy && dx && wpk, "convT_dgrad: null pointer");
   IUNET_REQUIRE(nd == 2 || nd == 3, "convT_dgrad: nd must be 2 or 3");
@@ -577,16 +697,22 @@
   IUNET_REQUIRE(Cin >= 32 && Cout >= 32 && Cin % 32 == 0 && Cout % 32 == 0, "convT_dgrad: channels must be positive multiples of 32 (%d, %d)", Cin, Cout);
   ConvTDgradParams p;
   p.dy = dy; p.dy_ss = dy_ss; p.dx = dx; p.dx_ss = dx_ss; p.wpk = wpk; p.N = N; p.D = D; p.H = H; p.W = W; p.Cin = Cin; p.Cout = Cout;
+  const bool bw = bw_y != nullptr;
+  p.stats = stats; p.bw_y = bw_y; p.bw_y_ss = bw_y_ss;
+  p.bw_mean = bw ? bw_par[0] : nullptr; p.bw_invstd = bw ? bw_par[1] : nullptr; p.bw_scale = bw ? bw_par[2] : nullptr; p.bw_shift = bw ? bw_par[3] : nullptr;
   const long long waves = (long long)N * D * H * ((W + 15) / 16);
+  IUNET_REQUIRE(waves + 7 < (1ll << 31), "convT_dgrad: too many voxel groups (%lld)", waves);
   const int nk = Cout / 32;
-  if (nk <= 4 && waves >= 256) {
-    const int nci = (nk <= 2 && (Cin / 32) % 2 == 0 && (nd == 3 ? 8 : 4) * nk * 2 * 1024 * 2 <= 32768) ? 2 : 1;
-    const int lds = (nd == 3 ? 8 : 4) * nk * 2 * 1024 * nci;
-    int gx = (int)((waves + 7) / 8);
-    const int cap = 1024 / (Cin / 32 / nci);
-    if (gx > cap) gx = cap;
+  int nci = 0;
+  const int gx = convT_dgrad_grid(nd, N, D, H, W, Cin, Cout, &nci);
+  if (nci > 0) {
+    const int lds = (nd == 3 ? 8 : 4) * nk * 2 * 1024 * nci + (bw ? nci * 1536 : 0);
     dim3 g2(gx, Cin / 32 / nci);
-#define CDL(TT, NDV, NKV) do { if (nci == 2) { IUNET_SET_MAX_LDS((convT_dgrad_lds_kernel<TT, NDV, NKV, 2>), lds); \
+#define CDL(TT, NDV, NKV) do { if (bw && nci == 2) { IUNET_SET_MAX_LDS((convT_dgrad_lds_kernel<TT, NDV, NKV, 2, true>), lds); \
+      hipLaunchKernelGGL((convT_dgrad_lds_kernel<TT, NDV, NKV, 2, true>), g2, dim3(256), lds, (hipStream_t)stream, p); } \
+    else if (bw) { IUNET_SET_MAX_LDS((convT_dgrad_lds_kernel<TT, NDV, NKV, 1, true>), lds); \
+      hipLaunchKernelGGL((convT_dgrad_lds_kernel<TT, NDV, NKV, 1, true>), g2, dim3(256), lds, (hipStream_t)stream, p); } \
+    else if (nci == 2) { IUNET_SET_MAX_LDS((convT_dgrad_lds_kernel<TT, NDV, NKV, 2>), lds); \
       hipLaunchKernelGGL((convT_dgrad_lds_kernel<TT, NDV, NKV, 2>), g2, dim3(256), lds, (hipStream_t)stream, p); } \
     else { IUNET_SET_MAX_LDS((convT_dgrad_lds_kernel<TT, NDV, NKV, 1>), lds); \
       hipLaunchKernelGGL((convT_dgrad_lds_kernel<TT, NDV, NKV, 1>), g2, dim3(256), lds, (hipStream_t)stream, p); } } while (0)
@@ -598,13 +724,41 @@
     IUNET_CHECK_HIP(hipGetLastError());
     return IUNET_OK;
   }
-  dim3 grid((unsigned)((waves + 3) / 4), Cin / 32);
-  if (dtype == 0) { if (nd == 3) hipLaunchKernelGGL((convT_dgrad_kernel<f16, 3>), grid, dim3(256), 0, (hipStream_t)stream, p);
+  dim3 grid((unsigned)gx, Cin / 32);
+  if (bw) {
+    if (dtype == 0) { if (nd == 3) hipLaunchKernelGGL((convT_dgrad_kernel<f16, 3, true>), grid, dim3(256), 0, (hipStream_t)stream, p);
+                      else hipLaunchKernelGGL((convT_dgrad_kernel<f16, 2, true>), grid, dim3(256), 0, (hipStream_t)stream, p); }
+    else { if (nd == 3) hipLaunchKernelGGL((convT_dgrad_kernel<bf16, 3, true>), grid, dim3(256), 0, (hipStream_t)stream, p);
+           else hipLaunchKernelGGL((convT_dgrad_kernel<bf16, 2, true>), grid, dim3(256), 0, (hipStream_t)stream, p); }
+  }
+  else if (dtype == 0) { if (nd == 3) hipLaunchKernelGGL((convT_dgrad_kernel<f16, 3>), grid, dim3(256), 0, (hipStream_t)stream, p);
                     else hipLaunchKernelGGL((convT_dgrad_kernel<f16, 2>), grid, dim3(256), 0, (hipStream_t)stream, p); }
   else { if (nd == 3) hipLaunchKernelGGL((convT_dgrad_kernel<bf16, 3>), grid, dim3(256), 0, (hipStream_t)stream, p);
          else hipLaunchKernelGGL((convT_dgrad_kernel<bf16, 2>), grid, dim3(256), 0, (hipStream_t)stream, p); }
   IUNET_CHECK_HIP(hipGetLastError());
   return IUNET_OK;
+}
+
+int iunet_convT_dgrad(int dtype, int nd, const void* dy, long long dy_ss, void* dx, long long dx_ss, const void* wpk,
+                      int N, int D, int H, int W, int Cin, int Cout, void* stream) {
+  return convT_dgrad_impl(dtype, nd, dy, dy_ss, dx, dx_ss, wpk, nullptr, nullptr, 0, nullptr, N, D, H, W, Cin, Cout, stream);
+}
+
+int iunet_convT_dgrad_stats_rows(int nd, int N, int D, int H, int W, int Cin, int Cout) {
+  IUNET_REQUIRE(nd == 2 || nd == 3, "convT_dgrad_stats_rows: nd must be 2 or 3");
+  IUNET_REQUIRE_GRID("convT_dgrad_stats_rows", N, D, H, W);
+  IUNET_REQUIRE(Cin >= 32 && Cout >= 32 && Cin % 32 == 0 && Cout % 32 == 0, "convT_dgrad_stats_rows: channels must be positive multiples of 32 (%d, %d)", Cin, Cout);
+  IUNET_REQUIRE((long long)N * D * H * ((W + 15) / 16) + 7 < (1ll << 31), "convT_dgrad_stats_rows: too many voxel groups");
+  int nci;
+  return convT_dgrad_grid(nd, N, D, H, W, Cin, Cout, &nci);
+}
+
+int iunet_convT_dgrad_bnstats(int dtype, int nd, const void* dy, long long dy_ss, void* dx, long long dx_ss, const void* wpk, void* stats,
+                              const void* bw_y, long long bw_y_ss, const void* mean, const void* invstd, const void* scale, const void* shift,
+                              int N, int D, int H, int W, int Cin, int Cout, void* stream) {
+  IUNET_REQUIRE(stats && bw_y && mean && invstd && scale && shift, "convT_dgrad_bnstats: null pointer");
+  const float* par[4] = {(const float*)mean, (const float*)invstd, (const float*)scale, (const float*)shift};
+  return convT_dgrad_impl(dtype, nd, dy, dy_ss, dx, dx_ss, wpk, (float*)stats, bw_y, bw_y_ss, par, N, D, H, W, Cin, Cout, stream);
 }
 
 int iunet_convT_wgrad_blocks(int nd, int N, int D, int H, int W, int Cin, int Cout) {
@@ -618,8 +772,9 @@
   return (int)(nb < 1 ? 1 : nb);
 }
 
-int iunet_convT_wgrad(int dtype, int nd, const void* x, long long x_ss, const void* dy, long long dy_ss, void* wslab,
-                      void* bslab, void* dW, void* db, int N, int D, int H, int W, int Cin, int Cout, void* stream) {
+static int convT_wgrad_impl(int dtype, int nd, const void* x, long long x_ss, const void* dy, long long dy_ss, void* wslab,
+                            void* bslab, void* dW, void* db, const float* x_scale, const float* x_shift, int N, int D, int H, int W,
+                            int Cin, int Cout, void* stream) {
   DT_OK(dtype);
   IUNET_REQUIRE(x && dy && wslab && bslab && dW && db, "convT_wgrad: null pointer");
   IUNET_REQUIRE(Cin >= 32 && Cout >= 32 && Cin % 32 == 0 && Cout % 32 == 0, "convT_wgrad: channels must be positive multiples of 32");
@@ -627,16 +782,21 @@
   IUNET_REQUIRE_GRID("convT_wgrad", N, D, H, W);
   ConvTWgradParams p;
   p.x = x; p.x_ss = x_ss; p.dy = dy; p.dy_ss = dy_ss; p.wslab = (float*)wslab; p.bslab = (float*)bslab;
-  p.N = N; p.D = D; p.H = H; p.W = W; p.Cin = Cin; p.Cout = Cout;
+  p.N = N; p.D = D; p.H = H; p.W = W; p.Cin = Cin; p.Cout = Cout; p.x_scale = x_scale; p.x_shift = x_shift;
+  const bool act = x_scale != nullptr;
   const int TZ = nd == 3 ? 2 : 1, TY = nd == 3 ? 4 : 8, TX = 16;
   p.tilesZ = (D + TZ - 1) / TZ; p.tilesY = (H + TY - 1) / TY; p.tilesX = (W + TX - 1) / TX;
   const int nb = iunet_convT_wgrad_blocks(nd, N, D, H, W, Cin, Cout);
   const int npos = nd == 3 ? 8 : 4;
   const int nvi = 128, nvo = nd == 3 ? 1024 : 512;
-  const int lds = 4 * (nvi * 16 + 64) + 4 * (nvo * 16 + 64);
   const int nci = (Cin / 32) % 2 == 0 ? 2 : 1;
+  const int lds = 4 * (nvi * 16 + 64) + 4 * (nvo * 16 + 64) + (act ? nci * 256 : 0);
   dim3 grid(nb, Cin / 32 / nci, Cout / 32);
-#define CTW(TT, NDV) do { if (nci == 2) { IUNET_SET_MAX_LDS((convT_wgrad_kernel<TT, NDV, 2>), lds); \
+#define CTW(TT, NDV) do { if (act && nci == 2) { IUNET_SET_MAX_LDS((convT_wgrad_kernel<TT, NDV, 2, true>), lds); \
+      hipLaunchKernelGGL((convT_wgrad_kernel<TT, NDV, 2, true>), grid, dim3(256), lds, (hipStream_t)stream, p); } \
+    else if (act) { IUNET_SET_MAX_LDS((convT_wgrad_kernel<TT, NDV, 1, true>), lds); \
+      hipLaunchKernelGGL((convT_wgrad_kernel<TT, NDV, 1, true>), grid, dim3(256), lds, (hipStream_t)stream, p); } \
+    else if (nci == 2) { IUNET_SET_MAX_LDS((convT_wgrad_kernel<TT, NDV, 2>), lds); \
       hipLaunchKernelGGL((convT_wgrad_kernel<TT, NDV, 2>), grid, dim3(256), lds, (hipStream_t)stream, p); } \
     else { IUNET_SET_MAX_LDS((convT_wgrad_kernel<TT, NDV, 1>), lds); \
       hipLaunchKernelGGL((convT_wgrad_kernel<TT, NDV, 1>), grid, dim3(256), lds, (hipStream_t)stream, p); } } while (0)
@@ -647,6 +807,19 @@
                      (const float*)wslab, nb, Cin, Cout, npos, (float*)dW);
   IUNET_CHECK_HIP(hipGetLastError());
   return iunet_reduce_slab(bslab, nb, Cout, db, 1.0f, 0, stream);
+}
+
+int iunet_convT_wgrad(int dtype, int nd, const void* x, long long x_ss, const void* dy, long long dy_ss, void* wslab,
+                      void* bslab, void* dW, void* db, int N, int D, int H, int W, int Cin, int Cout, void* stream) {
+  return convT_wgrad_impl(dtype, nd, x, x_ss, dy, dy_ss, wslab, bslab, dW, db, nullptr, nullptr, N, D, H, W, Cin, Cout, stream);
+}
+
+int iunet_convT_wgrad_act(int dtype, int nd, const void* x, long long x_ss, const void* dy, long long dy_ss, void* wslab,
+                          void* bslab, void* dW, void* db, const void* x_scale, const void* x_shift, int N, int D, int H, int W,
+                          int Cin, int Cout, void* stream) {
+  IUNET_REQUIRE(x_scale && x_shift, "convT_wgrad_act: null scale / shift");
+  return convT_wgrad_impl(dtype, nd, x, x_ss, dy, dy_ss, wslab, bslab, dW, db, (const float*)x_scale, (const float*)x_shift, N, D, H, W,
+                          Cin, Cout, stream);
 }
 
 int iunet_first_conv_wgrad_blocks(int nd, int N, int D, int H, int W) {
diff --git a/interactive-unet_amd/csrc/train_net.hip b/interactive-unet_amd/csrc/train_net.hip
--- a/interactive-unet_amd/csrc/train_net.hip
+++ b/interactive-unet_amd/csrc/train_net.hip
@@ -42,7 +42,7 @@
   int norm = 0, groups = 8;
   int dim, levels, base, cin, ncls, dtype, kind;
   int taps, npos;
-  bool fuse_act, fuse_bw, head_act, gn_conv_stats, gn_bw, head_bn, gn_head;
+  bool fuse_act, fuse_bw, head_act, up_fuse, gn_conv_stats, gn_bw, head_bn, gn_head;
   std::vector<int> ch;
   std::vector<TParam> params;
   long long nparams = 0;
@@ -248,6 +248,7 @@
   n->fuse_act = norm == 0 && !env_on("IUNET_NO_ACT_FUSION");
   n->fuse_bw = norm == 0 && !env_on("IUNET_NO_BW_FUSION");
   n->head_act = norm == 0 && !env_on("IUNET_NO_HEAD_ACT");
+  n->up_fuse = norm == 0 && !nested && !env_on("IUNET_NO_UP_FUSION");
   n->gn_head = norm == 1 && !env_on("IUNET_NO_HEAD_ACT") && !env_on("IUNET_NO_HEAD_BN_FUSION") && iunet_head_bn_bwd_ok(base, ncls);
   n->head_bn = n->head_act && !env_on("IUNET_NO_HEAD_BN_FUSION");
   n->gn_conv_stats = norm == 1 && !env_on("IUNET_NO_GN_CONV_STATS");
@@ -518,7 +519,7 @@
                 : conv_fwd(k1, WS + L.pin[l], (long long)ci * v, z1p, (long long)c * v, -1, nullptr, 0);
     if (rc) return rc;
     if (l < lv - 1) rc = conv_fwd(k2, x2, (long long)c * v, WS + L.cat[l], 2ll * c * v, fused ? k1 : -1, WS + L.pin[l + 1], (long long)c * vox(l + 1));
-    else rc = conv_fwd(k2, x2, (long long)c * v, WS + L.z[k2], (long long)c * v, fused ? k1 : -1, nullptr, 0);
+    else rc = conv_fwd(k2, x2, (long long)c * v, n->up_fuse ? nullptr : (void*)(WS + L.z[k2]), (long long)c * v, fused ? k1 : -1, nullptr, 0);
     if (rc) return rc;
   }
   for (int l = lv - 2; l >= 0 && !n->nested; --l) {
@@ -528,8 +529,12 @@
     const int c = n->ch[l], cn = n->ch[l + 1];
     const int ksrc = l == lv - 2 ? idx(false, l + 1, 2) : idx(true, l + 1, 2);
     const TUp& u = n->up[lv - 2 - l];
-    rc = iunet_convT_fwd(dt, dim, WS + L.z[ksrc], (long long)cn * vi, WS + L.cat[l] + (long long)c * v * 2, 2ll * c * v, K + u.fwd, P + u.b, N, di, hi,
-                         wi, cn, c, stream);
+    if (n->up_fuse)
+      rc = iunet_convT_fwd_act(dt, dim, WS + L.y[ksrc], (long long)cn * vi, WS + L.cat[l] + (long long)c * v * 2, 2ll * c * v, K + u.fwd, P + u.b,
+                               F(L.scale[ksrc]), F(L.shift[ksrc]), N, di, hi, wi, cn, c, stream);
+    else
+      rc = iunet_convT_fwd(dt, dim, WS + L.z[ksrc], (long long)cn * vi, WS + L.cat[l] + (long long)c * v * 2, 2ll * c * v, K + u.fwd, P + u.b, N, di, hi,
+                           wi, cn, c, stream);
     if (rc) return rc;
     const int k1 = idx(true, l, 1), k2 = idx(true, l, 2);
     const bool fused = conv2_fused(l);
@@ -537,7 +542,7 @@
     const void* x2 = fused ? (const void*)(WS + L.y[k1]) : (const void*)(WS + L.z[k1]);
     rc = conv_fwd(k1, WS + L.cat[l], 2ll * c * v, z1p, (long long)c * v, -1, nullptr, 0);
     if (rc) return rc;
-    void* z2 = (l == 0 && (n->head_act || n->gn_head)) ? nullptr : (void*)(WS + L.z[k2]);
+    void* z2 = ((l == 0 && (n->head_act || n->gn_head)) || (l > 0 && n->up_fuse)) ? nullptr : (void*)(WS + L.z[k2]);
     rc = conv_fwd(k2, x2, (long long)c * v, z2, (long long)c * v, fused ? k1 : -1, nullptr, 0);
     if (rc) return rc;
   }
@@ -740,8 +745,12 @@
     const int ksrc = l == lv - 2 ? idx(false, l + 1, 2) : idx(true, l + 1, 2);
     const TUp& u = n->up[lv - 2 - l];
     void* dup = WS + L.dcat[l] + (long long)c * v * 2;
-    rc = iunet_convT_wgrad(dt, dim, WS + L.z[ksrc], (long long)cn * vi, dup, 2ll * c * v, F(L.wslab), F(L.bslab[l]), G + u.w, G + u.b, N, di, hi, wi, cn,
-                           c, stream);
+    if (n->up_fuse)
+      rc = iunet_convT_wgrad_act(dt, dim, WS + L.y[ksrc], (long long)cn * vi, dup, 2ll * c * v, F(L.wslab), F(L.bslab[l]), G + u.w, G + u.b,
+                                 F(L.scale[ksrc]), F(L.shift[ksrc]), N, di, hi, wi, cn, c, stream);
+    else
+      rc = iunet_convT_wgrad(dt, dim, WS + L.z[ksrc], (long long)cn * vi, dup, 2ll * c * v, F(L.wslab), F(L.bslab[l]), G + u.w, G + u.b, N, di, hi, wi, cn,
+                             c, stream);
     if (rc) return rc;
     rc = iunet_convT_dgrad(dt, dim, dup, 2ll * c * v, WS + L.dz[ksrc], (long long)cn * vi, K + u.dgr, N, di, hi, wi, cn, c, stream);
     if (rc) return rc;
diff --git a/interactive-unet_amd/interactive_unet/train_engine.py b/interactive-unet_amd/interactive_unet/train_engine.py
--- a/interactive-unet_amd/interactive_unet/train_engine.py
+++ b/interactive-unet_amd/interactive_unet/train_engine.py
@@ -125,6 +125,7 @@
         self.gn_conv_stats = self.gn and not os.environ.get('IUNET_NO_GN_CONV_STATS')
         self.gn_bw = self.gn_conv_stats and not os.environ.get('IUNET_NO_GN_BW_FUSION')
         self.head_act = not self.gn and not os.environ.get('IUNET_NO_HEAD_ACT')
+        self.up_fuse = not self.gn and not os.environ.get('IUNET_NO_UP_FUSION')
         self.head_bn = self.head_act and not os.environ.get('IUNET_NO_HEAD_BN_FUSION')
         self.gn_head = (self.gn and not os.environ.get('IUNET_NO_HEAD_ACT') and not os.environ.get('IUNET_NO_HEAD_BN_FUSION')
                         and bool(nv.lib().iunet_head_bn_bwd_ok(self.ch[0], self.ncls)))
@@ -351,6 +352,10 @@
         z1 = ws[f'z.{stage}.conv1']
         return self._P(z1), None, self._P(z1)
 
+    def _up_input(self, ws, l):
+        name = f'enc{l + 1}.conv2' if l == self.levels - 2 else f'dec{l + 1}.conv2'
+        return (name, ws['y.' + name], name) if self.up_fuse else (name, ws['z.' + name], None)
+
     def forward_train(self, x, x_strides, N, D, H, W):
         ws = self.workspace(N, D, H, W)
         L, ch, dims = self.levels, self.ch, ws['dims']
@@ -370,18 +375,23 @@
                                      pool=(self._P(ws[f'pin{l + 1}']), ch[l] * _vox(do), do))
             else:
                 self._stage_conv_fwd(ws, f'enc{l}.conv2', x2, ch[l] * v, ch[l], ch[l], l,
-                                     self._P(ws[f'z.enc{l}.conv2']), ch[l] * v, N, x_act=act)
+                                     None if self.up_fuse else self._P(ws[f'z.enc{l}.conv2']), ch[l] * v, N, x_act=act)
         for l in range(L - 2, -1, -1):
             v, vi, di = _vox(dims[l]), _vox(dims[l + 1]), dims[l + 1]
-            src = ws[f'z.enc{l + 1}.conv2'] if l == L - 2 else ws[f'z.dec{l + 1}.conv2']
+            _, src, src_act = self._up_input(ws, l)
             wf, _ = self.pk[f'dec{l}.up']
-            nv.call('iunet_convT_fwd', self.dt, self.dim, self._P(src), ch[l + 1] * vi, self._P(ws[f'cat{l}'], ch[l] * v),
-                    2 * ch[l] * v, nv.ptr(wf), nv.ptr(self.p(f'dec{l}.up.bias')), N, di[0], di[1], di[2],
-                    ch[l + 1], ch[l], s)
+            if src_act is None:
+                nv.call('iunet_convT_fwd', self.dt, self.dim, self._P(src), ch[l + 1] * vi, self._P(ws[f'cat{l}'], ch[l] * v),
+                        2 * ch[l] * v, nv.ptr(wf), nv.ptr(self.p(f'dec{l}.up.bias')), N, di[0], di[1], di[2],
+                        ch[l + 1], ch[l], s)
+            else:
+                nv.call('iunet_convT_fwd_act', self.dt, self.dim, self._P(src), ch[l + 1] * vi, self._P(ws[f'cat{l}'], ch[l] * v),
+                        2 * ch[l] * v, nv.ptr(wf), nv.ptr(self.p(f'dec{l}.up.bias')), nv.ptr(ws['scale.' + src_act]),
+                        nv.ptr(ws['shift.' + src_act]), N, di[0], di[1], di[2], ch[l + 1], ch[l], s)
             x2, act, z1p = self._conv2_input(ws, f'dec{l}', l, N)
             self._stage_conv_fwd(ws, f'dec{l}.conv1', self._P(ws[f'cat{l}']), 2 * ch[l] * v, 2 * ch[l], ch[l], l,
                                  z1p, ch[l] * v, N)
-            z2 = None if (l == 0 and (self.head_act or self.gn_head)) else self._P(ws[f'z.dec{l}.conv2'])
+            z2 = None if ((l == 0 and (self.head_act or self.gn_head)) or (l > 0 and self.up_fuse)) else self._P(ws[f'z.dec{l}.conv2'])
             self._stage_conv_fwd(ws, f'dec{l}.conv2', x2, ch[l] * v, ch[l], ch[l], l, z2, ch[l] * v, N, x_act=act)
         return ws
 
@@ -533,12 +543,18 @@
             self._stage_conv_bwd(ws, f'dec{l}.conv1', self._P(dz1), ch[l] * v, self._P(z1), ch[l] * v,
                                  self._P(ws[f'cat{l}']), 2 * ch[l] * v, 2 * ch[l], ch[l], l, self._P(ws[f'dcat{l}']),
                                  2 * ch[l] * v, N)
-            src_name = f'enc{l + 1}.conv2' if l == L - 2 else f'dec{l + 1}.conv2'
-            src, dsrc = ws['z.' + src_name], ws['dz.' + src_name]
+            src_name, src, src_act = self._up_input(ws, l)
+            dsrc = ws['dz.' + src_name]
             dup = self._P(ws[f'dcat{l}'], ch[l] * v)
-            nv.call('iunet_convT_wgrad', self.dt, self.dim, self._P(src), ch[l + 1] * vi, dup, 2 * ch[l] * v,
-                    nv.ptr(ws['wslab']), nv.ptr(ws[f'bslab{l}']), nv.ptr(self.g(f'dec{l}.up.weight')),
-                    nv.ptr(self.g(f'dec{l}.up.bias')), N, di[0], di[1], di[2], ch[l + 1], ch[l], s)
+            if src_act is None:
+                nv.call('iunet_convT_wgrad', self.dt, self.dim, self._P(src), ch[l + 1] * vi, dup, 2 * ch[l] * v,
+                        nv.ptr(ws['wslab']), nv.ptr(ws[f'bslab{l}']), nv.ptr(self.g(f'dec{l}.up.weight')),
+                        nv.ptr(self.g(f'dec{l}.up.bias')), N, di[0], di[1], di[2], ch[l + 1], ch[l], s)
+            else:
+                nv.call('iunet_convT_wgrad_act', self.dt, self.dim, self._P(src), ch[l + 1] * vi, dup, 2 * ch[l] * v,
+                        nv.ptr(ws['wslab']), nv.ptr(ws[f'bslab{l}']), nv.ptr(self.g(f'dec{l}.up.weight')),
+                        nv.ptr(self.g(f'dec{l}.up.bias')), nv.ptr(ws['scale.' + src_act]), nv.ptr(ws['shift.' + src_act]),
+                        N, di[0], di[1], di[2], ch[l + 1], ch[l], s)
             _, wd = self.pk[f'dec{l}.up']
             nv.call('iunet_convT_dgrad', self.dt, self.dim, dup, 2 * ch[l] * v, self._P(dsrc), ch[l + 1] * vi,
                     nv.ptr(wd), N, di[0], di[1], di[2], ch[l + 1], ch[l], s)
```
